# alexandrainst/coral

Hardware: AMD Instinct MI355X
Metric: audio-seconds/sec (CTC finetune step: fwd+bwd+allreduce+clip+AdamW), wav2vec2-large, 10 s utterances (higher is better)
Workload: dtype bf16; 1 GPU; wav2vec2-large (XLS-R shape d=1920 L=48 ffn=7680) CTC finetune, 8 x 10 s per GPU, SpecAugment on, activation_dropout 0.1, layerdrop 0 (multi-GPU rule), fp32 master + AdamW + clip 1.0; global_batch=8, frames_per_utt=499, parallelism=dp1

## Files before the change

### coral_amd/_lib.py

```python

from __future__ import annotations

import ctypes as C
import os
from pathlib import Path

_HERE = Path(__file__).resolve().parent
LIB_PATH = _HERE / "libcoral_amd.so"


class CoralAmdError(RuntimeError):
    """Raised when the HIP library is missing or a call into it fails."""


class CaGemmDesc(C.Structure):

    _fields_ = [
        ("A", C.c_void_p),
        ("B", C.c_void_p),
        ("C", C.c_void_p),
        ("C2", C.c_void_p),
        ("R", C.c_void_p),
        ("bias", C.c_void_p),
        ("M", C.c_int32),
        ("N", C.c_int32),
        ("K", C.c_int32),
        ("a_layout", C.c_int32),
        ("b_layout", C.c_int32),
        ("lda", C.c_int64),
        ("ldb", C.c_int64),
        ("ldc", C.c_int64),
        ("ldr", C.c_int64),
        ("a_kseg", C.c_int32),
        ("b_kseg", C.c_int32),
        ("a_kseg_stride", C.c_int64),
        ("b_kseg_stride", C.c_int64),
        ("batch1", C.c_int32),
        ("batch2", C.c_int32),
        ("sA1", C.c_int64),
        ("sA2", C.c_int64),
        ("sB1", C.c_int64),
        ("sB2", C.c_int64),
        ("sC1", C.c_int64),
        ("sC2", C.c_int64),
        ("sR1", C.c_int64),
        ("sR2", C.c_int64),
        ("sBias1", C.c_int64),
        ("sBias2", C.c_int64),
        ("epilogue", C.c_int32),
        ("out_f32", C.c_int32),
        ("accumulate", C.c_int32),
        ("alpha", C.c_float),
        ("dropout_p", C.c_float),
        ("dropout_seed", C.c_uint64),
        ("a_colsum", C.c_void_p),
        ("a_colsum_ld", C.c_int64),
        ("c_row_index", C.c_void_p),
        ("c_row_mul", C.c_int64),
        ("c_split_n", C.c_int32),
        ("C_hi", C.c_void_p),
        ("ldc_hi", C.c_int64),
        ("a_scale", C.c_void_p),
        ("b_scale", C.c_void_p),
        ("a_row_scale", C.c_void_p),
        ("c_sumsq", C.c_void_p),
        ("c_stream_out", C.c_int32),
        ("C8", C.c_void_p),
        ("c8_scale", C.c_void_p),
        ("c8_amax", C.c_void_p),
        ("a_ln_gamma", C.c_void_p),
        ("a_ln_beta", C.c_void_p),
        ("a_ln_eps", C.c_float),
        ("xcd_balanced", C.c_int32),
    ]


class CaReduceDesc(C.Structure):
    _fields_ = [("partial", C.c_void_p), ("out", C.c_void_p), ("stride", C.c_int64), ("nparts", C.c_int32),
                ("n", C.c_int32), ("accumulate", C.c_int32)]


class CaDecodeLayer(C.Structure):

    FIELDS = ("ln1_g", "ln1_b", "wqkv", "bqkv", "wo", "bo", "ln2_g", "ln2_b", "wq2", "bq2", "wo2", "bo2", "ln3_g", "ln3_b",
              "w1", "b1", "w2", "b2", "self_kv", "cross_kv")
    _fields_ = [(n, C.c_void_p) for n in FIELDS]


class CaDecodeDesc(C.Structure):

    _fields_ = ([("layers", C.c_void_p)]
                + [(n, C.c_int32) for n in ("n_layers", "B", "d", "f", "H", "Te", "max_len", "V")]
                + [(n, C.c_void_p) for n in ("embed", "embed_pos", "lnf_g", "lnf_b")]
                + [("eps", C.c_float), ("logits", C.c_void_p), ("ld_logits", C.c_int64), ("suppress", C.c_void_p),
                   ("out", C.c_void_p), ("done", C.c_void_p), ("ids", C.c_void_p), ("ld_ids", C.c_int64),
                   ("tok", C.c_void_p), ("pos", C.c_void_p), ("klen", C.c_void_p), ("pad_id", C.c_int32),
                   ("eos_id", C.c_int32), ("ws", C.c_void_p), ("ws_bytes", C.c_int64), ("status", C.c_void_p),
                   ("cross_head_major", C.c_int32)])


DECODE_MAX_B = 16


def decode_ws_bytes(B, d, f, H, n_layers):
    return (8192 + n_layers * 16 * H * 4 + 16 * (7 * d + f) * 2 + 16 * H * 4 * 16 * 66 * 4 + 256 * 16 * 8 + 4096)


class CaAttnDesc(C.Structure):

    _fields_ = ([(n, C.c_void_p) for n in ("Q", "K", "V", "O", "dO", "dQ", "dK", "dV", "lse", "Dq", "klen", "key_slot")]
                + [(n, C.c_int64) for n in ("ldq", "ldk", "ldv", "ldo", "lddo", "lddq", "lddk", "lddv",
                                             "sqb", "skb", "svb", "sob", "sdob", "sdqb", "sdkb", "sdvb")]
                + [(n, C.c_int32) for n in ("B", "H", "Tq", "Tk", "hd", "Tqp", "causal")]
                + [("scale", C.c_float), ("dropout_p", C.c_float), ("dropout_seed", C.c_uint64)]
                + [("O8", C.c_void_p), ("o8_scale", C.c_void_p), ("o8_amax", C.c_void_p),
                   ("split_ws", C.c_void_p), ("split_ws_bytes", C.c_int64), ("row_off", C.c_void_p)])


class CaFp8RefreshTask(C.Structure):

    _fields_ = ([(n, C.c_void_p) for n in ("x_bf16", "q_fp8", "q_fp8_t", "scale", "amax_next")]
                + [("rows", C.c_int32), ("cols", C.c_int32)])


class CaCtcBeamDesc(C.Structure):

    _fields_ = [("logits", C.c_void_p), ("ldv", C.c_int64), ("in_len", C.c_void_p),
                ("B", C.c_int32), ("T", C.c_int32), ("V", C.c_int32), ("blank", C.c_int32), ("delimiter", C.c_int32),
                ("forbidden", C.c_void_p), ("pfx_keys", C.c_void_p), ("pfx_wid", C.c_void_p), ("n_pfx", C.c_int64),
                ("ng_keys", C.c_void_p), ("ng_logp", C.c_void_p), ("ng_backoff", C.c_void_p),
                ("ng_count", C.c_int64 * 5),
                ("order", C.c_int32), ("bos_wid", C.c_int32), ("eos_wid", C.c_int32), ("unk_wid", C.c_int32),
                ("beam_width", C.c_int32),
                ("alpha", C.c_float), ("beta", C.c_float), ("unk_score_offset", C.c_float),
                ("token_min_logp", C.c_float), ("beam_prune_logp", C.c_float), ("score_boundary", C.c_int32),
                ("ids_out", C.c_void_p), ("out_len", C.c_void_p), ("score_out", C.c_void_p),
                ("ws", C.c_void_p), ("ws_bytes", C.c_int64)]


class CaBeamDesc(C.Structure):

    _fields_ = ([(n, C.c_int32) for n in ("B", "k", "max_len", "prompt_len", "max_length", "eos_id", "early_stopping")]
                + [(n, C.c_void_p) for n in ("len_pen", "cand_score", "cand_parent", "cand_token", "run_score", "tok", "pos",
                                              "klen", "anc_in", "anc_out", "ids_in", "ids_out", "fin_score", "fin_len",
                                              "fin_seq", "fin_ids", "fin_count", "heur", "done", "tr_parent", "tr_token",
                                              "tr_score")])


BEAM_MAX_BEAMS, BEAM_MAX_ROWS = 16, 128
ALIGN_MAX_TOKENS, ALIGN_MAX_FRAMES, ALIGN_MAX_HEADS, ALIGN_MAX_HEAD_DIM, ALIGN_MAX_FILTER_WIDTH = 447, 1500, 32, 128, 31


def align_ws_bytes_per_clip(A, Lw, Fmax):
    return A * Fmax * (Lw + 4) * 4


FP8_GROUP_MAX = 8
CTC_COLLAPSE_TILE = 4096
KMAJOR, MNMAJOR = 0, 1
EPI_NONE, EPI_GELU, EPI_RESIDUAL, EPI_DGELU, EPI_GELU_RESIDUAL = 0, 1, 2, 3, 4

_vp, _i32, _i64, _f32, _u64 = C.c_void_p, C.c_int32, C.c_int64, C.c_float, C.c_uint64

SIGNATURES = {
    "ca_version": (C.c_int, []),
    "ca_last_error": (C.c_char_p, []),
    "ca_device_count": (C.c_int, []),
    "ca_gemm_bf16_group": (C.c_int, [_vp, _i32, _vp]),
    "ca_gemm_bf16": (C.c_int, [C.POINTER(CaGemmDesc), _vp]),
    "ca_gemm_fp8": (C.c_int, [C.POINTER(CaGemmDesc), _vp]),
    "ca_quantize_fp8": (C.c_int, [_vp, _i64, _vp, _vp, _vp, _vp]),
    "ca_quantize_fp8_delayed": (C.c_int, [_vp, _i64, _vp, _vp, _vp, _vp]),
    "ca_fp8_amax_rotate": (C.c_int, [_vp, _vp, _vp, _i32, _f32, _vp]),
    "ca_dropout_rows_fp8": (C.c_int, [_vp, _vp, _vp, _vp, _i64, _i32, _f32, _u64, _vp]),
    "ca_quantize_fp8_transposed": (C.c_int, [_vp, _i32, _i32, _vp, _vp, _vp]),
    "ca_fp8_refresh_group": (C.c_int, [_vp, _i32, _vp]),
    "ca_gemm_force_kernel": (C.c_int, [C.c_int]),
    "ca_gemm_debug_general_epilogue": (C.c_int, [C.c_int]),
    "ca_debug_cu_hog": (C.c_int, [_i32, _i32, _i32, C.c_double, _vp]),
    "ca_gemm_set_compute_cus": (C.c_int, [C.c_int]),
    "ca_background_update_fits": (C.c_int, [C.POINTER(C.c_int32)]),
    "ca_prof_begin": (C.c_int, []),
    "ca_prof_end": (C.c_int, [C.POINTER(C.c_double), C.POINTER(C.c_int64), C.POINTER(C.c_double)]),
    "ca_pack_rows": (C.c_int, [_vp, _vp, _vp, _i32, _i32, _i32, _i32, _vp]),
    "ca_unpack_rows": (C.c_int, [_vp, _vp, _vp, _i32, _i32, _i32, _i32, _vp]),
    "ca_attn_fwd": (C.c_int, [C.POINTER(CaAttnDesc), _vp]),
    "ca_attn_bwd": (C.c_int, [C.POINTER(CaAttnDesc), _vp]),
    "ca_decode_attn_qproj": (C.c_int, [C.POINTER(CaAttnDesc), _vp, _i64, _vp, _vp, _f32, _vp, _i64, _vp, _i32, _vp]),
    "ca_layernorm_fwd": (C.c_int, [_vp, _vp, _vp, _vp, _vp, _i64, _i32, _f32, _i32, _vp]),
    "ca_layernorm_fwd_ex": (C.c_int, [_vp, _vp, _vp, _vp, _vp, _i64, _i32, _f32, _i32, _i32, _i32, _vp]),
    "ca_layernorm_bwd_ex": (
        C.c_int,
        [_vp, _vp, _vp, _vp, _vp, _vp, _vp, _vp, _vp, _vp, _i64, _i32, _i32, _i32, _vp],
    ),
    "ca_layernorm_bwd_dropout": (
        C.c_int,
        [_vp, _vp, _vp, _vp, _vp, _vp, _vp, _vp, _f32, _u64, _vp, _vp, _vp, _i64, _i32, _i32, _vp],
    ),
    "ca_layernorm_fwd_fp8": (C.c_int, [_vp, _vp, _vp, _vp, _vp, _vp, _vp, _i64, _i32, _f32, _vp]),
    "ca_layernorm_bwd_partial_floats": (_i64, [_i64, _i32]),
    "ca_layernorm_bwd": (
        C.c_int,
        [_vp, _vp, _vp, _vp, _vp, _vp, _vp, _vp, _vp, _vp, _i64, _i32, _i32, _vp],
    ),
    "ca_colsum_partial_floats": (_i64, [_i64, _i32]),
    "ca_colsum_bf16": (C.c_int, [_vp, _i64, _i64, _i32, _vp, _vp, _i32, _vp, _vp]),
    "ca_dgelu_mul": (C.c_int, [_vp, _vp, _vp, _i64, _vp]),
    "ca_dropout_bf16": (C.c_int, [_vp, _vp, _i64, _f32, _u64, _vp]),
    "ca_reduce_rows_f32": (C.c_int, [_vp, _i32, _i64, _i32, _vp, _i32, _vp]),
    "ca_reduce_rows_multi": (C.c_int, [C.POINTER(CaReduceDesc), _i32, _vp]),
    "ca_wave_normalize": (C.c_int, [_vp, _vp, _vp, _i32, _i64, _f32, _vp]),
    "ca_frame_lengths": (C.c_int, [_vp, _i32, _i64, C.POINTER(C.c_int32), C.POINTER(C.c_int32), _i32, _vp, _vp]),
    "ca_wave_scale": (C.c_int, [_vp, _vp, _vp, _i32, _i64, _vp]),
    "ca_fir_filter": (C.c_int, [_vp, _vp, _vp, _vp, _vp, _i64, _i32, _vp, _i32, _i64, _vp]),
    "ca_mix_noise": (C.c_int, [_vp, _vp, _vp, _i64, _i64, _vp, _vp, _vp, _vp, _i32, _i64, _vp]),
    "ca_white_noise": (C.c_int, [_vp, _i64, C.c_uint64, _vp]),
    "ca_pcm_prepare": (C.c_int, [_vp, _i32, _i64, _vp, _vp, _vp, _i32, _i64, _i32, _i32, _f32, _vp]),
    "ca_conv0_ln_gelu_fwd": (
        C.c_int,
        [_vp, _vp, _vp, _vp, _vp, _vp, _i32, _i64, _i32, _i32, _i32, _f32, _vp],
    ),
    "ca_conv0_bwd_partial_floats": (_i64, [_i32, _i64, _i32, _i32, _i32]),
    "ca_conv0_ln_gelu_bwd": (
        C.c_int,
        [_vp] * 11 + [_i32, _i64, _i32, _i32, _i32, _f32, _vp],
    ),
    "ca_col2im_1d": (C.c_int, [_vp, _vp, _i32, _i64, _i64, _i32, _i32, _i32, _vp]),
    "ca_ctc_workspace_bytes": (_i64, [_i32, _i32, _i32]),
    "ca_ctc_loss_fwd_bwd": (
        C.c_int,
        [_vp, _vp, _vp, _vp, _vp, _vp, _vp, _i32, _i32, _i32, _i64, _i32, _i32, _i32, _vp],
    ),
    "ca_ctc_greedy_decode": (
        C.c_int,
        [_vp, _vp, _vp, _vp, _vp, _i32, _i32, _i32, _i64, _i32, _vp],
    ),
    "ca_ctc_stitch": (C.c_int, [_vp, _vp, _vp, _vp, _i32, _i32, _i32, _i64, _i32, _i32, _vp]),
    "ca_ctc_collapse_workspace_bytes": (_i64, [_i32, _i32]),
    "ca_ctc_collapse_offsets": (C.c_int, [_vp, _vp, _vp, _vp, _vp, _vp, _vp, _i64, _i32, _i32, _i32, _vp]),
    "ca_ctc_beam_workspace_bytes": (_i64, [_i32, _i32, _i32, _i32]),
    "ca_ctc_beam_decode": (C.c_int, [C.POINTER(CaCtcBeamDesc), _vp]),
    "ca_beam_select_workspace_bytes": (_i64, [_i32, _i32, _i32]),
    "ca_beam_select": (C.c_int, [_vp, _i64, _vp, _vp, _i32, _i32, _i32, _vp, _vp, _vp, _vp, _i64, _vp]),
    "ca_beam_advance": (C.c_int, [C.POINTER(CaBeamDesc), _vp]),
    "ca_mask_frames": (C.c_int, [_vp, _vp, _vp, _vp, _vp, _i32, _i32, _i32, _vp]),
    "ca_regroup_pad": (C.c_int, [_vp, _vp, _i32, _i32, _i32, _i32, _i32, _vp]),
    "ca_posconv_partial_floats": (_i64, [_i32]),
    "ca_posconv_weight": (C.c_int, [_vp, _vp, _vp, _vp, _vp, _vp, _i32, _i32, _i32, _vp]),
    "ca_posconv_weight_bwd": (
        C.c_int,
        [_vp, _vp, _vp, _vp, _vp, _vp, _vp, _i32, _i32, _i32, _vp],
    ),
    "ca_cast_f32_bf16": (C.c_int, [_vp, _vp, _i64, _vp]),
    "ca_cast_bf16_f32": (C.c_int, [_vp, _vp, _i64, _vp]),
    "ca_transpose_f32_bf16": (C.c_int, [_vp, _vp, _i32, _i32, _vp]),
    "ca_conv_weight_reorder": (C.c_int, [_vp, _vp, _i32, _i32, _i32, _vp]),
    "ca_conv_weight_grad_reorder": (C.c_int, [_vp, _vp, _i32, _i32, _i32, _vp]),
    "ca_sumsq_f32": (C.c_int, [_vp, _i64, _vp, _i32, _vp, _vp]),
    "ca_sumsq_ranges_f32": (C.c_int, [_vp, _vp, _i32, _vp, _i32, _vp, _vp]),
    "ca_clear_ranges": (C.c_int, [_vp, _vp, _i32, _i64, _vp]),
    "ca_sum_f32": (C.c_int, [_vp, _i64, _vp, _i32, _vp, _vp]),
    "ca_adamw_step": (
        C.c_int,
        [_vp, _vp, _vp, _vp, _vp, _i64, _f32, _f32, _f32, _f32, _f32, _i32, _f32, _f32, _vp, _vp],
    ),
    "ca_adamw_step_ex": (
        C.c_int,
        [_vp, _vp, _vp, _vp, _vp, _i64, _f32, _f32, _f32, _f32, _f32, _i32, _f32, _f32, _vp, _i32, _vp],
    ),
    "ca_adamw_step_g16": (
        C.c_int,
        [_vp, _vp, _vp, _vp, _vp, _i64, _f32, _f32, _f32, _f32, _f32, _i32, _f32, _f32, _vp, _i32, _vp],
    ),
    "ca_logmel_workspace_bytes": (_i64, [_i32]),
    "ca_logmel": (C.c_int, [_vp, _vp, _vp, _vp, _i32, _i64, _i32, _vp]),
    "ca_cross_entropy_fwd_bwd": (
        C.c_int,
        [_vp, _vp, _vp, _vp, _vp, _i64, _i32, _i64, _i32, _vp],
    ),
    "ca_argmax_masked": (C.c_int, [_vp, _vp, _vp, _i64, _i32, _i64, _vp]),
    "ca_whisper_decode_token": (C.c_int, [C.POINTER(CaDecodeDesc), _vp]),
    "ca_whisper_decode_token_supported": (C.c_int, [_i32, _i32, _i32, _i32, _i32]),
    "ca_debug_decode_stamps": (C.c_int, [_vp, _i32]),
    "ca_argmax_advance": (C.c_int, [_vp, _vp, _vp, _i64, _i32, _i64, _vp, _vp, _i64, _vp, _vp, _vp, _i32, _i32, _vp]),
    "ca_argmax_timestamps": (C.c_int, [_vp, _vp, _vp, _i64, _i32, _i64, _vp, _i64, _vp, _i32, _i32, _i32, _i32, _vp]),
    "ca_argmax_timestamps_advance": (C.c_int, [_vp, _vp, _vp, _i64, _i32, _i64, _vp, _vp, _i64, _vp, _vp, _vp, _i32, _i32,
                                               _i32, _i32, _i32, _vp]),
    "ca_pick_scored_advance": (C.c_int, [_vp, _vp, _vp, _i64, _i32, _i64, _f32, _vp, _i64, _vp, _vp, _vp, _vp, _i64, _vp, _vp,
                                         _vp, _i32, _i32, _vp, _i32, _i32, _i32, _vp]),
    "ca_row_token_prob": (C.c_int, [_vp, _vp, _i64, _i32, _i64, _i32, _vp]),
    "ca_whisper_align_cost": (C.c_int, [_vp, C.POINTER(_vp), _i32, C.POINTER(_i32), _i32, _i32, _i32, _i32, _i32, _i32, _i64,
                                        _i64, _vp, _i32, _f32, _i32, _vp, _vp, _i64, _vp]),
    "ca_dtw_token_times": (C.c_int, [_vp, _i32, _i32, _vp, _i32, _vp, _vp, _vp, _vp, _vp, _vp]),
    "ca_embed_tokens": (C.c_int, [_vp, _vp, _vp, _vp, _vp, _i64, _i32, _vp]),
    "ca_embed_tokens_bwd": (C.c_int, [_vp, _vp, _vp, _vp, _vp, _i64, _i32, _vp]),
    "ca_comm_unique_id": (C.c_int, [_vp]),
    "ca_comm_init": (C.c_int, [C.POINTER(_vp), _vp, _i32, _i32]),
    "ca_comm_destroy": (C.c_int, [_vp]),
    "ca_comm_abort": (C.c_int, [_vp]),
    "ca_comm_stream": (_vp, [_vp]),
    "ca_comm_rank": (C.c_int, [_vp]),
    "ca_comm_world": (C.c_int, [_vp]),
    "ca_comm_after": (C.c_int, [_vp, _vp]),
    "ca_comm_before": (C.c_int, [_vp, _vp]),
    "ca_allreduce_bucket": (C.c_int, [_vp, _vp, _i64, _i32]),
    "ca_reduce_scatter_bucket": (C.c_int, [_vp, _vp, _i64, _i32]),
    "ca_allgather_bucket": (C.c_int, [_vp, _vp, _i64, _i32]),
}

_lib = None


def load() -> C.CDLL:
    global _lib
    if _lib is not None:
        return _lib
    path = Path(os.environ.get("CORAL_AMD_LIB", LIB_PATH))
    if not path.exists():
        raise CoralAmdError(
            f"{path} not found: build it with `python -c 'import __graft_entry__ as g; "
            "g.build()'` (or `make -C coral_amd/csrc`). There is no CPU fallback."
        )
    lib = C.CDLL(str(path))
    for name, (res, args) in SIGNATURES.items():
        fn = getattr(lib, name)
        fn.restype = res
        fn.argtypes = args
    _lib = lib
    return lib

# ... 6 lines not shown
```

### coral_amd/csrc/gemm.hip

```cpp
#include "common.h"
#include "gemm_plan.h"
#include <type_traits>
#include <cstdlib>

#define TILE_BYTES (BM * BK * 2)
#define STAGE_BYTES (2 * TILE_BYTES)
#define NSTAGE 2
static_assert(LDS_BYTES >= NSTAGE * STAGE_BYTES, "kernel S: the epilogue staging covers the operand stages");

__device__ __attribute__((aligned(16))) uint32_t g_ca_zero_page[4];
__device__ int g_ca_epi_general = 0;

typedef const __attribute__((address_space(1))) void* gptr_t;
typedef __attribute__((address_space(3))) void* lptr_t;

__device__ __forceinline__ void glds16(const void* g, char* lds_wave_base) {
  asm volatile("s_mov_b32 m0, %1\n\ts_nop 0\n\tglobal_load_lds_dwordx4 %0, off"
               :
               : "v"(g), "s"((uint32_t)(uintptr_t)(lptr_t)lds_wave_base)
               : "memory", "m0");
}

template <int NI>
struct KMajorLoader {
// ... 97 lines not shown
  __device__ __forceinline__ void init_bytes(const char* b, int64_t ld, int row0, int nrows, int wave, int lane) {
    base = b + (int64_t)row0 * ld;
#pragma unroll
    for (int i = 0; i < NI; ++i) {
      const int r = (wave * NI + i) * 8 + (lane >> 3);
      const int c = (lane & 7) ^ ((r >> 1) & 7);
      int rr = row0 + r;
      rr = (rr < nrows ? rr : nrows - 1) - row0;
      kc[i] = c * 16;
      off[i] = (uint32_t)((int64_t)rr * ld + c * 16);
    }
  }
  __device__ __forceinline__ void issue_one(char* tile, int wave, int i) {
    glds16_sbase(base, off[i], (uint32_t)(uintptr_t)(lptr_t)(tile + (wave * NI + i) * 1024));
  }
  __device__ __forceinline__ void issue_one_tail(char* tile, int wave, int krem, int i) {
    glds16_sbase(base, kc[i] < krem ? off[i] : 0u, (uint32_t)(uintptr_t)(lptr_t)(tile + (wave * NI + i) * 1024));
  }
  __device__ __forceinline__ void zero_fix(char* tile, int wave, int lane, int krem) {
#pragma unroll
    for (int i = 0; i < NI; ++i)
      if (kc[i] >= krem) *(uint4*)(tile + (wave * NI + i) * 1024 + lane * 16) = make_uint4(0, 0, 0, 0);
  }
  __device__ __forceinline__ void advance() { base += BK * 2; }
};
template <int NI, int PC>
struct MNMajorStream {
  const char* base;
  uint32_t off[NI];
  int64_t step;
  static constexpr int RPI = 64 / PC;
  __device__ __forceinline__ void init(const __bf16* b, int64_t ld, int col0, int ncols, int wave, int lane) {
    base = (const char*)(b + col0);
    step = (int64_t)BK * ld * 2;
#pragma unroll
    for (int i = 0; i < NI; ++i) {
      const int kr = (wave * NI + i) * RPI + lane / PC;
      const int swz = (kr & 3) | (((kr >> 3) & 1) << 2);
      const int c = (lane % PC) ^ (swz << 1);
      int cc = col0 + c * 8;
      const int nc8 = (ncols + 7) & ~7;
      cc = (cc <= nc8 - 8 ? cc : nc8 - 8) - col0;
      off[i] = (uint32_t)(((int64_t)kr * ld + cc) * 2);
    }
  }
  __device__ __forceinline__ void issue_one(char* tile, int wave, int i) {
    glds16_sbase(base, off[i], (uint32_t)(uintptr_t)(lptr_t)(tile + (wave * NI + i) * 1024));
  }
  __device__ __forceinline__ void issue_one_tail(char* tile, int wave, int lane, int krem, int i) {
    const int kr = (wave * NI + i) * RPI + lane / PC;
    glds16_sbase(base, kr < krem ? off[i] : 0u, (uint32_t)(uintptr_t)(lptr_t)(tile + (wave * NI + i) * 1024));
  }
  __device__ __forceinline__ void zero_fix(char* tile, int wave, int lane, int krem) {
#pragma unroll
    for (int i = 0; i < NI; ++i) {
      const int kr = (wave * NI + i) * RPI + lane / PC;
      if (kr >= krem) *(uint4*)(tile + (wave * NI + i) * 1024 + lane * 16) = make_uint4(0, 0, 0, 0);
    }
  }
  __device__ __forceinline__ void advance() { base += step; }
};

__device__ __forceinline__ bf16x8_t frag_kmajor(const char* tile, int rb, int s, int lane) {
  const int r = rb + (lane & 15);
  const int c = (4 * s + (lane >> 4)) ^ ((r >> 1) & 7);
  return *(const bf16x8_t*)(tile + r * 128 + c * 16);
}
__device__ __forceinline__ bf16x8_t frag_kmajor_async(const char* tile, int rb, int s, int lane) {
  const int r = rb + (lane & 15);
  const int c = (4 * s + (lane >> 4)) ^ ((r >> 1) & 7);
  const uint32_t a = (uint32_t)(uintptr_t)(lptr_t)(tile + r * 128 + c * 16);
  bf16x8_t v;
  asm volatile("ds_read_b128 %0, %1" : "=v"(v) : "v"(a));
  return v;
}
template <int PITCH>
__device__ __forceinline__ bf16x8_t frag_mnmajor(const char* tile, int cb, int s, int lane) {
  const int g = lane >> 4;
  const int q = (lane & 15) >> 2;
  const int p = lane & 3;
  const int kr = 32 * s + 8 * g + q;
  const int swz = q | ((g & 1) << 2);
  const int c = ((cb >> 3) + (p >> 1)) ^ (swz << 1);
  const uint32_t a0 = (uint32_t)(uintptr_t)(lptr_t)(tile + kr * PITCH + c * 16 + (p & 1) * 8);
  s16x4_t lo, hi;
  asm volatile("ds_read_b64_tr_b16 %0, %1" : "=v"(lo) : "v"(a0));
  asm volatile("ds_read_b64_tr_b16 %0, %1 offset:%2" : "=v"(hi) : "v"(a0), "n"(4 * PITCH));
  typedef __attribute__((ext_vector_type(8))) short s16x8_t;
  s16x8_t v = {lo[0], lo[1], lo[2], lo[3], hi[0], hi[1], hi[2], hi[3]};
  return __builtin_bit_cast(bf16x8_t, v);
}
template <int OFF>
__device__ __forceinline__ bf16x8_t lds_read_b128(uint32_t a) {
  static_assert(OFF >= 0 && OFF < 65536, "DS immediate offset");
  bf16x8_t v;
  asm volatile("ds_read_b128 %0, %1 offset:%2" : "=v"(v) : "v"(a), "n"(OFF));
  return v;
}
template <int OFF, int HI>
__device__ __forceinline__ bf16x8_t lds_read_tr(uint32_t a) {
  static_assert(OFF >= 0 && OFF + HI < 65536, "DS immediate offset");
  s16x4_t lo, hi;
  asm volatile("ds_read_b64_tr_b16 %0, %1 offset:%2" : "=v"(lo) : "v"(a), "n"(OFF));
  asm volatile("ds_read_b64_tr_b16 %0, %1 offset:%2" : "=v"(hi) : "v"(a), "n"(OFF + HI));
  typedef __attribute__((ext_vector_type(8))) short s16x8_t;
  s16x8_t v = {lo[0], lo[1], lo[2], lo[3], hi[0], hi[1], hi[2], hi[3]};
  return __builtin_bit_cast(bf16x8_t, v);
}
__device__ __forceinline__ void lds_wait(bf16x8_t (&f)[4]) {
  asm volatile("s_waitcnt lgkmcnt(0)" : "+v"(f[0]), "+v"(f[1]), "+v"(f[2]), "+v"(f[3]));
}

template <int SBM, int SBN>
__device__ __forceinline__ bool tile_of_block(int bid, int ntm, int ntn, int& tm, int& tn, bool bal = false) {
  return tile_of_block_g<SBM, SBN>(bid, (int)gridDim.x, ntm, ntn, tm, tn, bal);
}

__device__ __forceinline__ void epi_load_bias(const CaGemmDesc& d, int lane, int nw, int z1, int z2, float (&bias8)[8]) {
  const int nb = nw + 8 * (lane & 7);
  const int nvalid = (d.N - nb) < 8 ? (d.N - nb) : 8;
#pragma unroll
  for (int e = 0; e < 8; ++e) bias8[e] = 0.f;
  if (d.bias && nvalid > 0) {
    const float* bz = d.bias + z1 * d.sBias1 + z2 * d.sBias2 + nb;
    if (nvalid == 8 && (((uintptr_t)bz) & 15) == 0) {
      const f32x4_t b0 = *(const f32x4_t*)bz, b1 = *(const f32x4_t*)(bz + 4);
#pragma unroll
      for (int e = 0; e < 8; ++e) bias8[e] = e < 4 ? b0[e] : b1[e - 4];
    } else {
#pragma unroll
      for (int e = 0; e < 8; ++e)
        if (e < nvalid) bias8[e] = bz[e];
    }
  }
}
__device__ __forceinline__ void ca_store_fp8x8(unsigned char* dst, const float (&v)[8], float scale, float& amx) {
  float t[8];
#pragma unroll
  for (int e = 0; e < 8; ++e) {
    amx = fmaxf(amx, fabsf(v[e]));
    t[e] = fminf(fmaxf(v[e] * scale, -448.0f), 448.0f);
  }
  unsigned int w0 = 0, w1 = 0;
  w0 = __builtin_amdgcn_cvt_pk_fp8_f32(t[0], t[1], w0, false);
  w0 = __builtin_amdgcn_cvt_pk_fp8_f32(t[2], t[3], w0, true);
  w1 = __builtin_amdgcn_cvt_pk_fp8_f32(t[4], t[5], w1, false);
  w1 = __builtin_amdgcn_cvt_pk_fp8_f32(t[6], t[7], w1, true);
  *(uint2*)dst = make_uint2(w0, w1);
}

template <int EPI, bool F32, bool DROP>
__device__ __forceinline__ void gemm_epilogue_fast(const CaGemmDesc& d, const float* wt, int lane, int mw, int nb, int z,
                                                   int64_t zoffC, int64_t zoffR, const float (&bias8)[8], float& ssq,
                                                   float& amx) {
  const int M = d.M, N = d.N;
  const float alpha = d.alpha;
  const float keep_scale = DROP ? 1.f / (1.f - d.dropout_p) : 1.f;
  const int r0 = lane >> 3, c0 = 8 * (lane & 7);
  constexpr bool NEEDS_R = EPI == CA_EPI_RESIDUAL || EPI == CA_EPI_DGELU;
  const unsigned short* Rp = NEEDS_R ? (const unsigned short*)d.R + zoffR + nb + (int64_t)(mw + r0) * d.ldr : nullptr;
  const int64_t rstep = 8 * d.ldr;
  int64_t coff = zoffC + (int64_t)(mw + r0) * d.ldc + nb;
  const int64_t cstep = 8 * d.ldc;
  uint64_t idx = ((uint64_t)z * M + (mw + r0)) * (uint64_t)N + nb;
  const uint64_t istep = 8ull * (uint64_t)N;
  u16x8_t r_next = {0, 0, 0, 0, 0, 0, 0, 0};
  if (NEEDS_R) r_next = *(const u16x8_t*)Rp;
  const bool c8_on = (EPI == CA_EPI_GELU || EPI == CA_EPI_DGELU) && d.C8 != nullptr;
  const float s8 = c8_on ? d.c8_scale[0] : 1.f;
  unsigned int dg = 0, ds_eff = 0, dthr = 0;
  if (DROP) {
    const uint64_t ilo = ((uint64_t)z * M + mw) * (uint64_t)N;
    const unsigned int sd = (unsigned int)d.dropout_seed * 0x9E3779B9u + (unsigned int)(d.dropout_seed >> 32);
    ds_eff = sd ^ ((unsigned int)(ilo >> 34) * 0x85EBCA6Bu);
    dg = (unsigned int)(idx >> 2);
    dthr = ca_dropout_threshold(d.dropout_p);
  }
  const unsigned int dgstep = (unsigned int)(istep >> 2);
#pragma unroll 2
  for (int it = 0; it < 8; ++it) {
    const u16x8_t r_cur = r_next;
    if (NEEDS_R && it < 7) r_next = *(const u16x8_t*)(Rp + (it + 1) * rstep);
    const float* wr = wt + (it * 8 + r0) * EPI_PITCH + c0;
    const f32x4_t a4 = *(const f32x4_t*)wr, b4 = *(const f32x4_t*)(wr + 4);
    float v[8];
#pragma unroll
    for (int e = 0; e < 8; ++e) v[e] = (e < 4 ? a4[e] : b4[e - 4]) * alpha + bias8[e];
    unsigned int keep = 0xFFu;
    if (DROP) {
      keep = ca_dropout_keep4_lo(ds_eff, dg, dthr) | (ca_dropout_keep4_lo(ds_eff, dg + 1, dthr) << 4);
      dg += dgstep;
    }
    float v2[8];
    if (EPI == CA_EPI_GELU) {
#pragma unroll
      for (int e = 0; e < 8; ++e) {
        float g = gelu_erf(v[e]);
        if (DROP) g = ((keep >> e) & 1u) ? g * keep_scale : 0.f;
        v2[e] = g + 0.f;
      }
    } else if (EPI == CA_EPI_RESIDUAL) {
      if (DROP) {
#pragma unroll
        for (int e = 0; e < 8; ++e) v[e] = ((keep >> e) & 1u) ? v[e] * keep_scale : 0.f;
      }
#pragma unroll
      for (int e = 0; e < 8; ++e) v[e] += bf2f(r_cur[e]);
    } else if (EPI == CA_EPI_DGELU) {
#pragma unroll
      for (int e = 0; e < 8; ++e) {
        float dg = dgelu_erf(bf2f(r_cur[e]));
        if (DROP) dg = ((keep >> e) & 1u) ? dg * keep_scale : 0.f;
        v[e] *= dg;
      }
    }
    if (F32) {
      float* C = (float*)d.C + coff;
      if (d.accumulate) {
        const f32x4_t c0v = *(const f32x4_t*)C, c1v = *(const f32x4_t*)(C + 4);
#pragma unroll
        for (int e = 0; e < 8; ++e) v[e] += e < 4 ? c0v[e] : c1v[e - 4];
      }
      if (d.c_stream_out) {
        __builtin_nontemporal_store((f32x4_t){v[0], v[1], v[2], v[3]}, (f32x4_t*)C);
        __builtin_nontemporal_store((f32x4_t){v[4], v[5], v[6], v[7]}, (f32x4_t*)(C + 4));
      } else {
        *(f32x4_t*)C = (f32x4_t){v[0], v[1], v[2], v[3]};
        *(f32x4_t*)(C + 4) = (f32x4_t){v[4], v[5], v[6], v[7]};
      }
#pragma unroll
      for (int e = 0; e < 8; ++e) ssq = fmaf(v[e], v[e], ssq);
    } else {
      u16x8_t o;
#pragma unroll
      for (int e = 0; e < 8; ++e) o[e] = f2bf(v[e]);
      if (d.c_stream_out)
        __builtin_nontemporal_store(o, (u16x8_t*)((unsigned short*)d.C + coff));
      else
        *(u16x8_t*)((unsigned short*)d.C + coff) = o;
      if (EPI == CA_EPI_NONE && d.c_sumsq != nullptr) {
#pragma unroll
        for (int e = 0; e < 8; ++e) ssq = fmaf(bf2f(o[e]), bf2f(o[e]), ssq);
      }
      if (EPI == CA_EPI_DGELU && c8_on) ca_store_fp8x8((unsigned char*)d.C8 + coff, v, s8, amx);
    }
    if (EPI == CA_EPI_GELU) {
      u16x8_t o;
#pragma unroll
      for (int e = 0; e < 8; ++e) o[e] = f2bf(v2[e]);
      *(u16x8_t*)((unsigned short*)d.C2 + coff) = o;
      if (c8_on) ca_store_fp8x8((unsigned char*)d.C8 + coff, v2, s8, amx);
    }
    coff += cstep;
  }
}

template <bool PARKED = false>
__device__ __forceinline__ void gemm_epilogue(const CaGemmDesc& d, f32x4_t (&acc)[4][4], char* smem,
                                              int wave, int lane, int mw, int nw, int z, int z1,
                                              int z2, const float (*bias_pre)[8] = nullptr) {
  const int M = d.M, N = d.N;
  const int64_t zoffC = z1 * d.sC1 + z2 * d.sC2;
  const int64_t zoffR = z1 * d.sR1 + z2 * d.sR2;
  const bool vec_ok = ((d.ldc & 7) == 0) && ((zoffC & 7) == 0) && ((d.ldr & 7) == 0) && ((zoffR & 7) == 0);
  const float keep_scale = d.dropout_p > 0.f ? 1.f / (1.f - d.dropout_p) : 1.f;
  const int nb = nw + 8 * (lane & 7);
  const int nvalid = (N - nb) < 8 ? (N - nb) : 8;
  const bool full = nvalid == 8 && vec_ok;
  const int epi = d.epilogue;
  const bool has_gelu = epi == CA_EPI_GELU || epi == CA_EPI_GELU_RESIDUAL;
  const bool needs_r = epi == CA_EPI_RESIDUAL || epi == CA_EPI_DGELU || epi == CA_EPI_GELU_RESIDUAL;
  float bias8[8];
  if (bias_pre) {
#pragma unroll
    for (int e = 0; e < 8; ++e) bias8[e] = (*bias_pre)[e];
  } else {
    epi_load_bias(d, lane, nw, z1, z2, bias8);
  }
  const unsigned short* Rbase = (const unsigned short*)d.R + zoffR + nb;
  auto load_r = [&](int it, u16x8_t& u) {
    const int m = mw + it * 8 + (lane >> 3);
    if (needs_r && full && it < 8 && m < M) u = *(const u16x8_t*)(Rbase + (int64_t)m * d.ldr);
  };
  u16x8_t r_next = {0, 0, 0, 0, 0, 0, 0, 0};
  load_r(0, r_next);

  float* wt = (float*)smem + wave * (64 * EPI_PITCH);
  if (!PARKED) {
#pragma unroll
    for (int i = 0; i < 4; ++i)
#pragma unroll
      for (int j = 0; j < 4; ++j)
        *(f32x4_t*)(wt + (i * 16 + (lane & 15)) * EPI_PITCH + j * 16 + 4 * (lane >> 4)) = acc[i][j];
    asm volatile("s_waitcnt lgkmcnt(0)" ::: "memory");
  }
  const bool c8_on = d.C8 != nullptr && (epi == CA_EPI_GELU || epi == CA_EPI_DGELU);
  if (nvalid <= 0 && d.c_sumsq == nullptr && !c8_on) return;
  float ssq = 0.f;
  float amx = 0.f;
  const float s8 = c8_on ? d.c8_scale[0] : 1.f;
  const bool drop_on = d.dropout_p > 0.f;
  const bool drop32_ok = !drop_on || ((((uint64_t)z * M + mw) * (uint64_t)N) >> 34) == ((((uint64_t)z * M + mw + 64) * (uint64_t)N) >> 34);
  const bool interior = g_ca_epi_general == 0 && mw + 64 <= M && nw + 64 <= N && vec_ok && (N & 7) == 0 && d.C != nullptr && drop32_ok &&
                        (d.out_f32 || !d.accumulate) && (!has_gelu || (epi == CA_EPI_GELU && d.C2 != nullptr && !d.out_f32)) &&
                        !(d.out_f32 && epi != CA_EPI_NONE) && !(drop_on && epi == CA_EPI_NONE);
  if (interior) {
#define EPI_FAST(E, F, D) gemm_epilogue_fast<E, F, D>(d, wt, lane, mw, nb, z, zoffC, zoffR, bias8, ssq, amx)
    if (d.out_f32) {
      EPI_FAST(CA_EPI_NONE, true, false);
    } else if (epi == CA_EPI_NONE) {
      EPI_FAST(CA_EPI_NONE, false, false);
    } else if (epi == CA_EPI_GELU) {
      if (drop_on) EPI_FAST(CA_EPI_GELU, false, true); else EPI_FAST(CA_EPI_GELU, false, false);
    } else if (epi == CA_EPI_RESIDUAL) {
      if (drop_on) EPI_FAST(CA_EPI_RESIDUAL, false, true); else EPI_FAST(CA_EPI_RESIDUAL, false, false);
    } else {
      if (drop_on) EPI_FAST(CA_EPI_DGELU, false, true); else EPI_FAST(CA_EPI_DGELU, false, false);
    }
#undef EPI_FAST
  } else {
#pragma unroll 1
  for (int it = 0; it < 8; ++it) {
    const int ml = it * 8 + (lane >> 3);
    const int m = mw + ml;
    const u16x8_t r_cur = r_next;
    load_r(it + 1, r_next);
    if (m >= M || nvalid <= 0) continue;
    const f32x4_t a4 = *(const f32x4_t*)(wt + ml * EPI_PITCH + 8 * (lane & 7));
    const f32x4_t b4 = *(const f32x4_t*)(wt + ml * EPI_PITCH + 8 * (lane & 7) + 4);
    float v[8], v2[8], r[8];
#pragma unroll
    for (int e = 0; e < 8; ++e) {
      v[e] = (e < 4 ? a4[e] : b4[e - 4]) * d.alpha + bias8[e];
      v2[e] = 0.f;
      r[e] = 0.f;
    }
    const int64_t coff = zoffC + (int64_t)m * d.ldc + nb;
    if (needs_r) {
      if (full) {
#pragma unroll
        for (int e = 0; e < 8; ++e) r[e] = bf2f(r_cur[e]);
      } else {
        const unsigned short* R = Rbase + (int64_t)m * d.ldr;
#pragma unroll
        for (int e = 0; e < 8; ++e)
          if (e < nvalid) r[e] = bf2f(R[e]);
      }
    }
    unsigned int keep = 0xFFu;
    if (d.dropout_p > 0.f && (has_gelu || epi == CA_EPI_DGELU || epi == CA_EPI_RESIDUAL)) {
      const uint64_t idx = ((uint64_t)z * M + m) * (uint64_t)N + nb;
      if ((idx & 3) == 0) {
        keep = ca_dropout_keep4(d.dropout_seed, idx, d.dropout_p) |
               (ca_dropout_keep4(d.dropout_seed, idx + 4, d.dropout_p) << 4);
      } else {
        keep = 0;
#pragma unroll
        for (int e = 0; e < 8; ++e) keep |= (ca_dropout_keep(d.dropout_seed, idx + e, d.dropout_p) ? 1u : 0u) << e;
      }
    }
    if (has_gelu) {
#pragma unroll
      for (int e = 0; e < 8; ++e) {
        float g = gelu_erf(v[e]);
        if (d.dropout_p > 0.f) g = ((keep >> e) & 1u) ? g * keep_scale : 0.f;
        v2[e] = g + r[e];
      }
    } else if (epi == CA_EPI_RESIDUAL) {
      if (d.dropout_p > 0.f) {
#pragma unroll
        for (int e = 0; e < 8; ++e) v[e] = ((keep >> e) & 1u) ? v[e] * keep_scale : 0.f;
      }
#pragma unroll
      for (int e = 0; e < 8; ++e) v[e] += r[e];
    } else if (epi == CA_EPI_DGELU) {
#pragma unroll
      for (int e = 0; e < 8; ++e) {
        float dg = dgelu_erf(r[e]);
        if (d.dropout_p > 0.f) dg = ((keep >> e) & 1u) ? dg * keep_scale : 0.f;
        v[e] *= dg;
      }
    }
    if (d.out_f32) {
      float* C = (float*)d.C + coff;
      if (full) {
        if (d.accumulate) {
          const f32x4_t c0 = *(const f32x4_t*)C, c1 = *(const f32x4_t*)(C + 4);
#pragma unroll
          for (int e = 0; e < 8; ++e) v[e] += e < 4 ? c0[e] : c1[e - 4];
        }
        *(f32x4_t*)C = (f32x4_t){v[0], v[1], v[2], v[3]};
        *(f32x4_t*)(C + 4) = (f32x4_t){v[4], v[5], v[6], v[7]};
#pragma unroll
        for (int e = 0; e < 8; ++e) ssq = fmaf(v[e], v[e], ssq);
      } else {
#pragma unroll
        for (int e = 0; e < 8; ++e)
          if (e < nvalid) {
            const float t = d.accumulate ? C[e] + v[e] : v[e];
            C[e] = t;
            ssq = fmaf(t, t, ssq);
          }
      }
    } else if (d.C) {
      unsigned short* C = (unsigned short*)d.C + coff;
      if (full) {
        if (d.accumulate) {
          const u16x8_t c = *(const u16x8_t*)C;
#pragma unroll
          for (int e = 0; e < 8; ++e) v[e] += bf2f(c[e]);
        }
        u16x8_t o;
#pragma unroll
        for (int e = 0; e < 8; ++e) o[e] = f2bf(v[e]);
        *(u16x8_t*)C = o;
        if (d.c_sumsq != nullptr) {
#pragma unroll
          for (int e = 0; e < 8; ++e) ssq = fmaf(bf2f(o[e]), bf2f(o[e]), ssq);
        }
      } else {
#pragma unroll
        for (int e = 0; e < 8; ++e)
          if (e < nvalid) {
            const unsigned short t = f2bf(d.accumulate ? bf2f(C[e]) + v[e] : v[e]);
            C[e] = t;
            ssq = fmaf(bf2f(t), bf2f(t), ssq);
          }
      }
    }
    if (has_gelu && d.C2) {
      unsigned short* C2 = (unsigned short*)d.C2 + coff;
      if (full) {
        u16x8_t o;
#pragma unroll
        for (int e = 0; e < 8; ++e) o[e] = f2bf(v2[e]);
        *(u16x8_t*)C2 = o;
      } else {
#pragma unroll
        for (int e = 0; e < 8; ++e)
          if (e < nvalid) C2[e] = f2bf(v2[e]);
      }
    }
    if (c8_on) {
      unsigned char* C8 = (unsigned char*)d.C8 + coff;
      float w8[8];
#pragma unroll
      for (int e = 0; e < 8; ++e) w8[e] = epi == CA_EPI_GELU ? v2[e] : v[e];
      if (full) {
        ca_store_fp8x8(C8, w8, s8, amx);
      } else {
#pragma unroll
        for (int e = 0; e < 8; ++e)
          if (e < nvalid) {
            amx = fmaxf(amx, fabsf(w8[e]));
            const float t = fminf(fmaxf(w8[e] * s8, -448.0f), 448.0f);
            C8[e] = (unsigned char)(__builtin_amdgcn_cvt_pk_fp8_f32(t, 0.f, 0u, false) & 0xffu);
          }
      }
    }
  }
  }
  if (d.c_sumsq != nullptr) {
#pragma unroll
    for (int o = 32; o > 0; o >>= 1) ssq += __shfl_xor(ssq, o, 64);
    if (lane == 0 && mw < M && nw < N) d.c_sumsq[(int64_t)(mw >> 6) * ((N + 63) >> 6) + (nw >> 6)] = ssq;
  }
  if (c8_on && d.c8_amax != nullptr) {
#pragma unroll
    for (int o = 32; o > 0; o >>= 1) amx = fmaxf(amx, __shfl_xor(amx, o, 64));
    if (lane == 0 && amx > 0.f)
      atomicMax((unsigned int*)d.c8_amax + (((mw >> 6) * 7 + (nw >> 6)) & (CA_FP8_AMAX_SLOTS - 1)), __float_as_uint(amx));
  }
}

template <int AL, int BL, bool KS>
__global__ __launch_bounds__(256) void ca_gemm_kernel(const CaGemmDesc d) {
  extern __shared__ __attribute__((aligned(16))) char smem[];
  const int tid = threadIdx.x;
  const int lane = tid & 63;
  const int wave = __builtin_amdgcn_readfirstlane(tid >> 6);
// ... 130 lines not shown
  asm volatile("" ::: "memory");
  gemm_epilogue(d, acc, smem, wave, lane, m0 + wm * 64, n0 + wn * 64, z, z1, z2);
}

#define M_NST 4
static_assert(M_LDS_BYTES == 2 * M_NST * TILE_BYTES, "131072 >= 4 quadrants * 64*68*4 (69632) of epilogue staging");
template <int N>
__device__ __forceinline__ void lds_wait_n(bf16x8_t (&f)[N]) {
  if constexpr (N == 4)
    asm volatile("s_waitcnt lgkmcnt(0)" : "+v"(f[0]), "+v"(f[1]), "+v"(f[2]), "+v"(f[3]));
  else
    asm volatile("s_waitcnt lgkmcnt(0)" : "+v"(f[0]), "+v"(f[1]));
}
template <int AL, int BL>
__global__ __launch_bounds__(512) void ca_gemm_kernel_m(const CaGemmDesc d) {
  extern __shared__ __attribute__((aligned(16))) char smem[];
  const int tid = threadIdx.x;
  const int lane = tid & 63;
  const int wave = __builtin_amdgcn_readfirstlane(tid >> 6);
  const int wm = wave >> 2, wn = wave & 3;
  int tm, tn;
  if (!tile_of_block<8, 8>(blockIdx.x, (d.M + BM - 1) / BM, (d.N + BN - 1) / BN, tm, tn, d.xcd_balanced != 0)) return;
  const int m0 = tm * BM, n0 = tn * BN;
  const int z = blockIdx.z;
  const int z1 = z / d.batch2, z2 = z % d.batch2;
  const __bf16* A = (const __bf16*)d.A + z1 * d.sA1 + z2 * d.sA2;
  const __bf16* B = (const __bf16*)d.B + z1 * d.sB1 + z2 * d.sB2;
  const int K = d.K;
  const int nk = (K + BK - 1) / BK;

  KMajorStream<2> la_k, lb_k;
  MNMajorStream<2, 16> la_f, lb_f;
  if (AL == CA_KMAJOR) la_k.init(A, d.lda, m0, d.M, wave, lane); else la_f.init(A, d.lda, m0, d.M, wave, lane);
  if (BL == CA_KMAJOR) lb_k.init(B, d.ldb, n0, d.N, wave, lane); else lb_f.init(B, d.ldb, n0, d.N, wave, lane);

  f32x4_t acc[4][2];
#pragma unroll
  for (int i = 0; i < 4; ++i)
#pragma unroll
    for (int j = 0; j < 2; ++j) acc[i][j] = (f32x4_t){0.f, 0.f, 0.f, 0.f};

  auto burst = [&](int kt) {
    if (kt >= nk) return;
    char* na = smem + (kt % M_NST) * TILE_BYTES;
    char* nb = na + M_NST * TILE_BYTES;
    const bool full = (kt + 1) * BK <= K;
#pragma unroll
    for (int part = 0; part < 2; ++part) {
      if (full) {
        if (AL == CA_KMAJOR) la_k.issue_one(na, wave, part); else la_f.issue_one(na, wave, part);
        if (BL == CA_KMAJOR) lb_k.issue_one(nb, wave, part); else lb_f.issue_one(nb, wave, part);
      } else {
        if (AL == CA_KMAJOR) la_k.issue_one_tail(na, wave, K - kt * BK, part); else la_f.issue_one_tail(na, wave, lane, K - kt * BK, part);
        if (BL == CA_KMAJOR) lb_k.issue_one_tail(nb, wave, K - kt * BK, part); else lb_f.issue_one_tail(nb, wave, lane, K - kt * BK, part);
      }
    }
    if (AL == CA_KMAJOR) la_k.advance(); else la_f.advance();
    if (BL == CA_KMAJOR) lb_k.advance(); else lb_f.advance();
  };
  auto zero_tail = [&](int kt) {
    if (kt != nk - 1 || nk * BK == K) return;
    char* na = smem + (kt % M_NST) * TILE_BYTES;
    char* nb = na + M_NST * TILE_BYTES;
    const int krem = K - kt * BK;
    if (AL == CA_KMAJOR) la_k.zero_fix(na, wave, lane, krem); else la_f.zero_fix(na, wave, lane, krem);
    if (BL == CA_KMAJOR) lb_k.zero_fix(nb, wave, lane, krem); else lb_f.zero_fix(nb, wave, lane, krem);
    asm volatile("s_waitcnt lgkmcnt(0)" ::: "memory");
  };
#pragma unroll
  for (int p = 0; p < M_NST - 1; ++p) burst(p);
  for (int kt = 0; kt < nk; ++kt) {
    if (kt + 2 < nk)
      asm volatile("s_waitcnt vmcnt(8) lgkmcnt(0)" ::: "memory");
    else if (kt + 1 < nk)
      asm volatile("s_waitcnt vmcnt(4) lgkmcnt(0)" ::: "memory");
    else
      asm volatile("s_waitcnt vmcnt(0) lgkmcnt(0)" ::: "memory");
    zero_tail(kt);
    __builtin_amdgcn_s_barrier();
    asm volatile("" ::: "memory");
    burst(kt + M_NST - 1);

    const char* ta = smem + (kt % M_NST) * TILE_BYTES;
    const char* tb = ta + M_NST * TILE_BYTES;
    auto read_frags = [&](int sh, bf16x8_t (&af)[4], bf16x8_t (&bf)[2]) {
#pragma unroll
      for (int i = 0; i < 4; ++i)
        af[i] = (AL == CA_KMAJOR) ? frag_kmajor_async(ta, wm * 64 + i * 16, sh, lane)
                                  : frag_mnmajor<256>(ta, wm * 64 + i * 16, sh, lane);
#pragma unroll
      for (int j = 0; j < 2; ++j)
        bf[j] = (BL == CA_KMAJOR) ? frag_kmajor_async(tb, wn * 32 + j * 16, sh, lane)
                                  : frag_mnmajor<256>(tb, wn * 32 + j * 16, sh, lane);
    };
    auto mma = [&](bf16x8_t (&af)[4], bf16x8_t (&bf)[2]) {
#pragma unroll
      for (int i = 0; i < 4; ++i)
#pragma unroll
        for (int j = 0; j < 2; ++j) acc[i][j] = __builtin_amdgcn_mfma_f32_16x16x32_bf16(bf[j], af[i], acc[i][j], 0, 0, 0);
    };
    bf16x8_t a0[4], b0[2], a1[4], b1[2];
    read_frags(0, a0, b0);
    lds_wait_n(a0);
    lds_wait_n(b0);
    read_frags(1, a1, b1);
    __builtin_amdgcn_sched_barrier(0);
    mma(a0, b0);
    __builtin_amdgcn_sched_barrier(0);
    lds_wait_n(a1);
    lds_wait_n(b1);
    mma(a1, b1);
  }
  asm volatile("s_waitcnt lgkmcnt(0)" ::: "memory");
  __builtin_amdgcn_s_barrier();
  asm volatile("" ::: "memory");
  const int quad = wm * 2 + (wn >> 1);
  float* wt = (float*)smem + quad * (64 * EPI_PITCH);
#pragma unroll
  for (int i = 0; i < 4; ++i)
#pragma unroll
    for (int j = 0; j < 2; ++j)
      *(f32x4_t*)(wt + (i * 16 + (lane & 15)) * EPI_PITCH + (wn & 1) * 32 + j * 16 + 4 * (lane >> 4)) = acc[i][j];
  asm volatile("s_waitcnt lgkmcnt(0)" ::: "memory");
  __builtin_amdgcn_s_barrier();
  asm volatile("" ::: "memory");
  if ((wn & 1) == 0) {
    f32x4_t none[4][4];
    gemm_epilogue<true>(d, none, smem, quad, lane, m0 + wm * 64, n0 + (wn >> 1) * 64, z, z1, z2);
  }
}

#define XTILE (XBM * BK * 2)
#define XSTAGE (2 * XTILE)
static_assert(X_LDS_BYTES >= 2 * XSTAGE, "kernel X: the epilogue staging covers the two operand stages");

#define X_GROUP_MAX 8
struct CaGemmGroup {
  CaGemmDesc d[X_GROUP_MAX];
  int first[X_GROUP_MAX];
  int count;
  int total;
  int vgrid;
  unsigned* cnt;
  int dyn_first;
};
#define X_CNT_SLOTS 64
__device__ unsigned g_x_cnt[X_CNT_SLOTS][8];
#ifdef X_STAMPS
__device__ long long g_x_stamps[512 * 8 * 8];
extern "C" int ca_gemm_x_stamps(long long* host, int n) {
  return (int)hipMemcpyFromSymbol(host, HIP_SYMBOL(g_x_stamps), (size_t)n * sizeof(long long));
}
#endif
template <int AL, int BL, bool KS>
__device__ __forceinline__ void gemm_x_body(const CaGemmGroup& grp) {
  extern __shared__ __attribute__((aligned(16))) char smem[];
  const int tid = threadIdx.x;
  const int lane = tid & 63;
  const int wave = __builtin_amdgcn_readfirstlane(tid >> 6);
  const int wm = wave >> 2, wn = wave & 3;
  const int vgrid = grp.vgrid;
  const int xcd = (int)blockIdx.x & 7;
  const int npx = ((int)gridDim.x - xcd + 7) >> 3;
  const int nvx = (vgrid - xcd + 7) >> 3;
  const int ndyn = nvx > npx ? nvx - npx : 0;
  volatile unsigned* nextw = (volatile unsigned*)(smem + X_LDS_BYTES);
  KMajorStream<4> la_k, lb_k;
  MNMajorStream<4, 32> la_f, lb_f;
  MNMajorLoader<4, 32, KS> la_m, lb_m;
  int vb = (int)blockIdx.x;
  int dbase = npx, dcount = ndyn;
  if (grp.cnt != nullptr && grp.dyn_first) {
    dbase = 0;
    dcount = nvx;
    if (tid == 0) {
      const unsigned i = __hip_atomic_fetch_add(&grp.cnt[xcd], 1u, __ATOMIC_RELAXED, __HIP_MEMORY_SCOPE_AGENT);
      if (i == (unsigned)(dcount + npx - 1)) __hip_atomic_store(&grp.cnt[xcd], 0u, __ATOMIC_RELAXED, __HIP_MEMORY_SCOPE_AGENT);
      nextw[1] = i;
    }
    __syncthreads();
    const unsigned i = (unsigned)__builtin_amdgcn_readfirstlane((int)nextw[1]);
    vb = i < (unsigned)dcount ? xcd + 8 * (int)i : vgrid;
  }
  for (int iter = 0; vb < vgrid; ++iter) {
  int vb_next = vgrid;
  if (grp.cnt != nullptr && tid == 0) {
    const unsigned i = __hip_atomic_fetch_add(&grp.cnt[xcd], 1u, __ATOMIC_RELAXED, __HIP_MEMORY_SCOPE_AGENT);
    if (i == (unsigned)(dcount + npx - 1)) __hip_atomic_store(&grp.cnt[xcd], 0u, __ATOMIC_RELAXED, __HIP_MEMORY_SCOPE_AGENT);
    nextw[iter & 1] = i;
  }
  bool live = true;
  int which = 0, gt = 0;
  if (grp.count > 1) {
    gt = (vb & 7) * (vgrid >> 3) + (vb >> 3);
    live = gt < grp.total;
    if (live) {
#pragma unroll
      for (int i = 1; i < X_GROUP_MAX; ++i)
        if (grp.count > i && gt >= grp.first[i]) which = i;
    }
  }
  const CaGemmDesc d = grp.d[which];
  int tm = 0, tn = 0;
  if (live) {
    if (grp.count > 1)
      run_tile(gt - grp.first[which], (d.M + XBM - 1) / XBM, (d.N + XBN - 1) / XBN, tm, tn);
    else
      live = tile_of_block_g<4, 8>(vb, vgrid, (d.M + XBM - 1) / XBM, (d.N + XBN - 1) / XBN, tm, tn, d.xcd_balanced != 0);
  }
  if (live) {
  const int m0 = tm * XBM, n0 = tn * XBN;
  const int z = blockIdx.z;
  const int z1 = z / d.batch2, z2 = z % d.batch2;
  const __bf16* A = (const __bf16*)d.A + z1 * d.sA1 + z2 * d.sA2;
  const __bf16* B = (const __bf16*)d.B + z1 * d.sB1 + z2 * d.sB2;

  auto init_loaders = [&](int row0, int col0) {
    if (AL == CA_KMAJOR)
      la_k.init(A, d.lda, row0, d.M, wave, lane);
    else if (KS)
      la_m.init(A, d.lda, d.a_kseg, d.a_kseg_stride, row0, d.M, wave, lane);
    else
      la_f.init(A, d.lda, row0, d.M, wave, lane);
    if (BL == CA_KMAJOR)
      lb_k.init(B, d.ldb, col0, d.N, wave, lane);
    else if (KS)
      lb_m.init(B, d.ldb, d.b_kseg, d.b_kseg_stride, col0, d.N, wave, lane);
    else
      lb_f.init(B, d.ldb, col0, d.N, wave, lane);
  };
  init_loaders(m0, n0);

  f32x4_t acc[8][4];
#pragma unroll
  for (int i = 0; i < 8; ++i)
#pragma unroll
    for (int j = 0; j < 4; ++j) acc[i][j] = (f32x4_t){0.f, 0.f, 0.f, 0.f};
  float xbias[8];
  if constexpr (!KS) epi_load_bias(d, lane, n0 + wn * 64, z1, z2, xbias);
#ifdef X_STAMPS
  long long stamp_dma = 0, stamp_bar = 0;
#endif
  const int cs_parts = ((d.N + XBN - 1) / XBN) < 8 ? ((d.N + XBN - 1) / XBN) : 8;
  const bool do_colsum = d.a_colsum != nullptr && tn < cs_parts;
  float csum0 = 0.f, csum1 = 0.f;

  const int K = d.K;
  const int nk = (K + BK - 1) / BK;

  auto burst = [&](int kt) {
    if (kt >= nk) return;
    char* na = smem + (kt & 1) * XTILE;
    char* nb = na + 2 * XTILE;
    const bool full = (kt + 1) * BK <= K;
    if (full) {
#pragma unroll
      for (int part = 0; part < 4; ++part) {
        if (AL == CA_MNMAJOR && KS)
          la_m.issue_one(na, wave, lane, kt * BK, K, part);
        else if (AL == CA_KMAJOR)
          la_k.issue_one(na, wave, part);
        else
          la_f.issue_one(na, wave, part);
        if (BL == CA_MNMAJOR && KS)
          lb_m.issue_one(nb, wave, lane, kt * BK, K, part);
        else if (BL == CA_KMAJOR)
          lb_k.issue_one(nb, wave, part);
        else
          lb_f.issue_one(nb, wave, part);
      }
    } else {
#pragma unroll
      for (int part = 0; part < 4; ++part) {
        if (AL == CA_MNMAJOR && KS)
          la_m.issue_one(na, wave, lane, kt * BK, K, part);
        else if (AL == CA_KMAJOR)
          la_k.issue_one_tail(na, wave, K - kt * BK, part);
        else
          la_f.issue_one_tail(na, wave, lane, K - kt * BK, part);
        if (BL == CA_MNMAJOR && KS)
          lb_m.issue_one(nb, wave, lane, kt * BK, K, part);
        else if (BL == CA_KMAJOR)
          lb_k.issue_one_tail(nb, wave, K - kt * BK, part);
        else
          lb_f.issue_one_tail(nb, wave, lane, K - kt * BK, part);
      }
    }
    if (AL == CA_KMAJOR) la_k.advance();
    if (AL == CA_MNMAJOR && !KS) la_f.advance();
    if (BL == CA_KMAJOR) lb_k.advance();
    if (BL == CA_MNMAJOR && !KS) lb_f.advance();
  };
  auto zero_tail = [&](int kt) {
    if (kt != nk - 1 || nk * BK == K) return;
    char* na = smem + (kt & 1) * XTILE;
    char* nb = na + 2 * XTILE;
    const int krem = K - kt * BK;
    if (AL == CA_KMAJOR) la_k.zero_fix(na, wave, lane, krem);
    if (AL == CA_MNMAJOR && !KS) la_f.zero_fix(na, wave, lane, krem);
    if (BL == CA_KMAJOR) lb_k.zero_fix(nb, wave, lane, krem);
    if (BL == CA_MNMAJOR && !KS) lb_f.zero_fix(nb, wave, lane, krem);
    asm volatile("s_waitcnt lgkmcnt(0)" ::: "memory");
  };
  const uint32_t lds0 = (uint32_t)(uintptr_t)(lptr_t)smem;
  uint32_t abase[8], bbase[4];
  if (AL == CA_KMAJOR) {
    const int r = wm * 128 + (lane & 15);
#pragma unroll
    for (int sh = 0; sh < 2; ++sh) abase[sh] = lds0 + r * 128 + (((4 * sh + (lane >> 4)) ^ ((r >> 1) & 7)) * 16);
  } else {
    const int g = lane >> 4, q = (lane & 15) >> 2, pp = lane & 3;
    const int swz = q | ((g & 1) << 2);
#pragma unroll
    for (int f = 0; f < 8; ++f) {
      const int c = ((((wm * 128 + f * 16) >> 3) + (pp >> 1)) ^ (swz << 1));
      abase[f] = lds0 + (8 * g + q) * 512 + c * 16 + (pp & 1) * 8;
    }
  }
  if (BL == CA_KMAJOR) {
    const int r = wn * 64 + (lane & 15);
#pragma unroll
    for (int sh = 0; sh < 2; ++sh)
      bbase[sh] = lds0 + 2 * XTILE + r * 128 + (((4 * sh + (lane >> 4)) ^ ((r >> 1) & 7)) * 16);
  } else {
    const int g = lane >> 4, q = (lane & 15) >> 2, pp = lane & 3;
    const int swz = q | ((g & 1) << 2);
#pragma unroll
    for (int f = 0; f < 4; ++f) {
      const int c = ((((wn * 64 + f * 16) >> 3) + (pp >> 1)) ^ (swz << 1));
      bbase[f] = lds0 + 2 * XTILE + (8 * g + q) * 512 + c * 16 + (pp & 1) * 8;
    }
  }
  bf16x8_t A0[4], A1[4], B0[4], B1[4];
#define X_RD_A(ST, SH, F, dst)                                                            \
  do {                                                                                    \
    if (AL == CA_KMAJOR)                                                                  \
      dst = lds_read_b128<(ST) * XTILE + (F) * 2048>(abase[SH]);                          \
    else                                                                                  \
      dst = lds_read_tr<(ST) * XTILE + (SH) * 16384, 2048>(abase[F]);                     \
  } while (0)
#define X_RD_B(ST, SH, F, dst)                                                            \
  do {                                                                                    \
    if (BL == CA_KMAJOR)                                                                  \
      dst = lds_read_b128<(ST) * XTILE + (F) * 2048>(bbase[SH]);                          \
    else                                                                                  \
      dst = lds_read_tr<(ST) * XTILE + (SH) * 16384, 2048>(bbase[F]);                     \
  } while (0)
#define X_SB __builtin_amdgcn_sched_barrier(0)
#define X_MM2(IH, AF, BF, I, J)                                                                                   \
  do {                                                                                                            \
    acc[(IH) * 4 + (I)][J] = __builtin_amdgcn_mfma_f32_16x16x32_bf16(BF[J], AF[I], acc[(IH) * 4 + (I)][J], 0, 0, 0); \
    acc[(IH) * 4 + (I)][(J) + 1] =                                                                                \
        __builtin_amdgcn_mfma_f32_16x16x32_bf16(BF[(J) + 1], AF[I], acc[(IH) * 4 + (I)][(J) + 1], 0, 0, 0);       \
    X_SB;                                                                                                         \
  } while (0)
  auto colsum_acc = [&](bool cs_step, int ih, bf16x8_t (&af)[4]) {
    if (AL == CA_MNMAJOR && cs_step) {
      f32x4_t z;
      if (wn == 0)
        z = __builtin_bit_cast(f32x4_t, af[0]);
      else if (wn == 1)
        z = __builtin_bit_cast(f32x4_t, af[1]);
      else if (wn == 2)
        z = __builtin_bit_cast(f32x4_t, af[2]);
      else
        z = __builtin_bit_cast(f32x4_t, af[3]);
      typedef __attribute__((ext_vector_type(2))) __bf16 bf16x2_t;
      const bf16x2_t ones = __builtin_bit_cast(bf16x2_t, 0x3F803F80u);
      float s = ih == 0 ? csum0 : csum1;
#pragma unroll
      for (int q = 0; q < 4; ++q) {
        const unsigned int wq = __float_as_uint(z[q]);
        s = __builtin_amdgcn_fdot2_f32_bf16(__builtin_bit_cast(bf16x2_t, wq), ones, s, false);
      }
      if (ih == 0)
        csum0 = s;
      else
        csum1 = s;
    }
  };
  auto kstep = [&](auto st_c, int kt) {
    constexpr int ST = decltype(st_c)::value;
    const bool cs_step = do_colsum && (kt % cs_parts) == tn;
    constexpr bool LATE_BURST = AL == CA_MNMAJOR && BL == CA_MNMAJOR && !KS;
    if (!LATE_BURST && wave >= 4) burst(kt + 1);
    lds_wait(B0);
    lds_wait(A0);
    colsum_acc(cs_step, 0, A0);
    X_SB;
    __builtin_amdgcn_s_setprio(1);
    X_MM2(0, A0, B0, 0, 0); X_RD_A(ST, 0, 4, A1[0]); X_SB;
    X_MM2(0, A0, B0, 0, 2); X_RD_A(ST, 0, 5, A1[1]); X_SB;
    X_MM2(0, A0, B0, 1, 0); X_RD_A(ST, 0, 6, A1[2]); X_SB;
    X_MM2(0, A0, B0, 1, 2); X_RD_A(ST, 0, 7, A1[3]); X_SB;
    X_MM2(0, A0, B0, 2, 0);
    X_MM2(0, A0, B0, 2, 2);
    X_MM2(0, A0, B0, 3, 0);
    X_MM2(0, A0, B0, 3, 2);
    __builtin_amdgcn_s_setprio(0);
    if (LATE_BURST && wave >= 4) burst(kt + 1);
    lds_wait(A1);
    colsum_acc(cs_step, 1, A1);
    X_SB;
    __builtin_amdgcn_s_setprio(1);
    X_MM2(1, A1, B0, 0, 0); X_RD_B(ST, 1, 0, B1[0]); X_SB;
    X_MM2(1, A1, B0, 0, 2); X_RD_B(ST, 1, 1, B1[1]); X_SB;
    X_MM2(1, A1, B0, 1, 0); X_RD_B(ST, 1, 2, B1[2]); X_SB;
    X_MM2(1, A1, B0, 1, 2); X_RD_B(ST, 1, 3, B1[3]); X_SB;
    X_MM2(1, A1, B0, 2, 0); X_RD_A(ST, 1, 0, A0[0]); X_SB;
    X_MM2(1, A1, B0, 2, 2); X_RD_A(ST, 1, 1, A0[1]); X_SB;
    X_MM2(1, A1, B0, 3, 0); X_RD_A(ST, 1, 2, A0[2]); X_SB;
    X_MM2(1, A1, B0, 3, 2); X_RD_A(ST, 1, 3, A0[3]); X_SB;
    __builtin_amdgcn_s_setprio(0);
    lds_wait(B1);
    lds_wait(A0);
    colsum_acc(cs_step, 0, A0);
    X_SB;
    __builtin_amdgcn_s_setprio(1);
    X_MM2(0, A0, B1, 0, 0); X_RD_A(ST, 1, 4, A1[0]); X_SB;
    X_MM2(0, A0, B1, 0, 2); X_RD_A(ST, 1, 5, A1[1]); X_SB;
    X_MM2(0, A0, B1, 1, 0); X_RD_A(ST, 1, 6, A1[2]); X_SB;
    X_MM2(0, A0, B1, 1, 2); X_RD_A(ST, 1, 7, A1[3]); X_SB;
    X_MM2(0, A0, B1, 2, 0);
    X_MM2(0, A0, B1, 2, 2);
    X_MM2(0, A0, B1, 3, 0);
    X_MM2(0, A0, B1, 3, 2);
    __builtin_amdgcn_s_setprio(0);
    lds_wait(A1);
    colsum_acc(cs_step, 1, A1);
#ifdef X_STAMPS
    const long long st0 = __builtin_amdgcn_s_memtime();
#endif
    asm volatile("s_waitcnt vmcnt(0)" ::: "memory");
#ifdef X_STAMPS
    const long long st1 = __builtin_amdgcn_s_memtime();
#endif
    zero_tail(kt + 1);
    __builtin_amdgcn_s_barrier();
    asm volatile("" ::: "memory");
#ifdef X_STAMPS
    const long long st2 = __builtin_amdgcn_s_memtime();
    stamp_dma += st1 - st0;
    stamp_bar += st2 - st1;
#endif
    if (wave < 4) burst(kt + 2);
    X_SB;
    __builtin_amdgcn_s_setprio(1);
    X_MM2(1, A1, B1, 0, 0); X_RD_B(1 - ST, 0, 0, B0[0]); X_SB;
    X_MM2(1, A1, B1, 0, 2); X_RD_B(1 - ST, 0, 1, B0[1]); X_SB;
    X_MM2(1, A1, B1, 1, 0); X_RD_B(1 - ST, 0, 2, B0[2]); X_SB;
    X_MM2(1, A1, B1, 1, 2); X_RD_B(1 - ST, 0, 3, B0[3]); X_SB;
    X_MM2(1, A1, B1, 2, 0); X_RD_A(1 - ST, 0, 0, A0[0]); X_SB;
    X_MM2(1, A1, B1, 2, 2); X_RD_A(1 - ST, 0, 1, A0[1]); X_SB;
    X_MM2(1, A1, B1, 3, 0); X_RD_A(1 - ST, 0, 2, A0[2]); X_SB;
    X_MM2(1, A1, B1, 3, 2); X_RD_A(1 - ST, 0, 3, A0[3]); X_SB;
    __builtin_amdgcn_s_setprio(0);
  };
#ifdef X_STAMPS
  const long long stamp_t0 = __builtin_amdgcn_s_memtime();
#endif
  burst(0);
  asm volatile("s_waitcnt vmcnt(0) lgkmcnt(0)" ::: "memory");
  zero_tail(0);
  __builtin_amdgcn_s_barrier();
  asm volatile("" ::: "memory");
#ifdef X_STAMPS
  const long long stamp_t1 = __builtin_amdgcn_s_memtime();
  const long long stamp_r1 = __builtin_amdgcn_s_memrealtime();
  __builtin_amdgcn_s_waitcnt(0xC07F);
#endif
  X_RD_B(0, 0, 0, B0[0]); X_RD_B(0, 0, 1, B0[1]); X_RD_B(0, 0, 2, B0[2]); X_RD_B(0, 0, 3, B0[3]);
  X_RD_A(0, 0, 0, A0[0]); X_RD_A(0, 0, 1, A0[1]); X_RD_A(0, 0, 2, A0[2]); X_RD_A(0, 0, 3, A0[3]);
  if (wave < 4) burst(1);
  for (int kt = 0; kt < nk; kt += 2) {
    kstep(std::integral_constant<int, 0>{}, kt);
    if (kt + 1 < nk) kstep(std::integral_constant<int, 1>{}, kt + 1);
  }
#undef X_RD_A
#undef X_RD_B
#undef X_MM2
#undef X_SB
#ifdef X_STAMPS
  const long long stamp_t2 = __builtin_amdgcn_s_memtime();
  const long long stamp_r2 = __builtin_amdgcn_s_memrealtime();
#endif
  if (AL == CA_MNMAJOR && do_colsum) {
#pragma unroll
    for (int ih = 0; ih < 2; ++ih) {
      float s = ih == 0 ? csum0 : csum1;
      s += __shfl_xor(s, 16, 64);
      s += __shfl_xor(s, 32, 64);
      const int m = m0 + wm * 128 + (ih * 4 + wn) * 16 + (lane & 15);
      if (lane < 16 && m < d.M) d.a_colsum[(int64_t)tn * d.a_colsum_ld + m] = s;
    }
  }
  unsigned nxt = 0;
  if (grp.cnt != nullptr) nxt = (unsigned)__builtin_amdgcn_readfirstlane((int)nextw[iter & 1]);
  asm volatile("s_waitcnt lgkmcnt(0)" ::: "memory");
  __builtin_amdgcn_s_barrier();
  asm volatile("" ::: "memory");
  if (grp.cnt != nullptr) vb_next = nxt < (unsigned)dcount ? xcd + 8 * (dbase + (int)nxt) : vgrid;
#pragma unroll
  for (int ih = 0; ih < 2; ++ih) {
    f32x4_t half[4][4];
#pragma unroll
    for (int i = 0; i < 4; ++i)
#pragma unroll
      for (int j = 0; j < 4; ++j) half[i][j] = acc[ih * 4 + i][j];
    gemm_epilogue(d, half, smem, wave, lane, m0 + wm * 128 + ih * 64, n0 + wn * 64, z, z1, z2, KS ? nullptr : &xbias);
    asm volatile("s_waitcnt lgkmcnt(0)" ::: "memory");
  }
  if (grp.cnt != nullptr) __syncthreads();
#ifdef X_STAMPS
  {
    asm volatile("s_waitcnt vmcnt(0)" ::: "memory");
    const long long stamp_t3 = __builtin_amdgcn_s_memtime();
    if (lane == 0 && iter == 0) {
      long long* o = g_x_stamps + ((size_t)blockIdx.x * 8 + wave) * 8;
      o[0] = stamp_t1 - stamp_t0;
      o[1] = stamp_t2 - stamp_t1;
      o[2] = stamp_t3 - stamp_t2;
      o[3] = stamp_dma;
      o[4] = stamp_bar;
      o[5] = nk;
      o[6] = stamp_r2 - stamp_r1;
    }
  }
#endif
  }
  else if (grp.cnt != nullptr) {
    __syncthreads();
    const unsigned i = (unsigned)__builtin_amdgcn_readfirstlane((int)nextw[iter & 1]);
    vb_next = i < (unsigned)dcount ? xcd + 8 * (dbase + (int)i) : vgrid;
  }
  if (grp.cnt == nullptr) break;
  vb = vb_next;
  }
}

template <int AL, int BL, bool KS>
__global__ __launch_bounds__(512) void ca_gemm_kernel_x(const CaGemmGroup grp) {
  gemm_x_body<AL, BL, KS>(grp);
}
template <>
__global__ __launch_bounds__(512) __attribute__((amdgpu_num_vgpr(112)))
void ca_gemm_kernel_x<CA_KMAJOR, CA_KMAJOR, false>(const CaGemmGroup grp) {
  gemm_x_body<CA_KMAJOR, CA_KMAJOR, false>(grp);
}

#define LA_BYTES (LBM * BK * 2)
#define LB_BYTES (LBN * BK * 2)
#define L_NST 3
static_assert(L_LDS_BYTES == L_NST * (LA_BYTES + LB_BYTES), "147456 >= 8 waves * 64*68*4 (139264) epilogue staging");

template <int AL, int BL>
__global__ __launch_bounds__(512) void ca_gemm_kernel_l(const CaGemmDesc d) {
  extern __shared__ __attribute__((aligned(16))) char smem[];
  const int tid = threadIdx.x;
  const int lane = tid & 63;
  const int wave = __builtin_amdgcn_readfirstlane(tid >> 6);
  const int wm = wave >> 1, wn = wave & 1;
  int tm, tn;
  if (!tile_of_block<4, 8>(blockIdx.x, (d.M + LBM - 1) / LBM, (d.N + LBN - 1) / LBN, tm, tn, d.xcd_balanced != 0)) return;
  const int m0 = tm * LBM, n0 = tn * LBN;
  const int z = blockIdx.z;
  const int z1 = z / d.batch2, z2 = z % d.batch2;
  const __bf16* A = (const __bf16*)d.A + z1 * d.sA1 + z2 * d.sA2;
  const __bf16* B = (const __bf16*)d.B + z1 * d.sB1 + z2 * d.sB2;
  const int K = d.K;
  const int nk = (K + BK - 1) / BK;

  KMajorStream<4> la_k;
  KMajorStream<2> lb_k;
  MNMajorStream<4, 32> la_f;
  MNMajorStream<2, 16> lb_f;
  if (AL == CA_KMAJOR)
    la_k.init(A, d.lda, m0, d.M, wave, lane);
  else
    la_f.init(A, d.lda, m0, d.M, wave, lane);
  if (BL == CA_KMAJOR)
    lb_k.init(B, d.ldb, n0, d.N, wave, lane);
  else
    lb_f.init(B, d.ldb, n0, d.N, wave, lane);

  f32x4_t acc[4][4];
#pragma unroll
  for (int i = 0; i < 4; ++i)
#pragma unroll
    for (int j = 0; j < 4; ++j) acc[i][j] = (f32x4_t){0.f, 0.f, 0.f, 0.f};
  float lbias[8];
  epi_load_bias(d, lane, n0 + wn * 64, z1, z2, lbias);

  int bst = 0;
  auto burst = [&](int kt) {
    if (kt >= nk) return;
    char* na = smem + bst * LA_BYTES;
    char* nb = smem + L_NST * LA_BYTES + bst * LB_BYTES;
    bst = bst == L_NST - 1 ? 0 : bst + 1;
    const bool full = (kt + 1) * BK <= K;
    if (full) {
#pragma unroll
      for (int part = 0; part < 4; ++part) {
        if (AL == CA_KMAJOR)
          la_k.issue_one(na, wave, part);
        else
          la_f.issue_one(na, wave, part);
        if (part < 2) {
          if (BL == CA_KMAJOR)
            lb_k.issue_one(nb, wave, part);
          else
            lb_f.issue_one(nb, wave, part);
        }
      }
    } else {
#pragma unroll
      for (int part = 0; part < 4; ++part) {
        if (AL == CA_KMAJOR)
          la_k.issue_one_tail(na, wave, K - kt * BK, part);
        else
          la_f.issue_one_tail(na, wave, lane, K - kt * BK, part);
        if (part < 2) {
          if (BL == CA_KMAJOR)
            lb_k.issue_one_tail(nb, wave, K - kt * BK, part);
          else
            lb_f.issue_one_tail(nb, wave, lane, K - kt * BK, part);
        }
      }
    }
    if (AL == CA_KMAJOR) la_k.advance(); else la_f.advance();
    if (BL == CA_KMAJOR) lb_k.advance(); else lb_f.advance();
  };
  auto zero_tail = [&](int kt) {
    if (kt != nk - 1 || nk * BK == K) return;
    char* na = smem + (kt % L_NST) * LA_BYTES;
    char* nb = smem + L_NST * LA_BYTES + (kt % L_NST) * LB_BYTES;
    const int krem = K - kt * BK;
    if (AL == CA_KMAJOR) la_k.zero_fix(na, wave, lane, krem); else la_f.zero_fix(na, wave, lane, krem);
    if (BL == CA_KMAJOR) lb_k.zero_fix(nb, wave, lane, krem); else lb_f.zero_fix(nb, wave, lane, krem);
    asm volatile("s_waitcnt lgkmcnt(0)" ::: "memory");
  };
  const uint32_t lds0 = (uint32_t)(uintptr_t)(lptr_t)smem;
  uint32_t abase[4], bbase[4];
  if (AL == CA_KMAJOR) {
    const int r = wm * 64 + (lane & 15);
#pragma unroll
    for (int sh = 0; sh < 2; ++sh) abase[sh] = lds0 + r * 128 + (((4 * sh + (lane >> 4)) ^ ((r >> 1) & 7)) * 16);
  } else {
    const int g = lane >> 4, q = (lane & 15) >> 2, pp = lane & 3;
    const int swz = q | ((g & 1) << 2);
#pragma unroll
    for (int f = 0; f < 4; ++f) {
      const int c = ((((wm * 64 + f * 16) >> 3) + (pp >> 1)) ^ (swz << 1));
      abase[f] = lds0 + (8 * g + q) * 512 + c * 16 + (pp & 1) * 8;
    }
  }
  if (BL == CA_KMAJOR) {
    const int r = wn * 64 + (lane & 15);
#pragma unroll
    for (int sh = 0; sh < 2; ++sh)
      bbase[sh] = lds0 + L_NST * LA_BYTES + r * 128 + (((4 * sh + (lane >> 4)) ^ ((r >> 1) & 7)) * 16);
  } else {
    const int g = lane >> 4, q = (lane & 15) >> 2, pp = lane & 3;
    const int swz = q | ((g & 1) << 2);
#pragma unroll
    for (int f = 0; f < 4; ++f) {
      const int c = ((((wn * 64 + f * 16) >> 3) + (pp >> 1)) ^ (swz << 1));
      bbase[f] = lds0 + L_NST * LA_BYTES + (8 * g + q) * 256 + c * 16 + (pp & 1) * 8;
    }
  }
  uint32_t abase2[4];
#pragma unroll
  for (int f = 0; f < 4; ++f) abase2[f] = abase[f] + 2 * LA_BYTES;
  bf16x8_t A0[4], A1[4], B0[4], B1[4];
#define L_RD_A(ST, SH, F, dst)                                                                      \
  do {                                                                                              \
    if (AL == CA_KMAJOR)                                                                            \
      dst = lds_read_b128<((ST) % 2) * LA_BYTES + (F) * 2048>((ST) == 2 ? abase2[SH] : abase[SH]);  \
    else                                                                                            \
      dst = lds_read_tr<((ST) % 2) * LA_BYTES + (SH) * 16384, 2048>((ST) == 2 ? abase2[F] : abase[F]); \
  } while (0)
#define L_RD_B(ST, SH, F, dst)                                                  \
  do {                                                                          \
    if (BL == CA_KMAJOR)                                                        \
      dst = lds_read_b128<(ST) * LB_BYTES + (F) * 2048>(bbase[SH]);             \
    else                                                                        \
      dst = lds_read_tr<(ST) * LB_BYTES + (SH) * 8192, 1024>(bbase[F]);         \
  } while (0)
#define L_SB __builtin_amdgcn_sched_barrier(0)
#define L_MM2(AF, BF, I, J)                                                                             \
  do {                                                                                                  \
    acc[I][J] = __builtin_amdgcn_mfma_f32_16x16x32_bf16(BF[J], AF[I], acc[I][J], 0, 0, 0);              \
    acc[I][(J) + 1] = __builtin_amdgcn_mfma_f32_16x16x32_bf16(BF[(J) + 1], AF[I], acc[I][(J) + 1], 0, 0, 0); \
    L_SB;                                                                                               \
  } while (0)
  auto kstep = [&](auto st_c, int kt) {
    constexpr int ST = decltype(st_c)::value;
    constexpr int NS = (ST + 1) % L_NST;
    if (wave >= 4) burst(kt + 2);
    lds_wait(B0);
    lds_wait(A0);
// ... 159 lines not shown
      for (int c = 0; c < NC; ++c) {
        if (lane + c * 64 < nchunk) {
#pragma unroll
          for (int e = 0; e < 8; ++e) sx += bf2f(raw[i][c][e]);
        }
      }
      const float mean = wave_sum(sx) / (float)C;
      float s2 = 0.f;
#pragma unroll
      for (int c = 0; c < NC; ++c) {
        if (lane + c * 64 < nchunk) {
#pragma unroll
          for (int e = 0; e < 8; ++e) {
            const float dlt = bf2f(raw[i][c][e]) - mean;
            s2 += dlt * dlt;
          }
        }
      }
      const float rstd = rsqrtf(wave_sum(s2) / (float)C + d.a_ln_eps);
#pragma unroll
      for (int c = 0; c < NC; ++c) {
        const int ch = lane + c * 64;
        if (ch < nchunk) {
          u16x8_t o8;
#pragma unroll
          for (int e = 0; e < 8; ++e)
            o8[e] = f2bf(ln_apply(bf2f(raw[i][c][e]), mean, rstd, e < 4 ? gq[c][0][e] : gq[c][1][e - 4],
                                  e < 4 ? bq[c][0][e] : bq[c][1][e - 4]));
          *(u16x8_t*)(xs + (int64_t)lrow * xpitch + ch * 8) = o8;
        }
      }
    }
    __syncthreads();
  }
  for (int ks = ks0; ks < ks1; ks += U) {
    bf16x8_t wf[U], af[MB][U];
#pragma unroll
    for (int u = 0; u < U; ++u) {
      const int k = (ks + u) * 32 + 8 * g;
      const bool ok = ks + u < ks1 && k < d.K;
      if constexpr (LN) {
        wf[u] = ks == ks0 ? wf0[u] : (ok ? *(const bf16x8_t*)(wp + (int64_t)(ks + u) * 32) : zero);
#pragma unroll
        for (int mb = 0; mb < MB; ++mb)
          af[mb][u] = (ok && mrow0 + 16 * mb + r < d.M) ? *(const bf16x8_t*)(xs + (int64_t)(16 * mb + r) * xpitch + k) : zero;
      } else {
        wf[u] = ok ? *(const bf16x8_t*)(wp + (int64_t)(ks + u) * 32) : zero;
#pragma unroll
        for (int mb = 0; mb < MB; ++mb)
          af[mb][u] = (ok && mrow0 + 16 * mb + r < d.M) ? *(const bf16x8_t*)(ap[mb] + (int64_t)(ks + u) * 32) : zero;
      }
    }
#pragma unroll
    for (int u = 0; u < U; ++u)
#pragma unroll
      for (int mb = 0; mb < MB; ++mb) acc[mb] = __builtin_amdgcn_mfma_f32_16x16x32_bf16(wf[u], af[mb][u], acc[mb], 0, 0, 0);
  }
#pragma unroll
  for (int mb = 0; mb < MB; ++mb)
#pragma unroll
    for (int e = 0; e < 4; ++e) part[wave][mb * 256 + r * 16 + 4 * g + e] = acc[mb][e];
  __syncthreads();
  if (!wave0) return;
#pragma unroll
  for (int mb = 0; mb < MB; ++mb) {
    if (mrow0 + 16 * mb + r >= d.M) continue;
#pragma unroll
    for (int e = 0; e < 4; ++e) {
      const int n = n0 + 4 * g + e;
      if (n >= d.N || 4 * g + e >= NT) continue;
      const int i = mb * 256 + r * 16 + 4 * g + e;
      float v = (part[0][i] + part[1][i]) + (part[2][i] + part[3][i]);
      v = v * d.alpha + e_bias[e];
      float v2 = 0.f;
      if (epi == CA_EPI_GELU || epi == CA_EPI_GELU_RESIDUAL) {
        v2 = gelu_erf(v);
        if (epi == CA_EPI_GELU_RESIDUAL) v2 += e_res[mb][e];
      } else if (epi == CA_EPI_RESIDUAL) {
        v += e_res[mb][e];
      }
      const int64_t off = crow[mb] * ldcd + (n - ncol0);
      if (Cdst) {
        if (d.out_f32)
          ((float*)Cdst)[off] = d.accumulate ? ((float*)Cdst)[off] + v : v;
        else
          ((unsigned short*)Cdst)[off] = f2bf(d.accumulate ? bf2f(((unsigned short*)Cdst)[off]) + v : v);
      }
      if ((epi == CA_EPI_GELU || epi == CA_EPI_GELU_RESIDUAL) && d.C2) ((unsigned short*)d.C2)[off] = f2bf(v2);
    }
  }
}

#include <hip/hip_ext.h>
#include <vector>
struct ProfRec {
  hipEvent_t e0, e1;
  double flops;
  int variant;
};
static bool g_prof_on = false;
static std::vector<ProfRec> g_prof;
static hipEvent_t g_prof_e0 = nullptr, g_prof_e1 = nullptr;
#define CA_LAUNCH(kernel, grid, block, lds, stream, ...)                                                    \
  do {                                                                                                       \
    if (g_prof_e0)                                                                                           \
      hipExtLaunchKernelGGL(kernel, grid, block, lds, stream, g_prof_e0, g_prof_e1, 0, __VA_ARGS__);         \
    else                                                                                                     \
      hipLaunchKernelGGL(kernel, grid, block, lds, stream, __VA_ARGS__);                                     \
  } while (0)

extern "C" int ca_prof_begin(void) {
  g_prof.clear();
  g_prof_on = true;
  return CA_OK;
}
extern "C" int ca_prof_end(double* ms, int64_t* count, double* flops) {
  g_prof_on = false;
  for (int v = 0; v < 24; ++v) {
    ms[v] = 0.0;
    count[v] = 0;
    flops[v] = 0.0;
  }
  for (auto& r : g_prof) {
    float t = 0.f;
    if (hipEventSynchronize(r.e1) != hipSuccess || hipEventElapsedTime(&t, r.e0, r.e1) != hipSuccess) {
      ca_set_error("ca_prof_end: event query failed");
      return CA_ERR_LAUNCH;
    }
    ms[r.variant] += t;
    count[r.variant] += 1;
    flops[r.variant] += r.flops;
    hipEventDestroy(r.e0);
    hipEventDestroy(r.e1);
  }
  g_prof.clear();
  return CA_OK;
}

extern "C" int ca_gemm_debug_general_epilogue(int on) {
  const int v = on ? 1 : 0;
  if (hipMemcpyToSymbol(HIP_SYMBOL(g_ca_epi_general), &v, sizeof(int)) != hipSuccess) {
    ca_set_error("ca_gemm_debug_general_epilogue: hipMemcpyToSymbol failed");
    return CA_ERR_LAUNCH;
  }
  return CA_OK;
}
static int g_compute_cus = 0;
extern "C" int ca_gemm_set_compute_cus(int n) {
  g_compute_cus = n > 0 ? n : 0;
  return CA_OK;
}
extern "C" int ca_background_update_fits(int32_t* regs) {
  hipFuncAttributes ax, aw;
  const hipError_t e1 = hipFuncGetAttributes(&ax, (const void*)ca_gemm_kernel_x<0, 0, false>);
  const hipError_t e2 = hipFuncGetAttributes(&aw, ca_adamw_background_kernel());
  if (e1 != hipSuccess || e2 != hipSuccess) {
    ca_set_error("ca_background_update_fits: hipFuncGetAttributes: %s", hipGetErrorString(e1 != hipSuccess ? e1 : e2));
    return CA_ERR_LAUNCH;
  }
  if (regs) {
    regs[0] = ax.numRegs;
    regs[1] = aw.numRegs;
  }
  const int gx = (ax.numRegs + 7) / 8 * 8, gw = (aw.numRegs + 7) / 8 * 8;
  return 2 * gx + gw <= 512 ? 1 : 0;
}
static unsigned x_device_cus() {
  static const unsigned ncu = [] {
    int dev = 0, n = 256;
    if (hipGetDevice(&dev) == hipSuccess) hipDeviceGetAttribute(&n, hipDeviceAttributeMultiprocessorCount, dev);
    return (unsigned)(n >= 8 ? (n / 8) * 8 : 8);
  }();
  return ncu;
}
static int g_force_kernel = 0;
extern "C" int ca_gemm_force_kernel(int which) {
  g_force_kernel = which;
  return CA_OK;
}
static GemmKnobs gemm_knobs() {
  static const GemmKnobs env = [] {
    GemmKnobs k;
    const auto read = [](const char* name, int& v) { if (const char* e = getenv(name)) v = atoi(e); };
    read("CA_X_PERSIST", k.x_persist);
    read("CA_SKINNY_MB1", k.skinny_mb1);
    read("CA_SKINNY_MB1_ROWS", k.skinny_mb1_rows);
    read("CA_SKINNY_NT", k.skinny_nt);
    read("CA_SKINNY_U", k.skinny_u);
    read("CA_GEMM_PREFER_L", k.prefer_l);
    read("CA_GEMM_L_OVER_X", k.l_over_x);
    read("CA_GEMM_L_MIN", k.l_min);
    read("CA_GEMM_M", k.m_max);
    return k;
  }();
  GemmKnobs k = env;
  k.force_kernel = g_force_kernel;
  k.compute_cus = g_compute_cus;
  k.device_cus = x_device_cus();
  return k;
}
static int ca_gemm_launch(const CaGemmDesc* desc, void* stream);
static int g_last_kind = 0;

extern "C" int ca_gemm_bf16(const CaGemmDesc* desc, void* stream) {
  if (!g_prof_on || desc == nullptr) return ca_gemm_launch(desc, stream);
  ProfRec r;
  hipEventCreate(&r.e0);
  hipEventCreate(&r.e1);
  r.flops = 2.0 * desc->M * (double)desc->N * desc->K * desc->batch1 * desc->batch2;
  g_prof_e0 = r.e0;
  g_prof_e1 = r.e1;
  const int rc = ca_gemm_launch(desc, stream);
  g_prof_e0 = g_prof_e1 = nullptr;
  r.variant = g_last_kind * 8 + ((desc->a_kseg > 0 || desc->b_kseg > 0) ? 4 : 0) + (desc->a_layout ? 2 : 0) +
              (desc->b_layout ? 1 : 0);
  g_prof.push_back(r);
  return rc;
}

typedef __attribute__((ext_vector_type(8))) int fp8x32_t;
typedef __attribute__((ext_vector_type(4))) int i32x4_t;
__global__ __launch_bounds__(256) void ca_gemm_fp8_kernel(const CaGemmDesc d) {
  extern __shared__ __attribute__((aligned(16))) char smem[];
  const int tid = threadIdx.x;
  const int lane = tid & 63;
  const int wave = __builtin_amdgcn_readfirstlane(tid >> 6);
  const int wm = wave >> 1, wn = wave & 1;
  int tm, tn;
  if (!tile_of_block<8, 8>(blockIdx.x, (d.M + BM - 1) / BM, (d.N + BN - 1) / BN, tm, tn)) return;
  const int m0 = tm * BM, n0 = tn * BN;
  KMajorStream<4> la, lb;
  la.init_bytes((const char*)d.A, d.lda, m0, d.M, wave, lane);
  lb.init_bytes((const char*)d.B, d.ldb, n0, d.N, wave, lane);
  f32x4_t acc[4][4];
#pragma unroll
  for (int i = 0; i < 4; ++i)
#pragma unroll
    for (int j = 0; j < 4; ++j) acc[i][j] = (f32x4_t){0.f, 0.f, 0.f, 0.f};
  const int K = d.K;
  constexpr int FBK = 128;
  const int nk = (K + FBK - 1) / FBK;
  auto burst = [&](int kt) {
    if (kt >= nk) return;
    char* na = smem + (kt & 1) * TILE_BYTES;
    char* nb = na + 2 * TILE_BYTES;
    const bool full = (kt + 1) * FBK <= K;
    if (full) {
#pragma unroll
      for (int part = 0; part < 4; ++part) {
        la.issue_one(na, wave, part);
        lb.issue_one(nb, wave, part);
      }
    } else {
#pragma unroll
      for (int part = 0; part < 4; ++part) {
        la.issue_one_tail(na, wave, K - kt * FBK, part);
        lb.issue_one_tail(nb, wave, K - kt * FBK, part);
      }
    }
    la.advance();
    lb.advance();
  };
  auto zero_tail = [&](int kt) {
    if (kt != nk - 1 || nk * FBK == K) return;
    char* na = smem + (kt & 1) * TILE_BYTES;
    la.zero_fix(na, wave, lane, K - kt * FBK);
    lb.zero_fix(na + 2 * TILE_BYTES, wave, lane, K - kt * FBK);
    asm volatile("s_waitcnt lgkmcnt(0)" ::: "memory");
  };
  const uint32_t lds0 = (uint32_t)(uintptr_t)(lptr_t)smem;
  const int g = lane >> 4;
  uint32_t abase[2], bbase[2];
  {
    const int ra = wm * 64 + (lane & 15), rb = wn * 64 + (lane & 15);
#pragma unroll
    for (int h = 0; h < 2; ++h) {
      abase[h] = lds0 + ra * 128 + (((2 * g + h) ^ ((ra >> 1) & 7)) * 16);
      bbase[h] = lds0 + 2 * TILE_BYTES + rb * 128 + (((2 * g + h) ^ ((rb >> 1) & 7)) * 16);
    }
  }
  burst(0);
  auto kstep = [&](auto st_c, int kt) {
    constexpr int ST = decltype(st_c)::value;
    asm volatile("s_waitcnt vmcnt(0) lgkmcnt(0)" ::: "memory");
    zero_tail(kt);
    __builtin_amdgcn_s_barrier();
    asm volatile("" ::: "memory");
    burst(kt + 1);
    bf16x8_t al[4], ah[4], bl[4], bh[4];
#define F8_RD(dst, base, F) dst = lds_read_b128<ST * TILE_BYTES + (F) * 2048>(base)
    F8_RD(al[0], abase[0], 0); F8_RD(ah[0], abase[1], 0); F8_RD(al[1], abase[0], 1); F8_RD(ah[1], abase[1], 1);
    F8_RD(al[2], abase[0], 2); F8_RD(ah[2], abase[1], 2); F8_RD(al[3], abase[0], 3); F8_RD(ah[3], abase[1], 3);
    F8_RD(bl[0], bbase[0], 0); F8_RD(bh[0], bbase[1], 0); F8_RD(bl[1], bbase[0], 1); F8_RD(bh[1], bbase[1], 1);
    F8_RD(bl[2], bbase[0], 2); F8_RD(bh[2], bbase[1], 2); F8_RD(bl[3], bbase[0], 3); F8_RD(bh[3], bbase[1], 3);
#undef F8_RD
    lds_wait(al);
    lds_wait(ah);
    lds_wait(bl);
    lds_wait(bh);
    fp8x32_t af[4], bq[4];
#pragma unroll
    for (int i = 0; i < 4; ++i) {
      const i32x4_t a0 = __builtin_bit_cast(i32x4_t, al[i]), a1 = __builtin_bit_cast(i32x4_t, ah[i]);
      const i32x4_t b0 = __builtin_bit_cast(i32x4_t, bl[i]), b1 = __builtin_bit_cast(i32x4_t, bh[i]);
      af[i] = (fp8x32_t){a0[0], a0[1], a0[2], a0[3], a1[0], a1[1], a1[2], a1[3]};
      bq[i] = (fp8x32_t){b0[0], b0[1], b0[2], b0[3], b1[0], b1[1], b1[2], b1[3]};
    }
#pragma unroll
    for (int i = 0; i < 4; ++i)
#pragma unroll
      for (int j = 0; j < 4; ++j)
        acc[i][j] = __builtin_amdgcn_mfma_scale_f32_16x16x128_f8f6f4(bq[j], af[i], acc[i][j], 0, 0, 0, 0x7f7f7f7f, 0,
                                                                     0x7f7f7f7f);
  };
  for (int kt = 0; kt < nk; kt += 2) {
    kstep(std::integral_constant<int, 0>{}, kt);
    if (kt + 1 < nk) kstep(std::integral_constant<int, 1>{}, kt + 1);
  }
  asm volatile("s_waitcnt lgkmcnt(0)" ::: "memory");
  __builtin_amdgcn_s_barrier();
  asm volatile("" ::: "memory");
  CaGemmDesc dd = d;
  dd.alpha = d.alpha * (d.a_scale ? *d.a_scale : 1.f) * (d.b_scale ? *d.b_scale : 1.f);
  if (d.a_row_scale) {
#pragma unroll
    for (int i = 0; i < 4; ++i) {
      const int m = m0 + wm * 64 + i * 16 + (lane & 15);
      const float rs = d.a_row_scale[m < d.M ? m : d.M - 1];
#pragma unroll
      for (int j = 0; j < 4; ++j) acc[i][j] *= rs;
    }
  }
  gemm_epilogue(dd, acc, smem, wave, lane, m0 + wm * 64, n0 + wn * 64, 0, 0, 0);
}

__global__ __launch_bounds__(512) void ca_gemm_fp8_kernel_x(const CaGemmDesc d) {
  extern __shared__ __attribute__((aligned(16))) char smem[];
  const int tid = threadIdx.x;
  const int lane = tid & 63;
  const int wave = __builtin_amdgcn_readfirstlane(tid >> 6);
  const int wm = wave >> 2, wn = wave & 3;
  int tm, tn;
  if (!tile_of_block<4, 8>(blockIdx.x, (d.M + XBM - 1) / XBM, (d.N + XBN - 1) / XBN, tm, tn)) return;
  const int m0 = tm * XBM, n0 = tn * XBN;
  KMajorStream<4> la, lb;
  la.init_bytes((const char*)d.A, d.lda, m0, d.M, wave, lane);
  lb.init_bytes((const char*)d.B, d.ldb, n0, d.N, wave, lane);
  f32x4_t acc[8][4];
#pragma unroll
  for (int i = 0; i < 8; ++i)
#pragma unroll
    for (int j = 0; j < 4; ++j) acc[i][j] = (f32x4_t){0.f, 0.f, 0.f, 0.f};
  const int K = d.K;
  constexpr int FBK = 128;
  const int nk = (K + FBK - 1) / FBK;
  auto burst = [&](int kt) {
    if (kt >= nk) return;
    char* na = smem + (kt & 1) * XTILE;
    char* nb = na + 2 * XTILE;
    const bool full = (kt + 1) * FBK <= K;
    if (full) {
#pragma unroll
      for (int part = 0; part < 4; ++part) {
        la.issue_one(na, wave, part);
        lb.issue_one(nb, wave, part);
      }
    } else {
#pragma unroll
      for (int part = 0; part < 4; ++part) {
        la.issue_one_tail(na, wave, K - kt * FBK, part);
        lb.issue_one_tail(nb, wave, K - kt * FBK, part);
      }
    }
    la.advance();
    lb.advance();
  };
  auto zero_tail = [&](int kt) {
    if (kt != nk - 1 || nk * FBK == K) return;
    char* na = smem + (kt & 1) * XTILE;
    la.zero_fix(na, wave, lane, K - kt * FBK);
    lb.zero_fix(na + 2 * XTILE, wave, lane, K - kt * FBK);
    asm volatile("s_waitcnt lgkmcnt(0)" ::: "memory");
  };
  const uint32_t lds0 = (uint32_t)(uintptr_t)(lptr_t)smem;
  const int g = lane >> 4;
  uint32_t abase[2], bbase[2];
  {
    const int ra = wm * 128 + (lane & 15), rb = wn * 64 + (lane & 15);
#pragma unroll
    for (int h = 0; h < 2; ++h) {
      abase[h] = lds0 + ra * 128 + (((2 * g + h) ^ ((ra >> 1) & 7)) * 16);
      bbase[h] = lds0 + 2 * XTILE + rb * 128 + (((2 * g + h) ^ ((rb >> 1) & 7)) * 16);
    }
  }
  bf16x8_t A0[4][2], A1[4][2], Bq[4][2];
#define F8X_RD_A(ST, F, dst)                                        \
  do {                                                              \
    dst[0] = lds_read_b128<(ST) * XTILE + (F) * 2048>(abase[0]);    \
    dst[1] = lds_read_b128<(ST) * XTILE + (F) * 2048>(abase[1]);    \
  } while (0)
#define F8X_RD_B(ST, F, dst)                                        \
  do {                                                              \
    dst[0] = lds_read_b128<(ST) * XTILE + (F) * 2048>(bbase[0]);    \
    dst[1] = lds_read_b128<(ST) * XTILE + (F) * 2048>(bbase[1]);    \
  } while (0)
#define F8X_SB __builtin_amdgcn_sched_barrier(0)
  auto pack = [&](bf16x8_t (&f)[2]) {
    const i32x4_t lo = __builtin_bit_cast(i32x4_t, f[0]), hi = __builtin_bit_cast(i32x4_t, f[1]);
    return (fp8x32_t){lo[0], lo[1], lo[2], lo[3], hi[0], hi[1], hi[2], hi[3]};
  };
#define F8X_MM(IH, AF, I, J)                                                                                         \
  do {                                                                                                               \
    acc[(IH) * 4 + (I)][J] = __builtin_amdgcn_mfma_scale_f32_16x16x128_f8f6f4(pack(Bq[J]), pack(AF[I]),              \
                                                                             acc[(IH) * 4 + (I)][J], 0, 0, 0,       \
                                                                             0x7f7f7f7f, 0, 0x7f7f7f7f);             \
    F8X_SB;                                                                                                          \
  } while (0)
  auto wait2 = [&](bf16x8_t (&f)[4][2]) {
    asm volatile("s_waitcnt lgkmcnt(0)"
                 : "+v"(f[0][0]), "+v"(f[0][1]), "+v"(f[1][0]), "+v"(f[1][1]), "+v"(f[2][0]), "+v"(f[2][1]), "+v"(f[3][0]),
                   "+v"(f[3][1]));
  };
  auto kstep = [&](auto st_c, int kt) {
    constexpr int ST = decltype(st_c)::value;
    if (wave >= 4) burst(kt + 1);
    wait2(A0);
    wait2(Bq);
    F8X_SB;
    __builtin_amdgcn_s_setprio(1);
    F8X_MM(0, A0, 0, 0); F8X_MM(0, A0, 0, 1); F8X_RD_A(ST, 4, A1[0]); F8X_SB;
    F8X_MM(0, A0, 0, 2); F8X_MM(0, A0, 0, 3); F8X_RD_A(ST, 5, A1[1]); F8X_SB;
    F8X_MM(0, A0, 1, 0); F8X_MM(0, A0, 1, 1); F8X_RD_A(ST, 6, A1[2]); F8X_SB;
    F8X_MM(0, A0, 1, 2); F8X_MM(0, A0, 1, 3); F8X_RD_A(ST, 7, A1[3]); F8X_SB;
    F8X_MM(0, A0, 2, 0); F8X_MM(0, A0, 2, 1); F8X_MM(0, A0, 2, 2); F8X_MM(0, A0, 2, 3);
    F8X_MM(0, A0, 3, 0); F8X_MM(0, A0, 3, 1); F8X_MM(0, A0, 3, 2); F8X_MM(0, A0, 3, 3);
    __builtin_amdgcn_s_setprio(0);
    wait2(A1);
    asm volatile("s_waitcnt vmcnt(0)" ::: "memory");
    zero_tail(kt + 1);
    __builtin_amdgcn_s_barrier();
    asm volatile("" ::: "memory");
    if (wave < 4) burst(kt + 2);
    F8X_SB;
    __builtin_amdgcn_s_setprio(1);
    F8X_MM(1, A1, 0, 0); F8X_MM(1, A1, 1, 0); F8X_RD_A(1 - ST, 0, A0[0]); F8X_SB;
    F8X_MM(1, A1, 2, 0); F8X_MM(1, A1, 3, 0); F8X_RD_B(1 - ST, 0, Bq[0]); F8X_SB;
    F8X_MM(1, A1, 0, 1); F8X_MM(1, A1, 1, 1); F8X_RD_A(1 - ST, 1, A0[1]); F8X_SB;
    F8X_MM(1, A1, 2, 1); F8X_MM(1, A1, 3, 1); F8X_RD_B(1 - ST, 1, Bq[1]); F8X_SB;
    F8X_MM(1, A1, 0, 2); F8X_MM(1, A1, 1, 2); F8X_RD_A(1 - ST, 2, A0[2]); F8X_SB;
    F8X_MM(1, A1, 2, 2); F8X_MM(1, A1, 3, 2); F8X_RD_B(1 - ST, 2, Bq[2]); F8X_SB;
    F8X_MM(1, A1, 0, 3); F8X_MM(1, A1, 1, 3); F8X_RD_A(1 - ST, 3, A0[3]); F8X_SB;
    F8X_MM(1, A1, 2, 3); F8X_MM(1, A1, 3, 3); F8X_RD_B(1 - ST, 3, Bq[3]); F8X_SB;
    __builtin_amdgcn_s_setprio(0);
  };
  burst(0);
  asm volatile("s_waitcnt vmcnt(0) lgkmcnt(0)" ::: "memory");
  zero_tail(0);
  __builtin_amdgcn_s_barrier();
  asm volatile("" ::: "memory");
  F8X_RD_B(0, 0, Bq[0]); F8X_RD_B(0, 1, Bq[1]); F8X_RD_B(0, 2, Bq[2]); F8X_RD_B(0, 3, Bq[3]);
  F8X_RD_A(0, 0, A0[0]); F8X_RD_A(0, 1, A0[1]); F8X_RD_A(0, 2, A0[2]); F8X_RD_A(0, 3, A0[3]);
  if (wave < 4) burst(1);
  for (int kt = 0; kt < nk; kt += 2) {
    kstep(std::integral_constant<int, 0>{}, kt);
    if (kt + 1 < nk) kstep(std::integral_constant<int, 1>{}, kt + 1);
  }
#undef F8X_RD_A
#undef F8X_RD_B
#undef F8X_MM
#undef F8X_SB
  asm volatile("s_waitcnt lgkmcnt(0)" ::: "memory");
  __builtin_amdgcn_s_barrier();
  asm volatile("" ::: "memory");
  CaGemmDesc dd = d;
  dd.alpha = d.alpha * (d.a_scale ? *d.a_scale : 1.f) * (d.b_scale ? *d.b_scale : 1.f);
#pragma unroll
  for (int ih = 0; ih < 2; ++ih) {
    f32x4_t half[4][4];
#pragma unroll
    for (int i = 0; i < 4; ++i) {
      float rs = 1.f;
      if (d.a_row_scale) {
        const int m = m0 + wm * 128 + (ih * 4 + i) * 16 + (lane & 15);
        rs = d.a_row_scale[m < d.M ? m : d.M - 1];
      }
#pragma unroll
      for (int j = 0; j < 4; ++j) half[i][j] = acc[ih * 4 + i][j] * rs;
    }
    gemm_epilogue(dd, half, smem, wave, lane, m0 + wm * 128 + ih * 64, n0 + wn * 64, 0, 0, 0);
    asm volatile("s_waitcnt lgkmcnt(0)" ::: "memory");
  }
}

typedef void (*DescKernel)(const CaGemmDesc);
typedef void (*GroupKernel)(const CaGemmGroup);
#define LAY4(K) K<0, 0>, K<0, 1>, K<1, 0>, K<1, 1>
#define LAY4_KS(K, KS) K<0, 0, KS>, K<0, 1, KS>, K<1, 0, KS>, K<1, 1, KS>
static const DescKernel k_gemm_s[8] = {LAY4_KS(ca_gemm_kernel, false), LAY4_KS(ca_gemm_kernel, true)};
static const DescKernel k_gemm_m[4] = {LAY4(ca_gemm_kernel_m)};
static const DescKernel k_gemm_l[4] = {LAY4(ca_gemm_kernel_l)};
static const GroupKernel k_gemm_x[8] = {LAY4_KS(ca_gemm_kernel_x, false), LAY4_KS(ca_gemm_kernel_x, true)};
static const DescKernel k_gemm_fp8[2] = {ca_gemm_fp8_kernel, ca_gemm_fp8_kernel_x};
#undef LAY4_KS
#undef LAY4
struct SkinnyKernel {
  int mb, nch, u, nt;
  DescKernel fn;
};
#define SK(MB, NCH, U, NT) {MB, NCH, U, NT, ca_gemm_skinny_kernel<MB, NCH, U, NT>}
#define SK_NT(MB, NCH, U) SK(MB, NCH, U, 16), SK(MB, NCH, U, 8), SK(MB, NCH, U, 4)
static const SkinnyKernel k_gemm_skinny[] = {
    SK_NT(1, 0, 8), SK_NT(1, 0, 16), SK_NT(1, 0, 32), SK(2, 0, 8, 16),
    SK_NT(1, 2, 8), SK_NT(1, 3, 8),  SK_NT(1, 4, 8),  SK(2, 2, 8, 16), SK(2, 3, 8, 16), SK(2, 4, 8, 16)
};
#undef SK_NT
#undef SK

enum { LDS_FAM_M, LDS_FAM_L, LDS_FAM_X, LDS_FAM_SKINNY_LN, LDS_FAM_FP8_S, LDS_FAM_FP8_X, LDS_FAM_COUNT };
static bool g_lds_allowed[LDS_FAM_COUNT];
template <typename K>
static void allow_lds(int fam, const K* kernels, int n, size_t bytes) {
  if (g_lds_allowed[fam]) return;
  for (int i = 0; i < n; ++i) hipFuncSetAttribute((const void*)kernels[i], hipFuncAttributeMaxDynamicSharedMemorySize, (int)bytes);
  g_lds_allowed[fam] = true;
}

static int gemm_launch_skinny(const GemmPlan& p, const CaGemmDesc& d, hipStream_t s) {
  if (p.nch > 0 && !g_lds_allowed[LDS_FAM_SKINNY_LN]) {
    for (const SkinnyKernel& k : k_gemm_skinny)
      if (k.nch > 0) hipFuncSetAttribute((const void*)k.fn, hipFuncAttributeMaxDynamicSharedMemorySize, 160 * 1024);
    g_lds_allowed[LDS_FAM_SKINNY_LN] = true;
  }
  for (const SkinnyKernel& k : k_gemm_skinny)
    if (k.mb == p.mb && k.nch == p.nch && k.u == p.u && k.nt == p.nt) {
      CA_LAUNCH(k.fn, dim3(p.grid_x, p.grid_y), dim3(p.block), p.lds, s, d);
      return CA_OK;
    }
  ca_set_error("ca_gemm_bf16: no skinny kernel <%d, %d, %d, %d>", p.mb, p.nch, p.u, p.nt);
  return CA_ERR_UNSUPPORTED;
}
static void gemm_launch_x(const GemmPlan& p, CaGemmGroup& g, hipStream_t s) {
  static unsigned seq = 0;
  allow_lds(LDS_FAM_X, k_gemm_x, 8, p.lds);
  g.vgrid = (int)p.vgrid;
  g.cnt = nullptr;
  g.dyn_first = p.dyn_first;
  dim3 grid(p.vgrid, 1, p.grid_z);
  if (p.persistent) {
    unsigned* base = nullptr;
    if (hipGetSymbolAddress((void**)&base, HIP_SYMBOL(g_x_cnt)) == hipSuccess && base) {
      g.cnt = base + (size_t)(seq++ % X_CNT_SLOTS) * 8;
      grid.x = p.grid_x;
    }
  }
  CA_LAUNCH(k_gemm_x[p.lay + 4 * p.ks], grid, dim3(p.block), p.lds, s, g);
}
static int gemm_launch_plan(const GemmPlan& p, const CaGemmDesc& d, CaGemmGroup* grp, hipStream_t s, const char* who) {
  const dim3 grid(p.grid_x, p.grid_y, p.grid_z), block(p.block);
  if (p.fp8) {
    const int x = p.family == GEMM_X ? 1 : 0;
    allow_lds(x ? LDS_FAM_FP8_X : LDS_FAM_FP8_S, &k_gemm_fp8[x], 1, p.lds);
    CA_LAUNCH(k_gemm_fp8[x], grid, block, p.lds, s, d);
  } else if (p.family == GEMM_SKINNY) {
    const int rc = gemm_launch_skinny(p, d, s);
    if (rc != CA_OK) return rc;
  } else if (p.family == GEMM_X) {
    CaGemmGroup one;
    if (!grp) one.d[0] = d, one.count = 0, one.first[0] = 0, one.total = 0;
    gemm_launch_x(p, grp ? *grp : one, s);
  } else if (p.family == GEMM_L) {
    allow_lds(LDS_FAM_L, k_gemm_l, 4, p.lds);
    CA_LAUNCH(k_gemm_l[p.lay], grid, block, p.lds, s, d);
  } else if (p.family == GEMM_M) {
    allow_lds(LDS_FAM_M, k_gemm_m, 4, p.lds);
    CA_LAUNCH(k_gemm_m[p.lay], grid, block, p.lds, s, d);
  } else {
    CA_LAUNCH(k_gemm_s[p.lay + 4 * p.ks], grid, block, p.lds, s, d);
  }
  CA_CHECK_LAUNCH(who);
  return CA_OK;
}

static int gemm_validate_fp8(const CaGemmDesc& d) {
  CA_CHECK_ARG(d.A && d.B && (d.C || d.C2) && d.M > 0 && d.N > 0 && d.K > 0, "ca_gemm_fp8: bad argument");
  CA_CHECK_ARG(d.C8 == nullptr || ((d.epilogue == CA_EPI_GELU || d.epilogue == CA_EPI_DGELU) && d.c8_scale != nullptr && (d.ldc % 8) == 0 &&
                                   ((uintptr_t)d.C8 % 8) == 0),
               "ca_gemm_fp8: C8 needs CA_EPI_GELU / CA_EPI_DGELU, a scale and 8-byte aligned rows");
  CA_CHECK_ARG(d.a_layout == CA_KMAJOR && d.b_layout == CA_KMAJOR && d.batch1 == 1 && d.batch2 == 1 && d.a_kseg == 0 &&
                   d.b_kseg == 0 && !d.a_colsum && !d.c_row_index,
               "ca_gemm_fp8: K-major operands, un-batched, plain rows only");
  CA_CHECK_ARG((d.K % 16) == 0 && (d.lda % 16) == 0 && (d.ldb % 16) == 0 && ((uintptr_t)d.A % 16) == 0 &&
                   ((uintptr_t)d.B % 16) == 0,
               "ca_gemm_fp8: K, lda, ldb must be multiples of 16 bytes and the operands 16-byte aligned");
  return CA_OK;
}
extern "C" int ca_gemm_fp8(const CaGemmDesc* desc, void* stream) {
  CA_CHECK_ARG(desc != nullptr, "ca_gemm_fp8: null descriptor");
  const int rc = gemm_validate_fp8(*desc);
  if (rc != CA_OK) return rc;
  return gemm_launch_plan(gemm_plan_fp8(*desc, gemm_knobs()), *desc, nullptr, (hipStream_t)stream, "ca_gemm_fp8");
}

static int gemm_validate_group(const CaGemmDesc* descs, int32_t count) {
  CA_CHECK_ARG(descs && count >= 1 && count <= X_GROUP_MAX, "ca_gemm_bf16_group: 1..8 problems");
  for (int i = 0; i < count; ++i) {
    const CaGemmDesc* p = descs + i;
    CA_CHECK_ARG(p->A && p->B && p->C && p->M > 0 && p->N > 0 && p->K >= 64, "ca_gemm_bf16_group: bad problem %d", i);
    CA_CHECK_ARG(p->batch1 == 1 && p->batch2 == 1 && p->a_kseg == 0 && p->b_kseg == 0 && p->epilogue == CA_EPI_NONE &&
                     p->bias == nullptr && p->dropout_p == 0.f,
                 "ca_gemm_bf16_group: only plain un-batched problems");
    CA_CHECK_ARG((p->lda % 8) == 0 && (p->ldb % 8) == 0 && ((uintptr_t)p->A % 16) == 0 && ((uintptr_t)p->B % 16) == 0,
                 "ca_gemm_bf16_group: alignment");
    CA_CHECK_ARG(p->a_layout == descs->a_layout && p->b_layout == descs->b_layout,
                 "ca_gemm_bf16_group: the problems differ in operand form");
    CA_CHECK_ARG(p->c_sumsq == nullptr || p->epilogue == CA_EPI_NONE, "ca_gemm_bf16_group: c_sumsq needs a plain epilogue");
  }
  return CA_OK;
}
extern "C" int ca_gemm_bf16_group(const CaGemmDesc* descs, int32_t count, void* stream) {
  const int rc = gemm_validate_group(descs, count);
  if (rc != CA_OK) return rc;
  CaGemmGroup g;
  int total = 0;
  for (int i = 0; i < X_GROUP_MAX; ++i) {
    g.d[i] = descs[i < count ? i : 0];
    g.first[i] = total;
    if (i < count) total += gemm_x_tiles(descs[i]);
  }
  g.total = total;
  g.count = count > 1 ? count : 0;
  const GemmPlan p = gemm_plan_group(descs, count, gemm_knobs());
  ProfRec r;
  if (g_prof_on) {
    hipEventCreate(&r.e0);
    hipEventCreate(&r.e1);
    r.flops = 0.0;
    for (int i = 0; i < count; ++i) r.flops += 2.0 * descs[i].M * (double)descs[i].N * descs[i].K;
    r.variant = p.kind * 8 + p.lay;
    g_prof_e0 = r.e0;
    g_prof_e1 = r.e1;
  }
  const int lrc = gemm_launch_plan(p, descs[0], &g, (hipStream_t)stream, "ca_gemm_bf16_group");
  if (g_prof_on) {
    g_prof_e0 = g_prof_e1 = nullptr;
    g_prof.push_back(r);
  }
  return lrc;
}

static int gemm_validate_bf16(const CaGemmDesc& d) {
  CA_CHECK_ARG(d.A && d.B &&
                   (d.C || ((d.epilogue == CA_EPI_GELU || d.epilogue == CA_EPI_GELU_RESIDUAL) && d.C2)),
               "ca_gemm_bf16: null operand");
  CA_CHECK_ARG(d.M > 0 && d.N > 0 && d.K > 0, "ca_gemm_bf16: bad shape %d %d %d", d.M, d.N,
               d.K);
  CA_CHECK_ARG(d.batch1 > 0 && d.batch2 > 0, "ca_gemm_bf16: bad batch");
  CA_CHECK_ARG((d.lda % 8) == 0 && (d.ldb % 8) == 0, "ca_gemm_bf16: lda/ldb must be multiples of 8");
  CA_CHECK_ARG((d.sA1 % 8) == 0 && (d.sA2 % 8) == 0 && (d.sB1 % 8) == 0 && (d.sB2 % 8) == 0,
               "ca_gemm_bf16: batch strides must be multiples of 8");
  CA_CHECK_ARG(((uintptr_t)d.A % 16) == 0 && ((uintptr_t)d.B % 16) == 0,
               "ca_gemm_bf16: A/B must be 16-byte aligned");
  CA_CHECK_ARG(d.a_kseg >= 0 && d.b_kseg >= 0, "ca_gemm_bf16: negative kseg");
  if (d.epilogue == CA_EPI_RESIDUAL || d.epilogue == CA_EPI_DGELU || d.epilogue == CA_EPI_GELU_RESIDUAL)
    CA_CHECK_ARG(d.R != nullptr, "ca_gemm_bf16: epilogue needs R");
  CA_CHECK_ARG(d.dropout_p >= 0.f && d.dropout_p < 1.f, "ca_gemm_bf16: bad dropout_p");
  CA_CHECK_ARG(d.C8 == nullptr || ((d.epilogue == CA_EPI_GELU || d.epilogue == CA_EPI_DGELU) && d.c8_scale != nullptr && d.batch1 == 1 && d.batch2 == 1 &&
                                   (d.ldc % 8) == 0 && ((uintptr_t)d.C8 % 8) == 0 && d.M > 32),
               "ca_gemm_bf16: C8 needs CA_EPI_GELU / CA_EPI_DGELU, a scale, an un-batched problem and 8-byte aligned rows");
  if (d.a_colsum)
    CA_CHECK_ARG(d.a_layout == CA_MNMAJOR && d.b_layout == CA_MNMAJOR && d.batch1 == 1 && d.batch2 == 1 && d.a_kseg == 0,
                 "ca_gemm_bf16: a_colsum needs the un-batched weight-gradient form");
  if (d.c_sumsq)
    CA_CHECK_ARG(d.epilogue == CA_EPI_NONE && d.batch1 == 1 && d.batch2 == 1 && d.c_row_index == nullptr && d.c_split_n == 0,
                 "ca_gemm_bf16: c_sumsq needs an un-batched output with the plain epilogue");
  CA_CHECK_ARG(d.a_layout == CA_KMAJOR || d.a_layout == CA_MNMAJOR, "ca_gemm_bf16: bad a_layout");
  CA_CHECK_ARG(d.b_layout == CA_KMAJOR || d.b_layout == CA_MNMAJOR, "ca_gemm_bf16: bad b_layout");
  return CA_OK;
}
static int gemm_validate_skinny(const CaGemmDesc& d) {
  CA_CHECK_ARG(d.c_split_n == 0 || (d.C_hi && (d.c_split_n % 16) == 0 && d.c_split_n < d.N && d.epilogue == CA_EPI_NONE),
               "ca_gemm_bf16: c_split_n needs C_hi, a multiple of 16 below N and no epilogue");
  if (d.a_ln_gamma)
    CA_CHECK_ARG(d.a_ln_beta && d.K <= 2048 && ((uintptr_t)d.a_ln_gamma % 16) == 0 && ((uintptr_t)d.a_ln_beta % 16) == 0,
                 "ca_gemm_bf16: a_ln_gamma needs a_ln_beta, K <= 2048 and 16-byte aligned vectors");
  return CA_OK;
}

static int ca_gemm_launch(const CaGemmDesc* desc, void* stream) {
  CA_CHECK_ARG(desc != nullptr, "ca_gemm_bf16: null descriptor");
  const GemmKnobs knobs = gemm_knobs();
  CaGemmDesc d = *desc;
  d.xcd_balanced = knobs.compute_cus > 0 ? 1 : 0;
  int rc = gemm_validate_bf16(d);
  if (rc != CA_OK) return rc;
  const GemmPlan p = gemm_plan_bf16(d, knobs);
  CA_CHECK_ARG(p.error != GEMM_PLAN_LN_NOT_SKINNY,
               "ca_gemm_bf16: a_ln_gamma exists in the skinny form only (M <= 128, K-major operands, un-batched)");
  CA_CHECK_ARG(p.error != GEMM_PLAN_ROWS_NOT_SKINNY,
               "ca_gemm_bf16: c_row_index / c_split_n exist in the skinny form only (M <= 128, K-major operands, un-batched)");
  g_last_kind = p.kind;
  if (p.family == GEMM_SKINNY && (rc = gemm_validate_skinny(d)) != CA_OK) return rc;
  return gemm_launch_plan(p, d, nullptr, (hipStream_t)stream, "ca_gemm_bf16");
}
```

### coral_amd/csrc/gemm_plan.h

```cpp
#pragma once
#include <stddef.h>
#include <stdint.h>
#include "../../include/coral_amd.h"

#if defined(__HIPCC__)
#define CA_PLAN_FN __host__ __device__ __forceinline__
#else
#define CA_PLAN_FN inline
#endif

#define BM 128
#define BN 128
#define BK 64
#define LBM 256
#define LBN 128
#define XBM 256
#define XBN 256
#define EPI_PITCH 68
#define LDS_BYTES (4 * 64 * EPI_PITCH * 4)
#define M_LDS_BYTES (2 * 4 * BM * BK * 2)
#define L_LDS_BYTES (3 * (LBM + LBN) * BK * 2)
#define X_LDS_BYTES (8 * 64 * EPI_PITCH * 4)
#define X_LAUNCH_LDS (X_LDS_BYTES + 64)
#define SKINNY_LN_PAD 32

CA_PLAN_FN int xcd_split(int ntm, int ntn, int& hb, int& wb) {
  int best = 1, cost = 1 << 30;
#pragma unroll
  for (int bm = 1; bm <= 8; bm *= 2) {
    const int bn = 8 / bm;
    const int c = (ntm + bm - 1) / bm + (ntn + bn - 1) / bn;
    if (c < cost) {
      cost = c;
      best = bm;
    }
  }
  hb = (ntm + best - 1) / best;
  wb = (ntn + 8 / best - 1) / (8 / best);
  return best;
}
CA_PLAN_FN void run_tile(int l, int ntm, int ntn, int& tm, int& tn) {
  if (ntn <= ntm) {
    tm = l / ntn;
    tn = l % ntn;
  } else {
    tn = l / ntm;
    tm = l % ntm;
  }
}
CA_PLAN_FN bool xcd_use_runs(int ntm, int ntn, int hb, int wb, bool bal = false) {
  return bal || 8 * hb * wb * 4 > ntm * ntn * 5;
}
CA_PLAN_FN int xcd_grid(int ntm, int ntn, bool bal = false) {
  if (ntm * ntn <= 8) return ntm * ntn;
  int hb, wb;
  xcd_split(ntm, ntn, hb, wb);
  if (xcd_use_runs(ntm, ntn, hb, wb, bal)) return 8 * ((ntm * ntn + 7) / 8);
  return 8 * hb * wb;
}
CA_PLAN_FN bool xcd_tile(int bid, int ntm, int ntn, int& tm, int& tn, bool bal = false) {
  if (ntm * ntn <= 8) {
    tm = bid / ntn;
    tn = bid % ntn;
    return true;
  }
  int hb, wb;
  const int bm = xcd_split(ntm, ntn, hb, wb);
  const int bn = 8 / bm;
  const int x = bid & 7, idx = bid >> 3;
  if (xcd_use_runs(ntm, ntn, hb, wb, bal)) {
    const int l = x * ((ntm * ntn + 7) / 8) + idx;
    run_tile(l, ntm, ntn, tm, tn);
    return l < ntm * ntn;
  }
  const int bi = x / bn, bj = x % bn;
  tm = bi * hb + idx / wb;
  tn = bj * wb + idx % wb;
  return tm < ntm && tn < ntn;
}
template <int SBM, int SBN>
CA_PLAN_FN bool tile_of_block_g(int bid, int grid, int ntm, int ntn, int& tm, int& tn, bool bal = false) {
  if (grid == xcd_grid(ntm, ntn, bal)) {
    return xcd_tile(bid, ntm, ntn, tm, tn, bal);
  }
  const int x = bid & 7, i = bid >> 3;
  const int per = SBM * SBN;
  const int sb = (i / per) * 8 + x, t = i % per;
  const int nsbn = (ntn + SBN - 1) / SBN;
  const int sbm = sb / nsbn, sbn = sb % nsbn;
  tm = sbm * SBM + (t % SBM);
  tn = sbn * SBN + (t / SBM);
  return tm < ntm && tn < ntn;
}
template <int SBM, int SBN>
CA_PLAN_FN unsigned tile_grid(int ntm, int ntn, bool bal = false) {
  if (ntm * ntn < 4 * 8 * SBM * SBN) return (unsigned)xcd_grid(ntm, ntn, bal);
  const int nsb = ((ntm + SBM - 1) / SBM) * ((ntn + SBN - 1) / SBN);
  return (unsigned)(((nsb + 7) / 8) * 8 * SBM * SBN);
}

struct GemmKnobs {
  int x_persist = 1;
  int skinny_mb1 = 4;
  int skinny_mb1_rows = 16;
  int skinny_nt = 0;
  int skinny_u = 0;
  int prefer_l = 3;
  int l_over_x = 0;
  int l_min = 100;
  int m_max = 256;
  int force_kernel = 0;
  int compute_cus = 0;
  unsigned device_cus = 256;
};
inline unsigned gemm_compute_cus(const GemmKnobs& k) {
  if (k.compute_cus <= 0) return k.device_cus;
  const unsigned c = (unsigned)(k.compute_cus >= 8 ? (k.compute_cus / 8) * 8 : 8);
  return c < k.device_cus ? c : k.device_cus;
}

enum GemmFamily { GEMM_SKINNY = 0, GEMM_S = 1, GEMM_M = 2, GEMM_L = 3, GEMM_X = 4 };
enum GemmPlanError { GEMM_PLAN_OK = 0, GEMM_PLAN_LN_NOT_SKINNY = 1, GEMM_PLAN_ROWS_NOT_SKINNY = 2 };
struct GemmPlan {
  int error = GEMM_PLAN_OK;
  int family = GEMM_S;
  int fp8 = 0;
  int lay = 0;
  int ks = 0;
  int mb = 0, nch = 0, u = 0, nt = 0;
  unsigned grid_x = 1, grid_y = 1, grid_z = 1, block = 256;
  size_t lds = 0;
  unsigned vgrid = 0;
  int persistent = 0, dyn_first = 0;
  int kind = 0;
};
inline int gemm_x_tiles(const CaGemmDesc& d) { return ((d.M + XBM - 1) / XBM) * ((d.N + XBN - 1) / XBN); }

inline void gemm_plan_x_geometry(GemmPlan& p, unsigned vgrid, unsigned nbz, const GemmKnobs& k) {
  const unsigned ncu = gemm_compute_cus(k);
  p.family = GEMM_X;
  p.kind = 2;
  p.vgrid = vgrid;
  p.dyn_first = k.compute_cus > 0 ? 1 : 0;
  p.persistent = (k.x_persist && nbz == 1 && vgrid > ncu) ? 1 : 0;
  p.grid_x = p.persistent ? ncu : vgrid;
  p.grid_z = nbz;
  p.block = 512;
  p.lds = X_LAUNCH_LDS;
}

inline bool gemm_takes_skinny(const CaGemmDesc& d, const GemmKnobs& k) {
  const bool skinny_wide = d.M > 32 && d.M <= 128 && d.C8 == nullptr && d.c_sumsq == nullptr &&
                           (d.a_ln_gamma || d.c_row_index || d.c_split_n > 0 || d.N <= 8192 || d.M <= 64);
  return k.force_kernel == 0 && (d.M <= 32 || skinny_wide) && d.a_layout == CA_KMAJOR && d.b_layout == CA_KMAJOR &&
         d.batch1 == 1 && d.batch2 == 1 && d.a_kseg == 0 && d.b_kseg == 0 && d.dropout_p == 0.f &&
         d.epilogue != CA_EPI_DGELU;
}
inline void gemm_plan_skinny(GemmPlan& p, const CaGemmDesc& d, const GemmKnobs& k) {
  p.family = GEMM_SKINNY;
  p.kind = 0;
  unsigned gy = d.M <= 32 ? 1u : (unsigned)((d.M + 31) / 32);
  const bool rows16 = k.skinny_mb1 && d.M > k.skinny_mb1_rows && d.M > 16 &&
                      (unsigned)((d.N + 15) / 16) * gy <= (unsigned)k.skinny_mb1 * k.device_cus;
  if (rows16) gy = (unsigned)((d.M + 15) / 16);
  int nt = 16;
  if (d.M <= 16 || rows16) {
    const unsigned want = 3u * k.device_cus / 4u;
    if ((unsigned)((d.N + 15) / 16) * gy < want) nt = (unsigned)((d.N + 7) / 8) * gy >= want ? 8 : 4;
    if (k.skinny_nt == 4 || k.skinny_nt == 8 || k.skinny_nt == 16) nt = k.skinny_nt;
  }
  p.grid_x = (unsigned)((d.N + nt - 1) / nt);
  p.grid_y = gy;
  p.block = 256;
  p.mb = (d.M <= 16 || rows16) ? 1 : 2;
  p.nt = nt;
  p.u = 8;
  if (d.a_ln_gamma) {
    p.nch = (d.K + 511) / 512 <= 2 ? 2 : (d.K + 511) / 512;
    p.lds = (size_t)4 * p.mb * 256 * sizeof(float) + (size_t)16 * p.mb * (d.K + SKINNY_LN_PAD) * 2;
    return;
  }
  p.lds = (size_t)4 * p.mb * 256 * sizeof(float);
  if (p.mb == 1) {
    const int per = ((d.K + 31) / 32 + 3) / 4;
    p.u = per <= 8 ? 8 : (per <= 16 ? 16 : 32);
    if (k.skinny_u == 8 || k.skinny_u == 16 || k.skinny_u == 32) p.u = k.skinny_u;
  }
}

inline int gemm_tiled_family(const CaGemmDesc& d, const GemmKnobs& k) {
  const int force = k.force_kernel;
  const int lay = (d.a_layout ? 2 : 0) + (d.b_layout ? 1 : 0);
  const bool ks = d.a_kseg > 0 || d.b_kseg > 0;
  const int64_t nb = (int64_t)d.batch1 * d.batch2;
  const int64_t tiles_l = (int64_t)((d.M + LBM - 1) / LBM) * ((d.N + LBN - 1) / LBN) * nb;
  bool use_l = force == 2 && !ks;
  const int xtm = (d.M + XBM - 1) / XBM, xtn = (d.N + XBN - 1) / XBN;
  const int64_t xt = (int64_t)xtm * xtn * nb;
  const int64_t cus = (int64_t)gemm_compute_cus(k);
  const double xwaves = (double)xt / (double)cus;
  const double xeff = xwaves / (double)((xt + cus - 1) / cus);
  const double xfill = ((double)d.M * d.N) / ((double)xtm * XBM * (double)xtn * XBN);
  const bool tn = d.a_layout == CA_MNMAJOR && d.b_layout == CA_MNMAJOR;
  bool use_x = force == 0 && d.K >= 512 && xt >= 160 && xeff * xfill >= (tn ? 0.60 : 0.70);
  if (force == 3 || d.a_colsum) use_x = true;
  const int lox = k.l_over_x;
  if (k.prefer_l && force == 0 && !ks && d.K >= 512 && tiles_l >= k.l_min &&
      (tiles_l <= cus * k.prefer_l || (use_x && lox)) && !d.a_colsum &&
      (!use_x || (lox == 1 && !tn) || lox == 2 || (lox == 3 && lay == 0))) {
    use_l = true;
    use_x = false;
  }
  const int ntm = (d.M + BM - 1) / BM, ntn = (d.N + BN - 1) / BN;
  const int64_t ts = (int64_t)ntm * ntn;
  if (force == 0 && k.compute_cus > 0 && cus < (int64_t)k.device_cus && nb == 1 && !ks && d.K >= 512 && !d.a_colsum &&
      d.M > 128) {
    auto rounds = [](int64_t tiles, int64_t slots) { return (double)((tiles + slots - 1) / slots); };
    const double cx = rounds(xt, cus) * 4.0, cl = rounds(tiles_l, cus) * 2.0 / (tn ? 0.85 : 0.93),
                 cs = rounds(ts, 2 * cus) * 2.0 / (tn ? 0.6 : 0.8), cm = rounds(ts, cus) * 1.0 / 0.6;
    int family = GEMM_X;
    double best = cx;
    if (cl < best) { best = cl; family = GEMM_L; }
    if (cs < best) { best = cs; family = GEMM_S; }
    if (cm < best) { best = cm; family = GEMM_M; }
    return family;
  }
  if (use_x) return GEMM_X;
  if (use_l) return GEMM_L;
  if (!ks && (force == 5 || (force == 0 && ts * nb <= k.m_max && d.K >= 2 * BK))) return GEMM_M;
  return GEMM_S;
}

inline GemmPlan gemm_plan_bf16(const CaGemmDesc& d, const GemmKnobs& k) {
  GemmPlan p;
  p.lay = (d.a_layout ? 2 : 0) + (d.b_layout ? 1 : 0);
  p.ks = (d.a_kseg > 0 || d.b_kseg > 0) ? 1 : 0;
  if (gemm_takes_skinny(d, k)) {
    gemm_plan_skinny(p, d, k);
    return p;
  }
  if (d.a_ln_gamma) p.error = GEMM_PLAN_LN_NOT_SKINNY;
  else if (d.c_row_index || d.c_split_n != 0) p.error = GEMM_PLAN_ROWS_NOT_SKINNY;
  if (p.error) return p;
  const bool bal = k.compute_cus > 0;
  const unsigned nb = (unsigned)((int64_t)d.batch1 * d.batch2);
  p.family = gemm_tiled_family(d, k);
  p.grid_z = nb;
  switch (p.family) {
    case GEMM_X:
      gemm_plan_x_geometry(p, tile_grid<4, 8>((d.M + XBM - 1) / XBM, (d.N + XBN - 1) / XBN, bal), nb, k);
      break;
    case GEMM_L:
      p.kind = 1;
      p.grid_x = tile_grid<4, 8>((d.M + LBM - 1) / LBM, (d.N + LBN - 1) / LBN, bal);
      p.block = 512;
      p.lds = L_LDS_BYTES;
      break;
    default:
      p.kind = 0;
      p.grid_x = tile_grid<8, 8>((d.M + BM - 1) / BM, (d.N + BN - 1) / BN, bal);
      p.block = p.family == GEMM_M ? 512 : 256;
      p.lds = p.family == GEMM_M ? M_LDS_BYTES : LDS_BYTES;
      break;
  }
  return p;
}

inline GemmPlan gemm_plan_fp8(const CaGemmDesc& d, const GemmKnobs& k) {
  GemmPlan p;
  p.fp8 = 1;
  p.kind = -1;
  const int xtm = (d.M + XBM - 1) / XBM, xtn = (d.N + XBN - 1) / XBN;
  const int64_t xt = (int64_t)xtm * xtn;
  const double xeff = ((double)xt / 256.0) / (double)((xt + 255) / 256);
  const double xfill = ((double)d.M * d.N) / ((double)xtm * XBM * (double)xtn * XBN);
  if (k.force_kernel == 3 || (k.force_kernel == 0 && d.K >= 512 && xt >= 160 && xeff * xfill >= 0.70)) {
    p.family = GEMM_X;
    p.grid_x = tile_grid<4, 8>(xtm, xtn);
    p.block = 512;
    p.lds = X_LDS_BYTES;
  } else {
    p.family = GEMM_S;
    p.grid_x = tile_grid<8, 8>((d.M + BM - 1) / BM, (d.N + BN - 1) / BN);
    p.block = 256;
    p.lds = LDS_BYTES;
  }
  return p;
}

inline GemmPlan gemm_plan_group(const CaGemmDesc* descs, int count, const GemmKnobs& k) {
  GemmPlan p;
  p.lay = (descs->a_layout ? 2 : 0) + (descs->b_layout ? 1 : 0);
  int total = 0;
  for (int i = 0; i < count; ++i) total += gemm_x_tiles(descs[i]);
  const unsigned vgrid = count > 1 ? (unsigned)(8 * ((total + 7) / 8))
                                   : tile_grid<4, 8>((descs->M + XBM - 1) / XBM, (descs->N + XBN - 1) / XBN);
  gemm_plan_x_geometry(p, vgrid, 1, k);
  return p;
}
```

### coral_amd/ops.py

```python

from __future__ import annotations

import ctypes as C
import os

import torch

from . import _lib
from ._lib import (CaAttnDesc, EPI_DGELU, EPI_GELU, EPI_GELU_RESIDUAL, EPI_NONE, EPI_RESIDUAL, KMAJOR,
                   MNMAJOR, CaGemmDesc, CoralAmdError, check)

__all__ = ["KMAJOR", "MNMAJOR", "EPI_NONE", "EPI_GELU", "EPI_RESIDUAL", "EPI_DGELU",
           "EPI_GELU_RESIDUAL", "CoralAmdError"]

_ELT = {torch.bfloat16: 2, torch.float32: 4, torch.int32: 4, torch.uint8: 1, torch.int64: 8, torch.int16: 2,
        torch.uint32: 4}


def _stream() -> int:
    return torch.cuda.current_stream().cuda_stream


def _p(t: torch.Tensor | None, off: int = 0) -> int | None:
    if t is None:
        return None
    if not t.is_cuda:
        raise CoralAmdError("coral_amd ops need device tensors (there is no CPU path)")
    return t.data_ptr() + off * _ELT[t.dtype]


def lib():
    return _lib.load()


_SIDE_STREAMS: dict = {}


def background_update_fits():
    regs = (C.c_int32 * 2)()
    rc = lib().ca_background_update_fits(regs)
    if rc < 0:
        check(rc, "ca_background_update_fits")
    return bool(rc), int(regs[0]), int(regs[1])


def side_stream(device, role: str, priority: int = 0):
    dev = torch.device(device)
    if os.environ.get("CA_SHARED_STREAMS", "1") == "0":
        return torch.cuda.Stream(device=dev, priority=priority)
    key = (dev.index if dev.index is not None else torch.cuda.current_device(), role, priority)
    st = _SIDE_STREAMS.get(key)
    if st is None:
        st = _SIDE_STREAMS[key] = torch.cuda.Stream(device=dev, priority=priority)
    return st


def _gemm_desc(A, B, Cout, *, M, N, K, lda, ldb, ldc, a_layout=KMAJOR, b_layout=KMAJOR, a_off=0,
         b_off=0, c_off=0, bias=None, bias_off=0, R=None, r_off=0, ldr=0, C2=None, c2_off=None,
         epilogue=EPI_NONE, out_f32=None, accumulate=False, alpha=1.0, batch1=1, batch2=1,
         sA=(0, 0), sB=(0, 0), sC=(0, 0), sR=(0, 0), sBias=(0, 0), a_kseg=0, a_kseg_stride=0, b_kseg=0,
         b_kseg_stride=0, dropout_p=0.0, dropout_seed=0, a_colsum=None, a_colsum_off=0,
         a_colsum_ld=0, c_row_index=None, c_row_mul=0, c_split_n=0, C_hi=None, c_hi_off=0, ldc_hi=0,
         c_sumsq=None, c_sumsq_off=0, stream_out=False, C8=None, c8_scale=None, c8_amax=None, a_ln=None):
    d = CaGemmDesc()
    if a_ln is not None:
        d.a_ln_gamma, d.a_ln_beta, d.a_ln_eps = _p(a_ln[0]), _p(a_ln[1]), float(a_ln[2])
    d.c_stream_out = int(stream_out)
    if C8 is not None:
        d.C8, d.c8_scale, d.c8_amax = _p(C8), _p(c8_scale), _p(c8_amax)
    if c_sumsq is not None:
        d.c_sumsq = _p(c_sumsq, c_sumsq_off)
    if c_split_n:
        d.c_split_n, d.C_hi, d.ldc_hi = c_split_n, _p(C_hi, c_hi_off), ldc_hi
    if c_row_index is not None:
        d.c_row_index, d.c_row_mul = _p(c_row_index), c_row_mul
    if a_colsum is not None:
        d.a_colsum = _p(a_colsum, a_colsum_off)
        d.a_colsum_ld = a_colsum_ld
    d.A, d.B = _p(A, a_off), _p(B, b_off)
    d.C = _p(Cout, c_off) if Cout is not None else None
    if C2 is not None:
        d.C2 = _p(C2, c_off if c2_off is None else c2_off)
    if R is not None:
        d.R = _p(R, r_off)
    if bias is not None:
        d.bias = _p(bias, bias_off)
    d.M, d.N, d.K = M, N, K
    d.a_layout, d.b_layout = a_layout, b_layout
    d.lda, d.ldb, d.ldc, d.ldr = lda, ldb, ldc, ldr
    d.a_kseg, d.b_kseg = a_kseg, b_kseg
    d.a_kseg_stride, d.b_kseg_stride = a_kseg_stride, b_kseg_stride
    d.batch1, d.batch2 = batch1, batch2
    d.sA1, d.sA2 = sA
    d.sB1, d.sB2 = sB
    d.sC1, d.sC2 = sC
    d.sR1, d.sR2 = sR
    d.sBias1, d.sBias2 = sBias
    d.epilogue = epilogue
    ref_out = Cout if Cout is not None else C2
    d.out_f32 = int(ref_out.dtype == torch.float32) if out_f32 is None else int(out_f32)
    d.accumulate = int(accumulate)
    d.alpha = alpha
    d.dropout_p = dropout_p
    d.dropout_seed = dropout_seed
    return d


def gemm(A, B, Cout, **kw):
    d = _gemm_desc(A, B, Cout, **kw)
    check(lib().ca_gemm_bf16(C.byref(d), _stream()), "ca_gemm_bf16")


_SPLITK_WS: dict = {}
FUSE_BIAS_GRAD = os.environ.get("CA_FUSE_BIAS", "1") == "1"
FUSE_BIAS_PARTIAL_MIN_K = int(os.environ.get("CA_FUSE_BIAS_PARTIAL_MIN_K", "8192"))


def gemm_fp8(A8, B8, Cout, *, a_scale=None, b_scale=None, a_row_scale=None, **kw):
    d = _gemm_desc(A8, B8, Cout, **kw)
    d.a_scale, d.b_scale, d.a_row_scale = _p(a_scale), _p(b_scale), _p(a_row_scale)
    check(lib().ca_gemm_fp8(C.byref(d), _stream()), "ca_gemm_fp8")


FP8_AMAX_SLOTS = 64


def quantize_fp8_delayed(x, q, scale, amax_next, n=None):
    check(lib().ca_quantize_fp8_delayed(_p(x), x.numel() if n is None else n, _p(q), _p(scale), _p(amax_next), _stream()),
          "ca_quantize_fp8_delayed")


def fp8_amax_rotate(amax_next, scale, inv_scale, count, margin=1.0):
    check(lib().ca_fp8_amax_rotate(_p(amax_next), _p(scale), _p(inv_scale), count, float(margin), _stream()), "ca_fp8_amax_rotate")


def dropout_rows_fp8(x, y, q, row_scale, rows, Cn, p, seed):
    check(lib().ca_dropout_rows_fp8(_p(x), _p(y), _p(q), _p(row_scale), rows, Cn, float(p), int(seed), _stream()),
          "ca_dropout_rows_fp8")


def quantize_fp8_transposed(x, rows, cols, qt, scale, x_off=0, qt_off=0):
    check(lib().ca_quantize_fp8_transposed(_p(x, x_off), rows, cols, _p(qt, qt_off), _p(scale), _stream()),
          "ca_quantize_fp8_transposed")


def fp8_refresh_group(tasks):
    for i in range(0, len(tasks), _lib.FP8_GROUP_MAX):
        part = tasks[i:i + _lib.FP8_GROUP_MAX]
        arr = (_lib.CaFp8RefreshTask * len(part))()
        for t, (x, x_off, rows, cols, q, q_off, qt, qt_off, scale, amax) in zip(arr, part):
            t.x_bf16, t.q_fp8, t.q_fp8_t = _p(x, x_off), _p(q, q_off), _p(qt, qt_off)
            t.scale, t.amax_next, t.rows, t.cols = _p(scale), _p(amax), rows, cols
        check(lib().ca_fp8_refresh_group(arr, len(part), _stream()), "ca_fp8_refresh_group")


def quantize_fp8(x, q, inv_scale, amax_ws, n=None):
    check(lib().ca_quantize_fp8(_p(x), x.numel() if n is None else n, _p(q), _p(inv_scale), _p(amax_ws), _stream()),
          "ca_quantize_fp8")


COLSUM_PARTS = 8
STREAM_U = os.environ.get("CA_STREAM_U", "1") == "1"
STREAM_WGRAD = os.environ.get("CA_STREAM_WGRAD", "1") == "1"


def _wgrad_splits(M, N, K):
    tiles = ((M + 127) // 128) * ((N + 127) // 128)
    xt = ((M + 255) // 256) * ((N + 255) // 256)
    if xt < 160 and tiles <= 256:
        for s in (8, 4, 2):
            if tiles * s <= 512 and K % s == 0 and K // s >= 256:
                return s
    return 1


def sumsq_slots(M, N):
    return ((M + 63) // 64) * ((N + 63) // 64)


def wgrad_gemm(dY, X, G, *, M, N, K, lda, ldb, c_off, accumulate, a_off=0, b_off=0, bias_off=None, part=None,
               cs=None, sq=None, Gb=None):
    splits = 1 if cs is not None else _wgrad_splits(M, N, K)
    g16 = G.dtype == torch.bfloat16
    if g16 and accumulate:
        raise CoralAmdError("wgrad_gemm: a bf16 gradient buffer is written, never accumulated into")
    if bias_off is not None:
        colsum(dY, lda, K, M, Gb if g16 else G, part, x_off=a_off, out_off=bias_off)
    if splits == 1:
        kw = dict(a_colsum=cs[0], a_colsum_off=cs[1], a_colsum_ld=cs[2]) if cs is not None else {}
        if sq is not None:
            kw.update(c_sumsq=sq[0], c_sumsq_off=sq[1])
        gemm(dY, X, G, M=M, N=N, K=K, a_layout=MNMAJOR, lda=lda, b_layout=MNMAJOR, ldb=ldb, ldc=N, c_off=c_off,
             a_off=a_off, b_off=b_off, out_f32=not g16, accumulate=accumulate, stream_out=STREAM_WGRAD, **kw)
        return
    ws = _SPLITK_WS.get(G.device)
    need = max(splits * M * N, M * N + 4096)
    if ws is None or ws.numel() < need:
        ws = torch.empty(need, dtype=torch.float32, device=G.device)
        _SPLITK_WS[G.device] = ws
    Kc = K // splits
    gemm(dY, X, ws, M=M, N=N, K=Kc, a_layout=MNMAJOR, lda=lda, b_layout=MNMAJOR, ldb=ldb, ldc=N, a_off=a_off,
         b_off=b_off, out_f32=True, batch2=splits, sA=(0, Kc * lda), sB=(0, Kc * ldb), sC=(0, M * N))
    if g16:
        reduce_rows(ws, splits, M * N, M * N, ws, accumulate=False)
        cast_f32_bf16(ws, G, M * N, y_off=c_off)
        if sq is not None:
            cast_bf16_f32(G[c_off:], ws, M * N)
            sumsq(ws, M * N, sq[0][sq[1]:], ws[M * N:])
    else:
        reduce_rows(ws, splits, M * N, M * N, G[c_off:], accumulate=accumulate)
        if sq is not None:
            sumsq(G[c_off:], M * N, sq[0][sq[1]:], ws)
    if sq is not None:
        ns = sumsq_slots(M, N)
        if ns > 1:
            clear_f32(sq[0], ns - 1, off=sq[1] + 1)


def _xtiles(p):
    return ((p["M"] + 255) // 256) * ((p["N"] + 255) // 256)


def _fill(t):
    return t / (256.0 * ((t + 255) // 256))


GROUP_MAX = 8


_PLAN_CACHE: dict = {}
_CS_DIRTY: dict = {}


def _wgrad_plan_idx(shapes: tuple):
    import itertools

    xt = [((m + 255) // 256) * ((n + 255) // 256) for m, n, _ in shapes]
    big = [i for i, (_, _, k) in enumerate(shapes) if _fill(xt[i]) >= 0.85 and k >= 512]
    rest = [i for i in range(len(shapes)) if i not in big and shapes[i][2] >= 512]
    small_k = [i for i in range(len(shapes)) if i not in big and shapes[i][2] < 512]
    groups = []
    if 1 < len(rest) <= GROUP_MAX and _fill(sum(xt[i] for i in rest)) >= 0.6:
        groups.append(list(rest))
        rest = []
    while len(rest) > 1:
        best, best_fill = None, 0.0
        for r in range(min(GROUP_MAX, len(rest)), 1, -1):
            for combo in itertools.combinations(rest, r):
                total = sum(xt[i] for i in combo)
                alone = sum(xt[i] / _fill(xt[i]) for i in combo)
                f = _fill(total)
                if f >= 0.7 and total / f < 0.9 * alone and (f > best_fill + 1e-9 or (abs(f - best_fill) < 1e-9 and best is not None
                                                                                 and len(combo) > len(best))):
                    best, best_fill = combo, f
        if best is None:
            break
        groups.append(list(best))
        rest = [i for i in rest if i not in best]
    return big, groups, rest + small_k


def wgrad_plan(problems: list):
    key = tuple((p["M"], p["N"], p["K"]) for p in problems)
    plan = _PLAN_CACHE.get(key)
    if plan is None:
# ... 558 lines not shown
```

### include/coral_amd.h

```cpp
#ifndef CORAL_AMD_H
#define CORAL_AMD_H

#include <stdint.h>

#ifdef __cplusplus
extern "C" {
#endif

#define CA_OK 0
#define CA_ERR_ARG (-1)
#define CA_ERR_LAUNCH (-2)
#define CA_ERR_UNSUPPORTED (-3)

int ca_version(void);
const char* ca_last_error(void);
int ca_device_count(void);

#define CA_KMAJOR 0
#define CA_MNMAJOR 1

#define CA_EPI_NONE 0
#define CA_EPI_GELU 1
#define CA_EPI_RESIDUAL 2
#define CA_EPI_DGELU 3
#define CA_EPI_GELU_RESIDUAL 4

typedef struct CaGemmDesc {
  const void* A;
  const void* B;
  void* C;
  void* C2;
  const void* R;
  const float* bias;
  int32_t M, N, K;
  int32_t a_layout, b_layout;
  int64_t lda, ldb, ldc, ldr;
  int32_t a_kseg, b_kseg;
  int64_t a_kseg_stride, b_kseg_stride;
  int32_t batch1, batch2;
  int64_t sA1, sA2, sB1, sB2, sC1, sC2, sR1, sR2;
  int64_t sBias1, sBias2;
  int32_t epilogue;
  int32_t out_f32;
  int32_t accumulate;
  float alpha;
  float dropout_p;
  uint64_t dropout_seed;
  float* a_colsum;
  int64_t a_colsum_ld;
  const int32_t* c_row_index;
  int64_t c_row_mul;
  int32_t c_split_n;
  void* C_hi;
  int64_t ldc_hi;
  const float* a_scale;
  const float* b_scale;
  const float* a_row_scale;
  float* c_sumsq;
  int32_t c_stream_out;
  void* C8;
  const float* c8_scale;
  uint32_t* c8_amax;
  const float* a_ln_gamma;
  const float* a_ln_beta;
  float a_ln_eps;
  int32_t xcd_balanced;
} CaGemmDesc;

int ca_gemm_bf16(const CaGemmDesc* desc, void* stream);
int ca_gemm_fp8(const CaGemmDesc* desc, void* stream);
int ca_quantize_fp8(const void* x_bf16, int64_t n, void* q_fp8, float* inv_scale, float* amax_ws, void* stream);
#define CA_FP8_AMAX_SLOTS 64
int ca_quantize_fp8_delayed(const void* x_bf16, int64_t n, void* q_fp8, const float* scale, uint32_t* amax_next,
                            void* stream);
int ca_fp8_amax_rotate(uint32_t* amax_next, float* scale, float* inv_scale, int32_t count, float margin, void* stream);
int ca_dropout_rows_fp8(const void* x, void* y, void* q_fp8, float* row_scale, int64_t rows, int32_t C, float p,
                        uint64_t seed, void* stream);
int ca_quantize_fp8_transposed(const void* x_bf16, int32_t rows, int32_t cols, void* q_fp8_t, const float* scale,
                               void* stream);
#define CA_FP8_GROUP_MAX 8
typedef struct CaFp8RefreshTask {
  const void* x_bf16;
  void* q_fp8;
  void* q_fp8_t;
  const float* scale;
  uint32_t* amax_next;
  int32_t rows, cols;
} CaFp8RefreshTask;
int ca_fp8_refresh_group(const CaFp8RefreshTask* tasks, int32_t count, void* stream);
int ca_gemm_bf16_group(const CaGemmDesc* descs, int32_t count, void* stream);

int ca_prof_begin(void);
int ca_prof_end(double* ms, int64_t* count, double* flops);

int ca_gemm_force_kernel(int which);
int ca_gemm_debug_general_epilogue(int on);
int ca_debug_cu_hog(int32_t blocks, int32_t threads, int32_t lds_bytes, double ms, void* stream);

int ca_gemm_set_compute_cus(int n);

int ca_layernorm_fwd(const void* x, const float* gamma, const float* beta, void* y,
                     float* stats, int64_t rows, int32_t C, float eps, int32_t act,
                     void* stream);
int ca_layernorm_fwd_ex(const void* x, const float* gamma, const float* beta, void* y,
                        float* stats, int64_t rows, int32_t C, float eps, int32_t act,
                        int32_t x_f32, int32_t y_f32, void* stream);
int ca_layernorm_fwd_fp8(const void* x, const float* gamma, const float* beta, void* y, void* q_fp8,
                         float* row_scale, float* stats, int64_t rows, int32_t C, float eps, void* stream);
int64_t ca_layernorm_bwd_partial_floats(int64_t rows, int32_t C);
int ca_layernorm_bwd(const void* dy, const void* x, const float* gamma, const float* beta,
                     const float* stats, const void* dres, void* dx, float* dgamma,
                     float* dbeta, float* partial, int64_t rows, int32_t C, int32_t act,
                     void* stream);

int ca_layernorm_bwd_ex(const void* dy, const void* x, const float* gamma, const float* beta,
                        const float* stats, const void* dres, void* dx, float* dgamma,
                        float* dbeta, float* partial, int64_t rows, int32_t C, int32_t act,
                        int32_t x_f32, void* stream);

int ca_layernorm_bwd_dropout(const void* dy, const void* x, const float* gamma, const float* beta,
                             const float* stats, const void* dres, void* dx, void* dx_drop, float p, uint64_t seed,
                             float* dgamma, float* dbeta, float* partial, int64_t rows, int32_t C, int32_t x_f32,
                             void* stream);

int64_t ca_colsum_partial_floats(int64_t rows, int32_t N);
int ca_colsum_bf16(const void* x, int64_t ld, int64_t rows, int32_t N, const uint8_t* rowmask,
                   float* out, int32_t accumulate, float* partial, void* stream);
int ca_reduce_rows_f32(const float* partial, int32_t nparts, int64_t stride, int32_t n, float* out,
                       int32_t accumulate, void* stream);
#define CA_REDUCE_MAX 4
typedef struct CaReduceDesc {
  const float* partial;
  float* out;
  int64_t stride;
  int32_t nparts, n, accumulate;
} CaReduceDesc;
int ca_reduce_rows_multi(const CaReduceDesc* descs, int32_t count, void* stream);
int ca_dgelu_mul(const void* dy, const void* u, void* out, int64_t n, void* stream);
int ca_dropout_bf16(const void* x, void* y, int64_t n, float p, uint64_t seed, void* stream);

int ca_wave_normalize(const float* x, const int32_t* lengths, float* y, int32_t B,
                      int64_t N, float eps, void* stream);

int ca_frame_lengths(const int32_t* attention_mask, int32_t B, int64_t N, const int32_t* kernels,
                     const int32_t* strides, int32_t nconv, int32_t* out, void* stream);
int ca_pcm_prepare(const void* pcm, int32_t is_int16, int64_t ld_in, const int32_t* lengths, float* y,
                   int32_t* mask, int32_t B, int64_t N, int32_t peak_normalize, int32_t zero_mean_unit_var,
                   float eps, void* stream);
int ca_wave_scale(const float* x, const float* scale, float* y, int32_t B, int64_t N, void* stream);
int ca_fir_filter(const float* x, const int32_t* lengths, const float* taps, const int32_t* ntaps,
                  const int32_t* mode, int64_t ld_taps, int32_t max_taps, float* y, int32_t B, int64_t N,
                  void* stream);
int ca_mix_noise(const float* x, const int32_t* lengths, const float* noise, int64_t noise_ld, int64_t noise_len,
                 const int64_t* noise_off, const float* snr_db, const int32_t* active, float* y, int32_t B,
                 int64_t N, void* stream);
int ca_white_noise(float* out, int64_t n, uint64_t seed, void* stream);

int ca_conv0_ln_gelu_fwd(const float* x, const float* w, const float* bias,
                         const float* gamma, const float* beta, void* y, int32_t B,
                         int64_t N, int32_t C, int32_t k, int32_t stride, float eps,
                         void* stream);
int64_t ca_conv0_bwd_partial_floats(int32_t B, int64_t N, int32_t C, int32_t k,
                                    int32_t stride);
int ca_conv0_ln_gelu_bwd(const float* x, const float* w, const float* bias,
                         const float* gamma, const float* beta, const void* dy, float* dw,
                         float* dbias, float* dgamma, float* dbeta, float* partial,
                         int32_t B, int64_t N, int32_t C, int32_t k, int32_t stride,
                         float eps, void* stream);

int ca_col2im_1d(const void* dcol, void* dx, int32_t B, int64_t T, int64_t L, int32_t C,
                 int32_t k, int32_t stride, void* stream);

typedef struct CaAttnDesc {
  const void *Q, *K, *V;
  void* O;
  const void* dO;
  void *dQ, *dK, *dV;
  float* lse;
  float* Dq;
  const int32_t* klen;
  const int32_t* key_slot;
  int64_t ldq, ldk, ldv, ldo, lddo, lddq, lddk, lddv;
  int64_t sqb, skb, svb, sob, sdob, sdqb, sdkb, sdvb;
  int32_t B, H, Tq, Tk, hd, Tqp, causal;
  float scale;
  float dropout_p;
  uint64_t dropout_seed;
  void* O8;
  const float* o8_scale;
  uint32_t* o8_amax;
  void* split_ws;
  int64_t split_ws_bytes;
  const int32_t* row_off;
} CaAttnDesc;
#define CA_ATTN_SPLIT_MAX 4
#define CA_ATTN_SPLIT_WS_BYTES(B, H) \
  ((((int64_t)(B) * (H) * 4 + 255) / 256 * 256) + (int64_t)(B) * (H) * CA_ATTN_SPLIT_MAX * 16 * 66 * 4)
int ca_attn_fwd(const CaAttnDesc* desc, void* stream);
int ca_attn_bwd(const CaAttnDesc* desc, void* stream);
int ca_decode_attn_qproj(const CaAttnDesc* desc, const void* x, int64_t ldx, const float* ln_gamma,
                         const float* ln_beta, float ln_eps, const void* Wq, int64_t ldw, const float* bq,
                         int32_t d_model, void* stream);

#define CA_BEAM_MAX_BEAMS 16
#define CA_BEAM_MAX_ROWS 128
typedef struct CaBeamDesc {
  int32_t B, k, max_len, prompt_len, max_length, eos_id, early_stopping;
  const float* len_pen;
  const float* cand_score;
  const int32_t* cand_parent;
  const int32_t* cand_token;
  float* run_score;
  int32_t *tok, *pos, *klen;
  const int32_t* anc_in;
  int32_t* anc_out;
  const int32_t* ids_in;
  int32_t* ids_out;
  float* fin_score;
  int32_t *fin_len, *fin_seq;
  int32_t* fin_ids;
  int32_t* fin_count;
  int32_t* heur;
  uint8_t* done;
  int32_t *tr_parent, *tr_token;
  float* tr_score;
} CaBeamDesc;
int64_t ca_beam_select_workspace_bytes(int32_t B, int32_t k, int32_t V);
int ca_beam_select(const float* logits, int64_t ldv, const uint8_t* suppress, const float* run_score, int32_t B,
                   int32_t k, int32_t V, float* cand_score, int32_t* cand_parent, int32_t* cand_token, void* ws,
                   int64_t ws_bytes, void* stream);
int ca_beam_advance(const CaBeamDesc* desc, void* stream);

int64_t ca_ctc_workspace_bytes(int32_t B, int32_t T, int32_t Lmax);
int ca_ctc_loss_fwd_bwd(const float* logits, const int32_t* labels, const int32_t* in_len,
                        float* nll, float* grad, const float* gscale, void* ws, int32_t B,
                        int32_t T, int32_t V, int64_t ldv, int32_t Lmax, int32_t blank,
                        int32_t zero_infinity, void* stream);
int ca_ctc_greedy_decode(const float* logits, const int32_t* in_len, int32_t* raw,
                         int32_t* ids, int32_t* out_len, int32_t B, int32_t T, int32_t V,
                         int64_t ldv, int32_t blank, void* stream);

#define CA_CTC_COLLAPSE_TILE 4096
int ca_ctc_stitch(const float* logits, const int32_t* seg, int32_t* raw_out, float* logits_out, int32_t C, int32_t T,
                  int32_t V, int64_t ldv, int32_t R, int32_t Tout, void* stream);
int64_t ca_ctc_collapse_workspace_bytes(int32_t B, int32_t T);
int ca_ctc_collapse_offsets(const int32_t* raw, const int32_t* in_len, int32_t* ids, int32_t* start, int32_t* end,
                            int32_t* out_len, void* ws, int64_t ws_bytes, int32_t B, int32_t T, int32_t blank,
                            void* stream);

// ... 182 lines not shown
```

Baseline: 1127 audio-seconds/sec.

## Add 240-row tile variant of kernel X to balance waves across CUs

Adds a 240-row tile version of the large GEMM kernel. In this variant the waves of the second row half skip their last 16-row MFMA block and run a row-limited epilogue. A planner picks 240 rows when the tile count still fits in one wave of CUs and the padded rows per CU come out smaller than with 256-row tiles. It also adds an XCD-balanced tile mapping for the 240-row case. The aim is to cut tail-wave quantization on GEMMs whose M (8×499 frames ≈ 3992) fits badly into 256-row tiles. The cost is extra kernel instantiations and some idle MFMA slots in the skipped waves. It also adds register pressure checks for background AdamW co-residency.

```diff
diff --git a/coral_amd/_lib.py b/coral_amd/_lib.py
--- a/coral_amd/_lib.py
+++ b/coral_amd/_lib.py
@@ -176,6 +176,9 @@
     "ca_quantize_fp8_transposed": (C.c_int, [_vp, _i32, _i32, _vp, _vp, _vp]),
     "ca_fp8_refresh_group": (C.c_int, [_vp, _i32, _vp]),
     "ca_gemm_force_kernel": (C.c_int, [C.c_int]),
+    "ca_gemm_force_x_rows": (C.c_int, [C.c_int]),
+    "ca_gemm_x_rows": (C.c_int, [C.POINTER(CaGemmDesc), _i32, C.POINTER(C.c_int32)]),
+    "ca_gemm_x_counters_busy": (C.c_int, []),
     "ca_gemm_debug_general_epilogue": (C.c_int, [C.c_int]),
     "ca_debug_cu_hog": (C.c_int, [_i32, _i32, _i32, C.c_double, _vp]),
     "ca_gemm_set_compute_cus": (C.c_int, [C.c_int]),
diff --git a/coral_amd/csrc/gemm.hip b/coral_amd/csrc/gemm.hip
--- a/coral_amd/csrc/gemm.hip
+++ b/coral_amd/csrc/gemm.hip
@@ -273,7 +273,7 @@
 template <int EPI, bool F32, bool DROP>
 __device__ __forceinline__ void gemm_epilogue_fast(const CaGemmDesc& d, const float* wt, int lane, int mw, int nb, int z,
                                                    int64_t zoffC, int64_t zoffR, const float (&bias8)[8], float& ssq,
-                                                   float& amx) {
+                                                   float& amx, int npass = 8) {
   const int M = d.M, N = d.N;
   const float alpha = d.alpha;
   const float keep_scale = DROP ? 1.f / (1.f - d.dropout_p) : 1.f;
@@ -299,9 +299,9 @@
   }
   const unsigned int dgstep = (unsigned int)(istep >> 2);
 #pragma unroll 2
-  for (int it = 0; it < 8; ++it) {
+  for (int it = 0; it < npass; ++it) {
     const u16x8_t r_cur = r_next;
-    if (NEEDS_R && it < 7) r_next = *(const u16x8_t*)(Rp + (it + 1) * rstep);
+    if (NEEDS_R && it + 1 < npass) r_next = *(const u16x8_t*)(Rp + (it + 1) * rstep);
     const float* wr = wt + (it * 8 + r0) * EPI_PITCH + c0;
     const f32x4_t a4 = *(const f32x4_t*)wr, b4 = *(const f32x4_t*)(wr + 4);
     float v[8];
@@ -376,11 +376,12 @@
   }
 }
 
-template <bool PARKED = false>
+template <bool PARKED = false, bool ROWS = false>
 __device__ __forceinline__ void gemm_epilogue(const CaGemmDesc& d, f32x4_t (&acc)[4][4], char* smem,
                                               int wave, int lane, int mw, int nw, int z, int z1,
-                                              int z2, const float (*bias_pre)[8] = nullptr) {
+                                              int z2, const float (*bias_pre)[8] = nullptr, int nrows = 64) {
   const int M = d.M, N = d.N;
+  const int mend = ROWS ? (M < mw + nrows ? M : mw + nrows) : M;
   const int64_t zoffC = z1 * d.sC1 + z2 * d.sC2;
   const int64_t zoffR = z1 * d.sR1 + z2 * d.sR2;
   const bool vec_ok = ((d.ldc & 7) == 0) && ((zoffC & 7) == 0) && ((d.ldr & 7) == 0) && ((zoffR & 7) == 0);
@@ -401,7 +402,7 @@
   const unsigned short* Rbase = (const unsigned short*)d.R + zoffR + nb;
   auto load_r = [&](int it, u16x8_t& u) {
     const int m = mw + it * 8 + (lane >> 3);
-    if (needs_r && full && it < 8 && m < M) u = *(const u16x8_t*)(Rbase + (int64_t)m * d.ldr);
+    if (needs_r && full && it < 8 && m < mend) u = *(const u16x8_t*)(Rbase + (int64_t)m * d.ldr);
   };
   u16x8_t r_next = {0, 0, 0, 0, 0, 0, 0, 0};
   load_r(0, r_next);
@@ -409,10 +410,12 @@
   float* wt = (float*)smem + wave * (64 * EPI_PITCH);
   if (!PARKED) {
 #pragma unroll
-    for (int i = 0; i < 4; ++i)
+    for (int i = 0; i < 4; ++i) {
+      if (ROWS && i * 16 >= nrows) continue;
 #pragma unroll
       for (int j = 0; j < 4; ++j)
         *(f32x4_t*)(wt + (i * 16 + (lane & 15)) * EPI_PITCH + j * 16 + 4 * (lane >> 4)) = acc[i][j];
+    }
     asm volatile("s_waitcnt lgkmcnt(0)" ::: "memory");
   }
   const bool c8_on = d.C8 != nullptr && (epi == CA_EPI_GELU || epi == CA_EPI_DGELU);
@@ -422,11 +425,11 @@
   const float s8 = c8_on ? d.c8_scale[0] : 1.f;
   const bool drop_on = d.dropout_p > 0.f;
   const bool drop32_ok = !drop_on || ((((uint64_t)z * M + mw) * (uint64_t)N) >> 34) == ((((uint64_t)z * M + mw + 64) * (uint64_t)N) >> 34);
-  const bool interior = g_ca_epi_general == 0 && mw + 64 <= M && nw + 64 <= N && vec_ok && (N & 7) == 0 && d.C != nullptr && drop32_ok &&
+  const bool interior = g_ca_epi_general == 0 && mw + (ROWS ? nrows : 64) <= M && nw + 64 <= N && vec_ok && (N & 7) == 0 && d.C != nullptr && drop32_ok &&
                         (d.out_f32 || !d.accumulate) && (!has_gelu || (epi == CA_EPI_GELU && d.C2 != nullptr && !d.out_f32)) &&
                         !(d.out_f32 && epi != CA_EPI_NONE) && !(drop_on && epi == CA_EPI_NONE);
   if (interior) {
-#define EPI_FAST(E, F, D) gemm_epilogue_fast<E, F, D>(d, wt, lane, mw, nb, z, zoffC, zoffR, bias8, ssq, amx)
+#define EPI_FAST(E, F, D) gemm_epilogue_fast<E, F, D>(d, wt, lane, mw, nb, z, zoffC, zoffR, bias8, ssq, amx, ROWS ? nrows >> 3 : 8)
     if (d.out_f32) {
       EPI_FAST(CA_EPI_NONE, true, false);
     } else if (epi == CA_EPI_NONE) {
@@ -446,7 +449,7 @@
     const int m = mw + ml;
     const u16x8_t r_cur = r_next;
     load_r(it + 1, r_next);
-    if (m >= M || nvalid <= 0) continue;
+    if (m >= mend || nvalid <= 0) continue;
     const f32x4_t a4 = *(const f32x4_t*)(wt + ml * EPI_PITCH + 8 * (lane & 7));
     const f32x4_t b4 = *(const f32x4_t*)(wt + ml * EPI_PITCH + 8 * (lane & 7) + 4);
     float v[8], v2[8], r[8];
@@ -883,13 +886,17 @@
   return (int)hipMemcpyFromSymbol(host, HIP_SYMBOL(g_x_stamps), (size_t)n * sizeof(long long));
 }
 #endif
-template <int AL, int BL, bool KS>
+template <int AL, int BL, bool KS, int RM = XBM>
 __device__ __forceinline__ void gemm_x_body(const CaGemmGroup& grp) {
+  static_assert(RM == XBM || (RM == X_ROWS_240 && !KS), "kernel X: 256-row tiles, or 240-row ones without segmented K");
+  constexpr bool R240 = RM != XBM;
   extern __shared__ __attribute__((aligned(16))) char smem[];
   const int tid = threadIdx.x;
-  const int lane = tid & 63;
+  const int lane_wg = tid & 63;
+  int lane = lane_wg;
   const int wave = __builtin_amdgcn_readfirstlane(tid >> 6);
   const int wm = wave >> 2, wn = wave & 3;
+  const bool skip7 = R240 && wm == 1;
   const int vgrid = grp.vgrid;
   const int xcd = (int)blockIdx.x & 7;
   const int npx = ((int)gridDim.x - xcd + 7) >> 3;
@@ -935,12 +942,12 @@
   int tm = 0, tn = 0;
   if (live) {
     if (grp.count > 1)
-      run_tile(gt - grp.first[which], (d.M + XBM - 1) / XBM, (d.N + XBN - 1) / XBN, tm, tn);
+      run_tile(gt - grp.first[which], (d.M + RM - 1) / RM, (d.N + XBN - 1) / XBN, tm, tn);
     else
-      live = tile_of_block_g<4, 8>(vb, vgrid, (d.M + XBM - 1) / XBM, (d.N + XBN - 1) / XBN, tm, tn, d.xcd_balanced != 0);
+      live = tile_of_block_g<4, 8>(vb, vgrid, (d.M + RM - 1) / RM, (d.N + XBN - 1) / XBN, tm, tn, d.xcd_balanced != 0);
   }
   if (live) {
-  const int m0 = tm * XBM, n0 = tn * XBN;
+  const int m0 = tm * RM, n0 = tn * XBN;
   const int z = blockIdx.z;
   const int z1 = z / d.batch2, z2 = z % d.batch2;
   const __bf16* A = (const __bf16*)d.A + z1 * d.sA1 + z2 * d.sA2;
@@ -960,6 +967,10 @@
     else
       lb_f.init(B, d.ldb, col0, d.N, wave, lane);
   };
+  auto tile_body = [&](auto skip_c) {
+  constexpr bool SKIP7 = decltype(skip_c)::value;
+  int lane = lane_wg;
+  if constexpr (R240) asm volatile("" : "+v"(lane));
   init_loaders(m0, n0);
 
   f32x4_t acc[8][4];
@@ -1085,6 +1096,18 @@
         __builtin_amdgcn_mfma_f32_16x16x32_bf16(BF[(J) + 1], AF[I], acc[(IH) * 4 + (I)][(J) + 1], 0, 0, 0);       \
     X_SB;                                                                                                         \
   } while (0)
+#define X_MM2_B7(AF, BF, J)     \
+  do {                          \
+    if constexpr (!SKIP7) {     \
+      X_MM2(1, AF, BF, 3, J);   \
+    } else {                    \
+      X_SB;                     \
+    }                           \
+  } while (0)
+#define X_RD_A_B7(ST, SH, dst)                       \
+  do {                                               \
+    if constexpr (!SKIP7) X_RD_A(ST, SH, 7, dst);    \
+  } while (0)
   auto colsum_acc = [&](bool cs_step, int ih, bf16x8_t (&af)[4]) {
     if (AL == CA_MNMAJOR && cs_step) {
       f32x4_t z;
@@ -1123,7 +1146,7 @@
     X_MM2(0, A0, B0, 0, 0); X_RD_A(ST, 0, 4, A1[0]); X_SB;
     X_MM2(0, A0, B0, 0, 2); X_RD_A(ST, 0, 5, A1[1]); X_SB;
     X_MM2(0, A0, B0, 1, 0); X_RD_A(ST, 0, 6, A1[2]); X_SB;
-    X_MM2(0, A0, B0, 1, 2); X_RD_A(ST, 0, 7, A1[3]); X_SB;
+    X_MM2(0, A0, B0, 1, 2); X_RD_A_B7(ST, 0, A1[3]); X_SB;
     X_MM2(0, A0, B0, 2, 0);
     X_MM2(0, A0, B0, 2, 2);
     X_MM2(0, A0, B0, 3, 0);
@@ -1140,8 +1163,8 @@
     X_MM2(1, A1, B0, 1, 2); X_RD_B(ST, 1, 3, B1[3]); X_SB;
     X_MM2(1, A1, B0, 2, 0); X_RD_A(ST, 1, 0, A0[0]); X_SB;
     X_MM2(1, A1, B0, 2, 2); X_RD_A(ST, 1, 1, A0[1]); X_SB;
-    X_MM2(1, A1, B0, 3, 0); X_RD_A(ST, 1, 2, A0[2]); X_SB;
-    X_MM2(1, A1, B0, 3, 2); X_RD_A(ST, 1, 3, A0[3]); X_SB;
+    X_MM2_B7(A1, B0, 0); X_RD_A(ST, 1, 2, A0[2]); X_SB;
+    X_MM2_B7(A1, B0, 2); X_RD_A(ST, 1, 3, A0[3]); X_SB;
     __builtin_amdgcn_s_setprio(0);
     lds_wait(B1);
     lds_wait(A0);
@@ -1151,7 +1174,7 @@
     X_MM2(0, A0, B1, 0, 0); X_RD_A(ST, 1, 4, A1[0]); X_SB;
     X_MM2(0, A0, B1, 0, 2); X_RD_A(ST, 1, 5, A1[1]); X_SB;
     X_MM2(0, A0, B1, 1, 0); X_RD_A(ST, 1, 6, A1[2]); X_SB;
-    X_MM2(0, A0, B1, 1, 2); X_RD_A(ST, 1, 7, A1[3]); X_SB;
+    X_MM2(0, A0, B1, 1, 2); X_RD_A_B7(ST, 1, A1[3]); X_SB;
     X_MM2(0, A0, B1, 2, 0);
     X_MM2(0, A0, B1, 2, 2);
     X_MM2(0, A0, B1, 3, 0);
@@ -1183,8 +1206,8 @@
     X_MM2(1, A1, B1, 1, 2); X_RD_B(1 - ST, 0, 3, B0[3]); X_SB;
     X_MM2(1, A1, B1, 2, 0); X_RD_A(1 - ST, 0, 0, A0[0]); X_SB;
     X_MM2(1, A1, B1, 2, 2); X_RD_A(1 - ST, 0, 1, A0[1]); X_SB;
-    X_MM2(1, A1, B1, 3, 0); X_RD_A(1 - ST, 0, 2, A0[2]); X_SB;
-    X_MM2(1, A1, B1, 3, 2); X_RD_A(1 - ST, 0, 3, A0[3]); X_SB;
+    X_MM2_B7(A1, B1, 0); X_RD_A(1 - ST, 0, 2, A0[2]); X_SB;
+    X_MM2_B7(A1, B1, 2); X_RD_A(1 - ST, 0, 3, A0[3]); X_SB;
     __builtin_amdgcn_s_setprio(0);
   };
 #ifdef X_STAMPS
@@ -1207,6 +1230,8 @@
     kstep(std::integral_constant<int, 0>{}, kt);
     if (kt + 1 < nk) kstep(std::integral_constant<int, 1>{}, kt + 1);
   }
+#undef X_RD_A_B7
+#undef X_MM2_B7
 #undef X_RD_A
 #undef X_RD_B
 #undef X_MM2
@@ -1222,7 +1247,7 @@
       s += __shfl_xor(s, 16, 64);
       s += __shfl_xor(s, 32, 64);
       const int m = m0 + wm * 128 + (ih * 4 + wn) * 16 + (lane & 15);
-      if (lane < 16 && m < d.M) d.a_colsum[(int64_t)tn * d.a_colsum_ld + m] = s;
+      if (lane < 16 && m < d.M && (!R240 || m < m0 + RM)) d.a_colsum[(int64_t)tn * d.a_colsum_ld + m] = s;
     }
   }
   unsigned nxt = 0;
@@ -1238,7 +1263,11 @@
     for (int i = 0; i < 4; ++i)
 #pragma unroll
       for (int j = 0; j < 4; ++j) half[i][j] = acc[ih * 4 + i][j];
-    gemm_epilogue(d, half, smem, wave, lane, m0 + wm * 128 + ih * 64, n0 + wn * 64, z, z1, z2, KS ? nullptr : &xbias);
+    if constexpr (SKIP7)
+      gemm_epilogue<false, true>(d, half, smem, wave, lane, m0 + wm * 128 + ih * 64, n0 + wn * 64, z, z1, z2, &xbias,
+                                 ih == 1 ? 48 : 64);
+    else
+      gemm_epilogue(d, half, smem, wave, lane, m0 + wm * 128 + ih * 64, n0 + wn * 64, z, z1, z2, KS ? nullptr : &xbias);
     asm volatile("s_waitcnt lgkmcnt(0)" ::: "memory");
   }
   if (grp.cnt != nullptr) __syncthreads();
@@ -1258,6 +1287,15 @@
     }
   }
 #endif
+  };
+  if constexpr (R240) {
+    if (skip7)
+      tile_body(std::true_type{});
+    else
+      tile_body(std::false_type{});
+  } else {
+    tile_body(std::false_type{});
+  }
   }
   else if (grp.cnt != nullptr) {
     __syncthreads();
@@ -1277,6 +1315,16 @@
 __global__ __launch_bounds__(512) __attribute__((amdgpu_num_vgpr(112)))
 void ca_gemm_kernel_x<CA_KMAJOR, CA_KMAJOR, false>(const CaGemmGroup grp) {
   gemm_x_body<CA_KMAJOR, CA_KMAJOR, false>(grp);
+}
+
+template <int AL, int BL>
+__global__ __launch_bounds__(512) void ca_gemm_kernel_x240(const CaGemmGroup grp) {
+  gemm_x_body<AL, BL, false, X_ROWS_240>(grp);
+}
+template <>
+__global__ __launch_bounds__(512) __attribute__((amdgpu_num_vgpr(112)))
+void ca_gemm_kernel_x240<CA_KMAJOR, CA_KMAJOR>(const CaGemmGroup grp) {
+  gemm_x_body<CA_KMAJOR, CA_KMAJOR, false, X_ROWS_240>(grp);
 }
 
 #define LA_BYTES (LBM * BK * 2)
@@ -1742,17 +1790,21 @@
 }
 extern "C" int ca_background_update_fits(int32_t* regs) {
   hipFuncAttributes ax, aw;
+  hipFuncAttributes ax240;
   const hipError_t e1 = hipFuncGetAttributes(&ax, (const void*)ca_gemm_kernel_x<0, 0, false>);
   const hipError_t e2 = hipFuncGetAttributes(&aw, ca_adamw_background_kernel());
-  if (e1 != hipSuccess || e2 != hipSuccess) {
-    ca_set_error("ca_background_update_fits: hipFuncGetAttributes: %s", hipGetErrorString(e1 != hipSuccess ? e1 : e2));
+  const hipError_t e3 = hipFuncGetAttributes(&ax240, (const void*)ca_gemm_kernel_x240<0, 0>);
+  if (e1 != hipSuccess || e2 != hipSuccess || e3 != hipSuccess) {
+    ca_set_error("ca_background_update_fits: hipFuncGetAttributes: %s",
+                 hipGetErrorString(e1 != hipSuccess ? e1 : (e2 != hipSuccess ? e2 : e3)));
     return CA_ERR_LAUNCH;
   }
   if (regs) {
     regs[0] = ax.numRegs;
     regs[1] = aw.numRegs;
   }
-  const int gx = (ax.numRegs + 7) / 8 * 8, gw = (aw.numRegs + 7) / 8 * 8;
+  const int most = ax.numRegs > ax240.numRegs ? ax.numRegs : ax240.numRegs;
+  const int gx = (most + 7) / 8 * 8, gw = (aw.numRegs + 7) / 8 * 8;
   return 2 * gx + gw <= 512 ? 1 : 0;
 }
 static unsigned x_device_cus() {
@@ -1768,10 +1820,21 @@
   g_force_kernel = which;
   return CA_OK;
 }
+static int g_force_x_rows = 0;
+extern "C" int ca_gemm_force_x_rows(int rows) {
+  if (rows != 0 && rows != X_ROWS_240 && rows != XBM) {
+    ca_set_error("ca_gemm_force_x_rows: 0 (auto), 240 or 256, not %d", rows);
+    return CA_ERR_ARG;
+  }
+  g_force_x_rows = rows;
+  return CA_OK;
+}
 static GemmKnobs gemm_knobs() {
   static const GemmKnobs env = [] {
     GemmKnobs k;
     const auto read = [](const char* name, int& v) { if (const char* e = getenv(name)) v = atoi(e); };
+    k.x_rows240 = 1;
+    read("CA_X_ROWS240", k.x_rows240);
     read("CA_X_PERSIST", k.x_persist);
     read("CA_SKINNY_MB1", k.skinny_mb1);
     read("CA_SKINNY_MB1_ROWS", k.skinny_mb1_rows);
@@ -1785,9 +1848,33 @@
   }();
   GemmKnobs k = env;
   k.force_kernel = g_force_kernel;
+  k.force_x_rows = g_force_x_rows;
   k.compute_cus = g_compute_cus;
   k.device_cus = x_device_cus();
   return k;
+}
+extern "C" int ca_gemm_x_rows(const CaGemmDesc* descs, int32_t count, int32_t* tiles) {
+  if (descs == nullptr || count < 1 || count > 8) {
+    ca_set_error("ca_gemm_x_rows: 1..8 problems");
+    return -1;
+  }
+  const int rows = gemm_x_rows(descs, count, (int64_t)descs->batch1 * descs->batch2, gemm_knobs());
+  if (tiles) {
+    *tiles = 0;
+    for (int i = 0; i < count; ++i) *tiles += gemm_x_tiles(descs[i], rows);
+  }
+  return rows;
+}
+extern "C" int ca_gemm_x_counters_busy(void) {
+  static unsigned host[X_CNT_SLOTS][8];
+  if (hipDeviceSynchronize() != hipSuccess || hipMemcpyFromSymbol(host, HIP_SYMBOL(g_x_cnt), sizeof host) != hipSuccess) {
+    ca_set_error("ca_gemm_x_counters_busy: reading the counters failed");
+    return CA_ERR_LAUNCH;
+  }
+  int busy = 0;
+  for (int i = 0; i < X_CNT_SLOTS; ++i)
+    for (int x = 0; x < 8; ++x) busy += host[i][x] != 0u;
+  return busy;
 }
 static int ca_gemm_launch(const CaGemmDesc* desc, void* stream);
 static int g_last_kind = 0;
@@ -2090,6 +2177,7 @@
 static const DescKernel k_gemm_m[4] = {LAY4(ca_gemm_kernel_m)};
 static const DescKernel k_gemm_l[4] = {LAY4(ca_gemm_kernel_l)};
 static const GroupKernel k_gemm_x[8] = {LAY4_KS(ca_gemm_kernel_x, false), LAY4_KS(ca_gemm_kernel_x, true)};
+static const GroupKernel k_gemm_x240[4] = {LAY4(ca_gemm_kernel_x240)};
 static const DescKernel k_gemm_fp8[2] = {ca_gemm_fp8_kernel, ca_gemm_fp8_kernel_x};
 #undef LAY4_KS
 #undef LAY4
@@ -2106,7 +2194,7 @@
 #undef SK_NT
 #undef SK
 
-enum { LDS_FAM_M, LDS_FAM_L, LDS_FAM_X, LDS_FAM_SKINNY_LN, LDS_FAM_FP8_S, LDS_FAM_FP8_X, LDS_FAM_COUNT };
+enum { LDS_FAM_M, LDS_FAM_L, LDS_FAM_X, LDS_FAM_X240, LDS_FAM_SKINNY_LN, LDS_FAM_FP8_S, LDS_FAM_FP8_X, LDS_FAM_COUNT };
 static bool g_lds_allowed[LDS_FAM_COUNT];
 template <typename K>
 static void allow_lds(int fam, const K* kernels, int n, size_t bytes) {
@@ -2131,7 +2219,11 @@
 }
 static void gemm_launch_x(const GemmPlan& p, CaGemmGroup& g, hipStream_t s) {
   static unsigned seq = 0;
-  allow_lds(LDS_FAM_X, k_gemm_x, 8, p.lds);
+  const bool r240 = p.xrows == X_ROWS_240 && !p.ks;
+  if (r240)
+    allow_lds(LDS_FAM_X240, k_gemm_x240, 4, p.lds);
+  else
+    allow_lds(LDS_FAM_X, k_gemm_x, 8, p.lds);
   g.vgrid = (int)p.vgrid;
   g.cnt = nullptr;
   g.dyn_first = p.dyn_first;
@@ -2143,7 +2235,7 @@
       grid.x = p.grid_x;
     }
   }
-  CA_LAUNCH(k_gemm_x[p.lay + 4 * p.ks], grid, dim3(p.block), p.lds, s, g);
+  CA_LAUNCH(r240 ? k_gemm_x240[p.lay] : k_gemm_x[p.lay + 4 * p.ks], grid, dim3(p.block), p.lds, s, g);
 }
 static int gemm_launch_plan(const GemmPlan& p, const CaGemmDesc& d, CaGemmGroup* grp, hipStream_t s, const char* who) {
   const dim3 grid(p.grid_x, p.grid_y, p.grid_z), block(p.block);
@@ -2156,7 +2248,7 @@
     if (rc != CA_OK) return rc;
   } else if (p.family == GEMM_X) {
     CaGemmGroup one;
-    if (!grp) one.d[0] = d, one.count = 0, one.first[0] = 0, one.total = 0;
+    if (!grp) one.d[0] = d, one.d[0].xcd_balanced = p.xbal, one.count = 0, one.first[0] = 0, one.total = 0;
     gemm_launch_x(p, grp ? *grp : one, s);
   } else if (p.family == GEMM_L) {
     allow_lds(LDS_FAM_L, k_gemm_l, 4, p.lds);
@@ -2211,15 +2303,16 @@
   const int rc = gemm_validate_group(descs, count);
   if (rc != CA_OK) return rc;
   CaGemmGroup g;
+  const GemmPlan p = gemm_plan_group(descs, count, gemm_knobs());
   int total = 0;
   for (int i = 0; i < X_GROUP_MAX; ++i) {
     g.d[i] = descs[i < count ? i : 0];
+    g.d[i].xcd_balanced = p.xbal;
     g.first[i] = total;
-    if (i < count) total += gemm_x_tiles(descs[i]);
+    if (i < count) total += gemm_x_tiles(descs[i], p.xrows);
   }
   g.total = total;
   g.count = count > 1 ? count : 0;
-  const GemmPlan p = gemm_plan_group(descs, count, gemm_knobs());
   ProfRec r;
   if (g_prof_on) {
     hipEventCreate(&r.e0);
diff --git a/coral_amd/csrc/gemm_plan.h b/coral_amd/csrc/gemm_plan.h
--- a/coral_amd/csrc/gemm_plan.h
+++ b/coral_amd/csrc/gemm_plan.h
@@ -16,6 +16,7 @@
 #define LBN 128
 #define XBM 256
 #define XBN 256
+#define X_ROWS_240 240
 #define EPI_PITCH 68
 #define LDS_BYTES (4 * 64 * EPI_PITCH * 4)
 #define M_LDS_BYTES (2 * 4 * BM * BK * 2)
@@ -110,6 +111,8 @@
   int l_min = 100;
   int m_max = 256;
   int force_kernel = 0;
+  int force_x_rows = 0;
+  int x_rows240 = 0;
   int compute_cus = 0;
   unsigned device_cus = 256;
 };
@@ -133,8 +136,32 @@
   unsigned vgrid = 0;
   int persistent = 0, dyn_first = 0;
   int kind = 0;
+  int xrows = XBM;
+  int xbal = 0;
 };
-inline int gemm_x_tiles(const CaGemmDesc& d) { return ((d.M + XBM - 1) / XBM) * ((d.N + XBN - 1) / XBN); }
+inline int gemm_x_tiles(const CaGemmDesc& d, int rows = XBM) { return ((d.M + rows - 1) / rows) * ((d.N + XBN - 1) / XBN); }
+
+inline bool gemm_x240_balanced(int ntm, int ntn, const GemmKnobs& k) {
+  if (ntm * ntn <= 8) return false;
+  int hb, wb;
+  xcd_split(ntm, ntn, hb, wb);
+  const int per_xcd = (int)gemm_compute_cus(k) / 8, even = (ntm * ntn + 7) / 8;
+  return (hb * wb + per_xcd - 1) / per_xcd > (even + per_xcd - 1) / per_xcd;
+}
+inline int gemm_x_rows(const CaGemmDesc* descs, int count, int64_t nb, const GemmKnobs& k) {
+  int64_t t256 = 0, t240 = 0;
+  for (int i = 0; i < count; ++i) {
+    if (descs[i].a_kseg > 0 || descs[i].b_kseg > 0 || descs[i].c_sumsq != nullptr) return XBM;
+    t256 += gemm_x_tiles(descs[i], XBM);
+    t240 += gemm_x_tiles(descs[i], X_ROWS_240);
+  }
+  if (k.force_x_rows == X_ROWS_240 || k.force_x_rows == XBM) return k.force_x_rows;
+  if (!k.x_rows240) return XBM;
+  const int64_t cus = (int64_t)gemm_compute_cus(k);
+  const int64_t m256 = ((t256 * nb + cus - 1) / cus) * XBM, m240 = ((t240 * nb + cus - 1) / cus) * X_ROWS_240;
+  if (t240 * nb > cus) return XBM;
+  return m240 < m256 ? X_ROWS_240 : XBM;
+}
 
 inline void gemm_plan_x_geometry(GemmPlan& p, unsigned vgrid, unsigned nbz, const GemmKnobs& k) {
   const unsigned ncu = gemm_compute_cus(k);
@@ -248,7 +275,9 @@
   p.grid_z = nb;
   switch (p.family) {
     case GEMM_X:
-      gemm_plan_x_geometry(p, tile_grid<4, 8>((d.M + XBM - 1) / XBM, (d.N + XBN - 1) / XBN, bal), nb, k);
+      p.xrows = gemm_x_rows(&d, 1, nb, k);
+      p.xbal = (bal || (p.xrows == X_ROWS_240 && gemm_x240_balanced((d.M + p.xrows - 1) / p.xrows, (d.N + XBN - 1) / XBN, k))) ? 1 : 0;
+      gemm_plan_x_geometry(p, tile_grid<4, 8>((d.M + p.xrows - 1) / p.xrows, (d.N + XBN - 1) / XBN, p.xbal != 0), nb, k);
       break;
     case GEMM_L:
       p.kind = 1;
@@ -291,10 +320,13 @@
 inline GemmPlan gemm_plan_group(const CaGemmDesc* descs, int count, const GemmKnobs& k) {
   GemmPlan p;
   p.lay = (descs->a_layout ? 2 : 0) + (descs->b_layout ? 1 : 0);
+  p.xrows = gemm_x_rows(descs, count, 1, k);
   int total = 0;
-  for (int i = 0; i < count; ++i) total += gemm_x_tiles(descs[i]);
+  for (int i = 0; i < count; ++i) total += gemm_x_tiles(descs[i], p.xrows);
+  p.xbal = (count == 1 && p.xrows == X_ROWS_240 &&
+            gemm_x240_balanced((descs->M + p.xrows - 1) / p.xrows, (descs->N + XBN - 1) / XBN, k)) ? 1 : 0;
   const unsigned vgrid = count > 1 ? (unsigned)(8 * ((total + 7) / 8))
-                                   : tile_grid<4, 8>((descs->M + XBM - 1) / XBM, (descs->N + XBN - 1) / XBN);
+                                   : tile_grid<4, 8>((descs->M + p.xrows - 1) / p.xrows, (descs->N + XBN - 1) / XBN, p.xbal != 0);
   gemm_plan_x_geometry(p, vgrid, 1, k);
   return p;
 }
diff --git a/coral_amd/ops.py b/coral_amd/ops.py
--- a/coral_amd/ops.py
+++ b/coral_amd/ops.py
@@ -111,6 +111,15 @@
     check(lib().ca_gemm_bf16(C.byref(d), _stream()), "ca_gemm_bf16")
 
 
+def gemm_x_rows(descs):
+    arr = (CaGemmDesc * len(descs))(*descs)
+    tiles = C.c_int32(0)
+    rows = lib().ca_gemm_x_rows(arr, len(descs), C.byref(tiles))
+    if rows < 0:
+        check(rows, "ca_gemm_x_rows")
+    return int(rows), int(tiles.value)
+
+
 _SPLITK_WS: dict = {}
 FUSE_BIAS_GRAD = os.environ.get("CA_FUSE_BIAS", "1") == "1"
 FUSE_BIAS_PARTIAL_MIN_K = int(os.environ.get("CA_FUSE_BIAS_PARTIAL_MIN_K", "8192"))
diff --git a/include/coral_amd.h b/include/coral_amd.h
--- a/include/coral_amd.h
+++ b/include/coral_amd.h
@@ -95,6 +95,9 @@
 
 int ca_gemm_force_kernel(int which);
 int ca_gemm_debug_general_epilogue(int on);
+int ca_gemm_force_x_rows(int rows);
+int ca_gemm_x_rows(const CaGemmDesc* descs, int32_t count, int32_t* tiles);
+int ca_gemm_x_counters_busy(void);
 int ca_debug_cu_hog(int32_t blocks, int32_t threads, int32_t lds_bytes, double ms, void* stream);
 
 int ca_gemm_set_compute_cus(int n);
```

New measurement: 1129 audio-seconds/sec, median of 6. Within noise of the previous version (+0.2%).
